# OpenStitching/stitching

Hardware: AMD Instinct MI355X
Metric: warped+blended Mpix/s (higher is better)
Workload: dtype u8/int16 (fixed-point remap, int32 pyramid sums, fp32 weights); 1 GPU; BASELINE config 2: 8 synthetic 4000x3000 frames, one ring; yaw step 38.9 deg = 0.58 hfov (42 % overlap; SURVEY 8(d) names 0.70 hfov); spherical warp + 5-band multiband blend, inputs resident in HBM; frames_per_gpu=8, panoramas_in_flight=2

## Files before the change

### include/stitching_amd.h

```cpp
#ifndef STITCHING_AMD_H
#define STITCHING_AMD_H

#include <stddef.h>
#include <stdint.h>

#ifdef __cplusplus
extern "C" {
#endif

#define STX_VERSION 100

#define STX_OK 0
#define STX_ERR_INVALID (-1)
#define STX_ERR_HIP (-2)
#define STX_ERR_OOM (-3)
#define STX_ERR_STATE (-4)
#define STX_ERR_UNSUPPORTED (-5)

#define STX_TRIG_EXACT 0
#define STX_TRIG_GLIBC 1
#define STX_TRIG_GLIBC_NOFMA 2
int stx_set_trig_mode(int mode);
int stx_get_trig_mode(void);

#define STX_REMAP_Q15 0
#define STX_REMAP_FLOAT 1
#define STX_REMAP_FLOAT_FMA 2
int stx_set_remap_mode(int mode);
int stx_get_remap_mode(void);

#define STX_PYRDOWN_SCALAR 0
#define STX_PYRDOWN_SIMD_V 1
#define STX_PYRDOWN_SIMD_HV 3
#define STX_PYRDOWN_FMA 4
int stx_set_pyrdown_mode(int mode, int lanes);
int stx_get_pyrdown_mode(int* out_lanes);

#define STX_WARP_PLANE 0
#define STX_WARP_AFFINE 1
#define STX_WARP_CYLINDRICAL 2
#define STX_WARP_SPHERICAL 3
#define STX_WARP_FISHEYE 4
#define STX_WARP_STEREOGRAPHIC 5
#define STX_WARP_COMPRESSED_PLANE_A2B1 6
#define STX_WARP_COMPRESSED_PLANE_A15B1 7
#define STX_WARP_COMPRESSED_PLANE_PORTRAIT_A2B1 8
#define STX_WARP_COMPRESSED_PLANE_PORTRAIT_A15B1 9
#define STX_WARP_PANINI_A2B1 10
#define STX_WARP_PANINI_A15B1 11
#define STX_WARP_PANINI_PORTRAIT_A2B1 12
#define STX_WARP_PANINI_PORTRAIT_A15B1 13
#define STX_WARP_MERCATOR 14
#define STX_WARP_TRANSVERSE_MERCATOR 15
#define STX_WARP_TYPE_COUNT 16

#define STX_INTER_NEAREST 0
#define STX_INTER_LINEAR 1
#define STX_BORDER_CONSTANT 0
#define STX_BORDER_REFLECT 2

#define STX_BLEND_NO 0
#define STX_BLEND_FEATHER 1
#define STX_BLEND_MULTIBAND 2

#define STX_U8 0
#define STX_S16 1
#define STX_F32 2

typedef struct stx_ctx stx_ctx;
typedef struct stx_buf stx_buf;
typedef struct stx_blender stx_blender;

int stx_version(void);
const char* stx_last_error(void);
int stx_device_count(int* out_n);
int stx_ctx_create(int device, stx_ctx** out);
int stx_ctx_destroy(stx_ctx* ctx);
int stx_ctx_sync(stx_ctx* ctx);

int stx_buf_from_host(stx_ctx* ctx, const void* host, size_t host_stride_bytes, int w, int h, int channels, int elem,
                      stx_buf** out);
int stx_buf_alloc(stx_ctx* ctx, int w, int h, int channels, int elem, stx_buf** out);
int stx_host_alloc(size_t bytes, void** out);
int stx_host_free(void* p);
int stx_buf_to_host(const stx_buf* buf, void* host, size_t host_stride_bytes);
int stx_buf_from_host_async(stx_ctx* ctx, const void* host, size_t host_stride_bytes, int w, int h, int channels, int elem,
                            stx_buf** out);
int stx_buf_to_host_async(const stx_buf* buf, void* host, size_t host_stride_bytes);
int stx_buf_view(const stx_buf* buf, int x, int y, int w, int h, stx_buf** out);
int stx_buf_info(const stx_buf* buf, int64_t info[6]);
int stx_buf_device_ptr(const stx_buf* buf, void** out);
int stx_buf_free(stx_buf* buf);

int stx_warp_roi(stx_ctx* ctx, int type, float scale, const float K[9], const float R[9], int w, int h,
                 int out_xywh[4]);
int stx_warp_rois(stx_ctx* ctx, int type, float scale, int n, const float* K9s, const float* R9s, const int* sizes_wh,
                  int* out_xywh);
int stx_warp(stx_ctx* ctx, int type, float scale, const float K[9], const float R[9], const stx_buf* src, int interp,
             int border, stx_buf** out, int out_tl[2]);
int stx_warp_image_and_mask(stx_ctx* ctx, int type, float scale, const float K[9], const float R[9],
                            const stx_buf* src, stx_buf** out_img, stx_buf** out_mask, int out_xywh[4]);
int stx_warp_batch(stx_ctx* ctx, int type, float scale, int n, const float* K9s, const float* R9s,
                   const stx_buf* const* srcs, stx_buf** out_imgs, stx_buf** out_masks, int* out_xywh);
int stx_warp_batch_rects(stx_ctx* ctx, int type, float scale, int n, const float* K9s, const float* R9s,
                         const stx_buf* const* srcs, const int* rects_xywh, stx_buf** out_imgs, stx_buf** out_masks);
int stx_warp_batch_gain(stx_ctx* ctx, int type, float scale, int n, const float* K9s, const float* R9s, const stx_buf* const* srcs,
                        const int* rects_xywh, const stx_buf* const* gain_maps_f32, const int* gain_flags, stx_buf** out_imgs,
                        stx_buf** out_masks, int* out_xywh);
int stx_warp_batch_with_rois(stx_ctx* ctx, int type, float scale, int n, const float* K9s, const float* R9s, const stx_buf* const* srcs,
                             const stx_buf* const* gain_maps_f32_or_null, const int* gain_flags_or_null, stx_buf** out_imgs,
                             stx_buf** out_masks, int* out_xywh);
int stx_warp_mask(stx_ctx* ctx, int type, float scale, const float K[9], const float R[9], int w, int h,
                  stx_buf** out_mask, int out_xywh[4]);

int stx_result_roi(int n, const int* corners_xy, const int* sizes_wh, int out_xywh[4]);
int stx_blend_create(stx_ctx* ctx, int kind, int num_bands, float sharpness, const int roi_xywh[4],
                     stx_blender** out);
int stx_blend_num_bands(const stx_blender* b, int* out_num_bands);
int stx_blend_feed(stx_blender* b, const stx_buf* img, const stx_buf* mask, int tlx, int tly);
int stx_blend_finish(stx_blender* b, stx_buf** out_pano_u8, stx_buf** out_mask_u8);
int stx_blend_finish_ex(stx_blender* b, stx_buf** out_pano_u8, stx_buf** out_mask_u8, stx_buf** out_pano_s16);
int stx_blend_destroy(stx_blender* b);

int stx_gain_apply(stx_ctx* ctx, stx_buf* img_u8x3, const float gains_bgr[3]);
int stx_block_gain_apply(stx_ctx* ctx, stx_buf* img_u8x3, const stx_buf* gain_map_f32);
#define STX_GAIN_MAP_BOUNDED 1
int stx_block_gain_apply_batch(stx_ctx* ctx, int n, stx_buf* const* imgs_u8x3, const stx_buf* const* gain_maps_f32,
                               const int* full_wh_xy0, const int* flags);
#define STX_EXPOSURE_GAIN 1
#define STX_EXPOSURE_GAIN_BLOCKS 2
#define STX_EXPOSURE_CHANNELS 3
#define STX_EXPOSURE_CHANNELS_BLOCKS 4
int stx_exposure_feed(stx_ctx* ctx, int kind, int n, const stx_buf* const* imgs_u8x3, const stx_buf* const* masks_u8,
                      const int* corners_xy, int block_size, int nr_feeds, double* out_gains, long long* inout_count,
                      double out_info[4]);
int stx_exposure_stats(stx_ctx* ctx, int kind, int n, const stx_buf* const* imgs_u8x3, const stx_buf* const* masks_u8,
                       const int* corners_xy, int block_size, long long* inout_jobs, int* out_ab, long long* out_c,
                       double* out_sums);
int stx_exposure_solve(int m, int npairs, const int* pairs_ij, const double* n_iij_iji, const unsigned char* skip,
                       double* out_gains);
#define STX_EXPOSURE_SOLVER_DEFAULT (-1)
#define STX_EXPOSURE_SOLVER_HOST 0
#define STX_EXPOSURE_SOLVER_DEVICE 1
int stx_set_exposure_solver(int mode);
int stx_get_exposure_solver(void);
int stx_exposure_feed_ex(stx_ctx* ctx, int kind, int n, const stx_buf* const* imgs_u8x3, const stx_buf* const* masks_u8,
                         const int* corners_xy, int block_size, int nr_feeds, int solver, double* out_gains, long long* inout_count,
                         double out_info[8]);
int stx_exposure_solve_device(stx_ctx* ctx, int m, int npairs, const int* pairs_ij, const double* n_iij_iji, const unsigned char* skip,
                              double* out_gains, double out_info[4]);
int stx_lu_solve_device(stx_ctx* ctx, int n, const double* A_dense_host, const double* b_host, double* x_out, double out_info[4]);
#define STX_SEAM_NO 0
#define STX_SEAM_VORONOI 1
#define STX_SEAM_GAP 10
int stx_seam_find(stx_ctx* ctx, int kind, int n, const int* sizes_wh, const int* corners_xy, const stx_buf* const* masks_in,
                  stx_buf** masks_out, double out_info[4]);
int stx_seam_schedule(int n, const int* sizes_wh, const int* corners_xy, int* inout_npairs, int* out_pairs, int* out_levels);
#define STX_COLOR_SEAM_MAX_LENGTH 16384
#define STX_COLOR_SEAM_MAX_CROSS 4096
int stx_color_seam_find(stx_ctx* ctx, int n, const int* sizes_wh, const int* corners_xy, const stx_buf* const* images,
                        const stx_buf* const* masks_in, stx_buf** masks_out, double out_info[4]);
int stx_crop_lir(stx_ctx* ctx, const stx_buf* mask_u8x1, int out_xywh[4], int out_contours[2], double out_info[1]);
#define STX_FEATURES_MAX_SIDE 32767
#define STX_FEATURES_MAX_LEVELS 16
#define STX_FEATURES_MAX_FEATURES 65536
int stx_features_detect(stx_ctx* ctx, int n, const stx_buf* const* images, const stx_buf* const* masks, int nfeatures, int nlevels,
                        int fast_threshold, const int* level_counts, const int* level_wh, const int* quotas, const int* cxcy,
                        const signed char* patterns, int* out_counts, int* out_lxyb, long long* out_R, unsigned char* out_desc,
                        double out_info[4]);
int stx_resize_linear_exact(stx_ctx* ctx, const stx_buf* src_u8, int dst_w, int dst_h, stx_buf** out);
int stx_seam_mask_resize(stx_ctx* ctx, const stx_buf* seam_mask_u8x1, const stx_buf* final_mask_u8x1, stx_buf** out);
int stx_resize_linear_exact_batch(stx_ctx* ctx, int n, const stx_buf* const* srcs_u8, const int* dst_wh, stx_buf** outs);
int stx_seam_mask_resize_batch(stx_ctx* ctx, int n, const stx_buf* const* seam_masks, const stx_buf* const* final_masks,
                               stx_buf** outs);
int stx_seam_mask_resize_batch_sub(stx_ctx* ctx, int n, const stx_buf* const* seam_masks, const stx_buf* const* final_masks,
// ... 59 lines not shown
```

### stitching_amd/_lib.py

```python
import ctypes as C
import os

from .stitching_error import StitchingError

_HERE = os.path.dirname(os.path.abspath(__file__))
LIB_PATH = os.environ.get("STITCHING_AMD_LIB") or os.path.join(_HERE, "libstitching_amd.so")

STX_OK = 0
WARP_PLANE, WARP_AFFINE, WARP_CYLINDRICAL, WARP_SPHERICAL = 0, 1, 2, 3
WARP_TYPE_IDS = {"plane": 0, "affine": 1, "cylindrical": 2, "spherical": 3, "fisheye": 4, "stereographic": 5,
                 "compressedPlaneA2B1": 6, "compressedPlaneA1.5B1": 7, "compressedPlanePortraitA2B1": 8,
                 "compressedPlanePortraitA1.5B1": 9, "paniniA2B1": 10, "paniniA1.5B1": 11, "paniniPortraitA2B1": 12,
                 "paniniPortraitA1.5B1": 13, "mercator": 14, "transverseMercator": 15}
INTER_NEAREST, INTER_LINEAR = 0, 1
BORDER_CONSTANT, BORDER_REFLECT = 0, 2
BLEND_NO, BLEND_FEATHER, BLEND_MULTIBAND = 0, 1, 2
U8, S16, F32 = 0, 1, 2
TRIG_MODES = {"exact": 0, "glibc": 1, "glibc-nofma": 2}
REMAP_MODES = {"q15": 0, "float": 1, "float-fma": 2}
PYRDOWN_MODES = {"scalar": 0, "simd-v": 1, "simd-hv": 3, "simd-v-fma": 5, "simd-hv-fma": 7}
GAIN_MAP_BOUNDED = 1
EXPOSURE_KINDS = {"gain": 1, "gain_blocks": 2, "channel": 3, "channel_blocks": 4}
EXPOSURE_SOLVERS = {"host": 0, "device": 1}
LU_NB, LU_MAX_N = 32, 16384
SEAM_KINDS = {"no": 0, "voronoi": 1}
COLOR_SEAM_MAX_LENGTH, COLOR_SEAM_MAX_CROSS = 16384, 4096
FEATURES_MAX_SIDE, FEATURES_MAX_LEVELS, FEATURES_MAX_FEATURES = 32767, 16, 65536
CONTRIB_U8_BINARY = 1
STRIP_MASK_BITS = 2

EXPORTS = (
    "stx_version stx_last_error stx_set_trig_mode stx_get_trig_mode stx_set_remap_mode stx_get_remap_mode stx_set_pyrdown_mode stx_get_pyrdown_mode stx_device_count stx_ctx_create stx_ctx_destroy stx_ctx_sync "
    "stx_host_alloc stx_host_free stx_buf_from_host stx_buf_from_host_async stx_buf_alloc stx_buf_to_host stx_buf_to_host_async stx_buf_view stx_buf_info stx_buf_device_ptr stx_buf_free "
    "stx_warp_roi stx_warp_rois stx_warp stx_warp_image_and_mask stx_warp_batch stx_warp_batch_rects stx_warp_batch_gain stx_warp_batch_with_rois stx_warp_mask "
    "stx_gain_apply stx_block_gain_apply stx_block_gain_apply_batch stx_resize_linear_exact stx_resize_linear_exact_batch stx_seam_mask_resize stx_seam_mask_resize_batch stx_seam_mask_resize_batch_sub stx_timelapse_frame stx_result_roi stx_blend_create stx_blend_num_bands stx_blend_feed stx_blend_finish stx_blend_finish_ex "
    "stx_blend_destroy stx_blend_set_band stx_blend_feed_ex stx_blend_contrib_rect stx_blend_export_contrib stx_blend_export_contribs "
    "stx_blend_build stx_blend_feed_contrib stx_blend_feed_contrib_ex stx_buf_flags stx_strip_rect stx_view_rect stx_strip_pack stx_strip_pack_batch stx_strip_pack_batch_ex stx_strip_bytes stx_strip_unpack stx_blend_feed_strips stx_comm_unique_id stx_comm_create stx_comm_exchange stx_comm_exchange_begin stx_comm_exchange_end stx_comm_exchange_begin_on stx_comm_exchange_end_on stx_comm_info stx_comm_destroy stx_prof_enable stx_prof_reset stx_prof_count stx_prof_get stx_mark stx_mark_elapsed_ms "
    "stx_exposure_feed stx_exposure_stats stx_exposure_solve stx_set_exposure_solver stx_get_exposure_solver stx_exposure_feed_ex stx_exposure_solve_device stx_lu_solve_device stx_seam_find stx_seam_schedule stx_color_seam_find stx_crop_lir stx_features_detect "
    "stx_debug_warp_maps stx_debug_feather_dist_cap"
).split()

_lib = None


def build_hint():
    return "build it with `make -C stitching_amd/csrc` or `python -c 'import __graft_entry__ as g; g.build()'`"


def lib():
    global _lib
    if _lib is not None:
        return _lib
    if not os.path.exists(LIB_PATH):
        raise ImportError(f"{LIB_PATH} is missing: the HIP back end is not built ({build_hint()}). "
                          "stitching_amd has no CPU fallback.")
    L = C.CDLL(LIB_PATH)
    vp, vpp = C.c_void_p, C.POINTER(C.c_void_p)
    fp, ip = C.POINTER(C.c_float), C.POINTER(C.c_int)
    L.stx_version.restype = C.c_int
    L.stx_last_error.restype = C.c_char_p
    L.stx_set_trig_mode.argtypes = [C.c_int]
    L.stx_get_trig_mode.restype = C.c_int
    L.stx_set_remap_mode.argtypes = [C.c_int]
    L.stx_get_remap_mode.restype = C.c_int
    L.stx_set_pyrdown_mode.argtypes = [C.c_int, C.c_int]
    L.stx_get_pyrdown_mode.argtypes = [C.POINTER(C.c_int)]
    L.stx_get_pyrdown_mode.restype = C.c_int
    L.stx_device_count.argtypes = [ip]
    L.stx_ctx_create.argtypes = [C.c_int, vpp]
    L.stx_ctx_destroy.argtypes = [vp]
    L.stx_ctx_sync.argtypes = [vp]
    L.stx_buf_from_host.argtypes = [vp, vp, C.c_size_t, C.c_int, C.c_int, C.c_int, C.c_int, vpp]
    L.stx_buf_from_host_async.argtypes = L.stx_buf_from_host.argtypes
    L.stx_buf_alloc.argtypes = [vp, C.c_int, C.c_int, C.c_int, C.c_int, vpp]
    L.stx_host_alloc.argtypes = [C.c_size_t, vpp]
    L.stx_host_free.argtypes = [vp]
    L.stx_buf_to_host.argtypes = [vp, vp, C.c_size_t]
    L.stx_buf_to_host_async.argtypes = [vp, vp, C.c_size_t]
    L.stx_buf_view.argtypes = [vp, C.c_int, C.c_int, C.c_int, C.c_int, vpp]
    L.stx_buf_info.argtypes = [vp, C.POINTER(C.c_int64)]
    L.stx_buf_device_ptr.argtypes = [vp, vpp]
    L.stx_buf_free.argtypes = [vp]
    L.stx_warp_roi.argtypes = [vp, C.c_int, C.c_float, fp, fp, C.c_int, C.c_int, ip]
    L.stx_warp_rois.argtypes = [vp, C.c_int, C.c_float, C.c_int, fp, fp, ip, ip]
    L.stx_warp.argtypes = [vp, C.c_int, C.c_float, fp, fp, vp, C.c_int, C.c_int, vpp, ip]
    L.stx_warp_image_and_mask.argtypes = [vp, C.c_int, C.c_float, fp, fp, vp, vpp, vpp, ip]
    L.stx_warp_batch.argtypes = [vp, C.c_int, C.c_float, C.c_int, fp, fp, vpp, vpp, vpp, ip]
    L.stx_warp_batch_rects.argtypes = [vp, C.c_int, C.c_float, C.c_int, fp, fp, vpp, ip, vpp, vpp]
    L.stx_warp_batch_gain.argtypes = [vp, C.c_int, C.c_float, C.c_int, fp, fp, vpp, ip, vpp, ip, vpp, vpp, ip]
    L.stx_warp_batch_with_rois.argtypes = [vp, C.c_int, C.c_float, C.c_int, fp, fp, vpp, vpp, ip, vpp, vpp, ip]
    L.stx_warp_mask.argtypes = [vp, C.c_int, C.c_float, fp, fp, C.c_int, C.c_int, vpp, ip]
    L.stx_gain_apply.argtypes = [vp, vp, fp]
    L.stx_block_gain_apply.argtypes = [vp, vp, vp]
    L.stx_block_gain_apply_batch.argtypes = [vp, C.c_int, vpp, vpp, ip, ip]
    L.stx_resize_linear_exact.argtypes = [vp, vp, C.c_int, C.c_int, vpp]
    L.stx_resize_linear_exact_batch.argtypes = [vp, C.c_int, vpp, ip, vpp]
    L.stx_seam_mask_resize.argtypes = [vp, vp, vp, vpp]
    L.stx_seam_mask_resize_batch.argtypes = [vp, C.c_int, vpp, vpp, vpp]
    L.stx_seam_mask_resize_batch_sub.argtypes = [vp, C.c_int, vpp, vpp, ip, vpp]
    L.stx_timelapse_frame.argtypes = [vp, vp, C.c_int, C.c_int, ip, vpp]
    L.stx_result_roi.argtypes = [C.c_int, ip, ip, ip]
    L.stx_blend_create.argtypes = [vp, C.c_int, C.c_int, C.c_float, ip, vpp]
    L.stx_blend_num_bands.argtypes = [vp, ip]
    L.stx_blend_feed.argtypes = [vp, vp, vp, C.c_int, C.c_int]
    L.stx_blend_finish.argtypes = [vp, vpp, vpp]
    L.stx_blend_finish_ex.argtypes = [vp, vpp, vpp, vpp]
    L.stx_blend_destroy.argtypes = [vp]
    L.stx_blend_set_band.argtypes = [vp, C.c_int, C.c_int]
    L.stx_blend_feed_ex.argtypes = [vp, vp, vp, C.c_int, C.c_int, C.c_int]
    L.stx_blend_contrib_rect.argtypes = [vp, C.c_int, C.c_int, C.c_int, C.c_int, C.c_int, C.c_int, ip,
                                         C.POINTER(C.c_size_t)]
    L.stx_blend_export_contrib.argtypes = [vp, C.c_int, C.c_int, C.c_int, vpp, ip]
    L.stx_blend_export_contribs.argtypes = [vp, C.c_int, ip, ip, ip, vpp, ip]
    L.stx_blend_build.argtypes = [vp]
    L.stx_blend_feed_contrib.argtypes = [vp, C.c_int, ip, vp]
    L.stx_blend_feed_contrib_ex.argtypes = [vp, C.c_int, ip, vp, C.c_int]
    L.stx_buf_flags.argtypes = [vp, ip]
    L.stx_strip_rect.argtypes = [vp, C.c_int, C.c_int, C.c_int, C.c_int, C.c_int, C.c_int, ip, C.POINTER(C.c_size_t)]
    L.stx_view_rect.argtypes = [vp, C.c_int, C.c_int, C.c_int, C.c_int, C.c_int, C.c_int, C.c_int, C.c_int, ip]
    L.stx_strip_pack.argtypes = [vp, vp, vp, C.c_int, C.c_int, vpp]
    L.stx_strip_unpack.argtypes = [vp, C.c_int, C.c_int, C.c_int, vpp, vpp]
    L.stx_strip_pack_batch.argtypes = [vp, C.c_int, vpp, vpp, ip, ip, vpp]
    L.stx_strip_pack_batch_ex.argtypes = [vp, C.c_int, vpp, vpp, ip, ip, C.c_int, vpp]
    L.stx_strip_bytes.argtypes = [C.c_int, C.c_int, C.c_int, C.POINTER(C.c_size_t)]
    L.stx_blend_feed_strips.argtypes = [vp, C.c_int, vpp, ip, ip, ip, ip, ip, C.c_int]
    L.stx_comm_unique_id.argtypes = [C.POINTER(C.c_ubyte)]
    L.stx_comm_create.argtypes = [vp, C.c_int, C.c_int, C.POINTER(C.c_ubyte), vpp]
    L.stx_comm_exchange.argtypes = [vp, C.c_int, ip, ip, C.POINTER(C.c_void_p), C.POINTER(C.c_size_t)]
    L.stx_comm_exchange_begin.argtypes = [vp, C.c_int, ip, ip, C.POINTER(C.c_void_p), C.POINTER(C.c_size_t)]
    L.stx_comm_exchange_end.argtypes = [vp]
    L.stx_comm_exchange_begin_on.argtypes = [vp, vp, C.c_int, ip, ip, C.POINTER(C.c_void_p), C.POINTER(C.c_size_t)]
    L.stx_comm_exchange_end_on.argtypes = [vp, vp]
    L.stx_comm_info.argtypes = [vp, ip]
    L.stx_comm_destroy.argtypes = [vp]
    L.stx_prof_enable.argtypes = [vp, C.c_int]
    L.stx_prof_reset.argtypes = [vp]
    L.stx_prof_count.argtypes = [vp, ip]
    L.stx_prof_get.argtypes = [vp, C.c_int, C.c_char_p, C.c_int, C.POINTER(C.c_int64), C.POINTER(C.c_double),
                               C.POINTER(C.c_double)]
    L.stx_debug_warp_maps.argtypes = [vp, C.c_int, C.c_float, fp, fp, C.c_int, C.c_int, C.c_int, ip, vpp, vpp, ip]
    llp, dp = C.POINTER(C.c_longlong), C.POINTER(C.c_double)
    L.stx_exposure_feed.argtypes = [vp, C.c_int, C.c_int, vpp, vpp, ip, C.c_int, C.c_int, dp, llp, dp]
    L.stx_exposure_stats.argtypes = [vp, C.c_int, C.c_int, vpp, vpp, ip, C.c_int, llp, ip, llp, dp]
    L.stx_exposure_solve.argtypes = [C.c_int, C.c_int, ip, dp, C.POINTER(C.c_ubyte), dp]
    L.stx_set_exposure_solver.argtypes = [C.c_int]
    L.stx_exposure_feed_ex.argtypes = [vp, C.c_int, C.c_int, vpp, vpp, ip, C.c_int, C.c_int, C.c_int, dp, llp, dp]
    L.stx_exposure_solve_device.argtypes = [vp, C.c_int, C.c_int, ip, dp, C.POINTER(C.c_ubyte), dp, dp]
    L.stx_lu_solve_device.argtypes = [vp, C.c_int, dp, dp, dp, dp]
    L.stx_seam_find.argtypes = [vp, C.c_int, C.c_int, ip, ip, vpp, vpp, dp]
    L.stx_seam_schedule.argtypes = [C.c_int, ip, ip, ip, ip, ip]
    L.stx_color_seam_find.argtypes = [vp, C.c_int, ip, ip, vpp, vpp, vpp, dp]
    L.stx_crop_lir.argtypes = [vp, vp, ip, ip, dp]
    L.stx_features_detect.argtypes = [vp, C.c_int, vpp, vpp, C.c_int, C.c_int, C.c_int, ip, ip, ip, ip, C.POINTER(C.c_byte), ip, ip, llp,
                                      C.POINTER(C.c_ubyte), dp]
    L.stx_mark.argtypes = [vp, C.c_int]
    L.stx_mark_elapsed_ms.argtypes = [vp, C.c_int, C.c_int, C.POINTER(C.c_double)]
    for name in EXPORTS:
        if name not in ("stx_version", "stx_last_error"):
            getattr(L, name).restype = C.c_int
    _lib = L
# ... 8 lines not shown
```

### stitching_amd/blender.py

```python
import ctypes as C

import numpy as np

from . import _lib, config
from .device import DeviceImage, as_device, get_context
from .stitching_error import StitchingError


class _BlenderHandle:

    def __init__(self, ctx, kind, num_bands, sharpness, roi):
        self.ctx = ctx
        self.kind = kind
        h = C.c_void_p()
        r = (C.c_int * 4)(*[int(v) for v in roi])
        _lib.check(ctx._lib.stx_blend_create(ctx.handle, kind, int(num_bands), float(sharpness), r, C.byref(h)))
        self._h = h

    def num_bands(self):
        n = C.c_int()
        _lib.check(self.ctx._lib.stx_blend_num_bands(self._h, C.byref(n)))
        return n.value

    def feed(self, img, mask, corner):
        _lib.check(self.ctx._lib.stx_blend_feed(self._h, img._h, mask._h, int(corner[0]), int(corner[1])))

    def blend(self, want_s16=False):
        pano, mask, p16 = C.c_void_p(), C.c_void_p(), C.c_void_p()
        _lib.check(self.ctx._lib.stx_blend_finish_ex(self._h, C.byref(pano), C.byref(mask),
                                                     C.byref(p16) if want_s16 else None))
        res = [DeviceImage(self.ctx, pano), DeviceImage(self.ctx, mask)]
        if want_s16:
            res.append(DeviceImage(self.ctx, p16))
        return res

    def __del__(self):
        try:
            if self._h is not None:
                if getattr(self.ctx, "handle", None) or getattr(self.ctx, "device", 0) == -1:
                    self.ctx._lib.stx_blend_destroy(self._h)
                self._h = None
        except Exception:
            pass


class Blender:

    BLENDER_CHOICES = (
        "multiband",
        "feather",
        "no",
    )
    DEFAULT_BLENDER = "multiband"
    DEFAULT_BLEND_STRENGTH = 5

    def __init__(
        self, blender_type=DEFAULT_BLENDER, blend_strength=DEFAULT_BLEND_STRENGTH, ctx=None
    ):
        self.blender_type = blender_type
        self.blend_strength = blend_strength
        self.blender = None
        self.ctx = ctx

    @staticmethod
    def result_roi(corners, sizes):
        c = np.ascontiguousarray([[int(p[0]), int(p[1])] for p in corners], np.int32)
        s = np.ascontiguousarray([[int(p[0]), int(p[1])] for p in sizes], np.int32)
        if len(c) == 0 or len(c) != len(s):
            raise StitchingError("prepare needs one size per corner and at least one image")
        out = (C.c_int * 4)()
        ip = C.POINTER(C.c_int)
        _lib.check(_lib.lib().stx_result_roi(len(c), c.ctypes.data_as(ip), s.ctypes.data_as(ip), out))
        return tuple(int(v) for v in out)

    @staticmethod
    def plan(blender_type, blend_strength, dst_sz):
        blend_width = np.sqrt(dst_sz[2] * dst_sz[3]) * blend_strength / 100
        if blender_type == "no" or blend_width < 1:
# ... 38 lines not shown
```

### stitching_amd/csrc/stx_blend.hip

```cpp
#include <cstring>

#include "stx_blend_kernels.h"
#include "stx_device_math.h"
#include "stx_internal.h"

using namespace stxd;

namespace {

constexpr float WEIGHT_EPS = 1e-5f;
constexpr float INV255 = 0.0039215688593685627f;
constexpr float INV256 = 0.00390625f;

template <bool S16>
STX_DEV void load_px0(const StxMbImage& im, int sx, int sy, int& b, int& g, int& r)
{
    if (S16) {
        const short* p = reinterpret_cast<const short*>(im.img0 + (long long)sy * im.img0_stride) + sx * 3;
        b = p[0]; g = p[1]; r = p[2];
    } else {
        const uint8_t* p = im.img0 + (long long)sy * im.img0_stride + sx * 3;
        b = p[0]; g = p[1]; r = p[2];
    }
}
// ... 594 lines not shown
    }
    __syncthreads();
    for (int i = tid; i < CO_TW * CO_TH; i += 256) {
        const int yy = i / CO_TW, xx = i - yy * CO_TW;
        const int x = tx0 + xx, y = ty0 + yy;
        if (x >= tx1 || y >= ty1) continue;
        int v[3];
        mb_gather_norm(P.images, P.n_images, B, B - 2, x, y, v);
        short* O = P.out + (long long)y * P.out_stride + (x - P.out_x0);
#pragma unroll
        for (int c = 0; c < 3; c++)
            O[c * P.out_plane] = (short)sat_s16(pyr_up_at_lds(s1[c], CO_W1, ax0, ay0, pw1, ph1, x, y) + v[c]);
    }
}

template <bool L0>
__global__ __launch_bounds__(256) void mb_level_kernel(MbLevelK P)
{
    mb_level_body<L0>(P);
}

template <bool L0>
__global__ __launch_bounds__(256) void mb_level_multi_kernel(const MbLevelK* __restrict__ Ps)
{
    mb_level_body<L0>(Ps[blockIdx.z]);
}

constexpr int DT_INF = 1 << 28;
constexpr int DT_RC = STX_DT_RC;
STX_DEV int wave_excl_prefix_min(int v)
{
    constexpr int ID = 0x7fffffff;
    v = min(v, __builtin_amdgcn_update_dpp(ID, v, 0x111, 0xf, 0xf, false));
    v = min(v, __builtin_amdgcn_update_dpp(ID, v, 0x112, 0xf, 0xf, false));
    v = min(v, __builtin_amdgcn_update_dpp(ID, v, 0x114, 0xf, 0xf, false));
    v = min(v, __builtin_amdgcn_update_dpp(ID, v, 0x118, 0xf, 0xf, false));
    v = min(v, __builtin_amdgcn_update_dpp(ID, v, 0x142, 0xa, 0xf, false));
    v = min(v, __builtin_amdgcn_update_dpp(ID, v, 0x143, 0xc, 0xf, false));
    return __builtin_amdgcn_update_dpp(ID, v, 0x138, 0xf, 0xf, false);
}

int check_launch(const char* what)
{
    hipError_t e = hipGetLastError();
    if (e != hipSuccess) return stx_fail(STX_ERR_HIP, "%s launch failed: %s", what, hipGetErrorString(e));
    return STX_OK;
}

inline dim3 grid64x4(int w, int h) { return dim3((w + 63) / 64, (h + 3) / 4); }

}

int stx_launch_mb_pyramids(stx_ctx* ctx, const StxMbImage* d_images, const StxMbImage* h_images, int n, int num_bands, int pyr_mode,
                           int pyr_lanes)
{
    for (int lv = 0; lv < num_bands; lv++) {
        double bytes = 0.0;
        bool any_s16 = false;
        for (int i = 0; i < n; i++) {
            const StxMbImage& im = h_images[i];
            const double ip = (double)(im.fw >> lv) * (im.fh >> lv), op = ip / 4.0;
            const double gw = (im.g_u8 ? 3.0 : 6.0) + 4.0;
            const double gw1 = gw - (im.w1_f16 ? 2.0 : 0.0);
            if (lv == 0) bytes += ((im.img0_is_s16 ? 6.0 : 3.0) + 1.0) * im.iw * im.ih + gw1 * op;
            else bytes += (lv == 1 ? gw1 : gw) * ip + gw * op;
            any_s16 = any_s16 || im.img0_is_s16;
        }
        StxProfScope prof(ctx, lv == 0 ? "mb_down0" : "mb_down", bytes);
        const bool batched = pyr_mode == STX_PYRDOWN_SCALAR && stx_fast_mb_down_batch(ctx, d_images, h_images, n, lv);
        for (int i = 0; i < n; i++) {
            const StxMbImage& im = h_images[i];
            if (batched && !(lv == 0 && im.img0_is_s16)) continue;
            const int ow = (im.fw >> lv) >> 1, oh = (im.fh >> lv) >> 1;
            if (lv == 0) {
                if (im.img0_is_s16) hipLaunchKernelGGL(mb_down0_kernel<true>, grid64x4(ow, oh), dim3(256), 0, ctx->stream, im, pyr_mode, pyr_lanes);
                else hipLaunchKernelGGL(mb_down0_kernel<false>, grid64x4(ow, oh), dim3(256), 0, ctx->stream, im, pyr_mode, pyr_lanes);
            } else {
                hipLaunchKernelGGL(mb_down_kernel, grid64x4(ow, oh), dim3(256), 0, ctx->stream, im, lv, pyr_mode, pyr_lanes);
            }
        }
        STX_TRY(check_launch("mb_down"));
    }
    return STX_OK;
}

int stx_launch_mb_coarse(stx_ctx* ctx, const MbLevelK& K, double algo_bytes)
{
    if (K.x1 <= K.x0 || K.y1 <= K.y0) return STX_OK;
    if (K.level != K.num_bands - 2 || K.level < 1 || K.y0 != 0 || K.out_y0 != 0 || K.emit)
        return stx_fail(STX_ERR_INVALID, "mb_coarse: not the argument block of level B-2");
    StxProfScope prof(ctx, "mb_coarse", algo_bytes);
    MbCoarseK C;
    C.images = K.images; C.n_images = K.n_images; C.num_bands = K.num_bands;
    C.x0 = K.x0; C.x1 = K.x1; C.y1 = K.y1;
    C.out = K.out; C.out_stride = K.out_stride; C.out_plane = K.out_plane; C.out_x0 = K.out_x0;
    C.pw = K.pw; C.ph = K.ph;
    const dim3 grid((K.x1 - K.x0 + CO_TW - 1) / CO_TW, (K.y1 + CO_TH - 1) / CO_TH);
    hipLaunchKernelGGL(mb_coarse_kernel, grid, dim3(256), 0, ctx->stream, C);
    return check_launch("mb_coarse");
}

int stx_launch_mb_level(stx_ctx* ctx, const MbLevelK& K, double algo_bytes)
{
    if (K.x1 <= K.x0 || K.y1 <= K.y0) return STX_OK;
    StxProfScope prof(ctx, K.emit ? "mb_contrib" : (K.level == 0 ? "mb_level0" : "mb_level"), algo_bytes);
    if ((K.level > 0 || K.all_u8) && stx_fast_mb_level(ctx, K)) return STX_OK;
    const dim3 grid = grid64x4(K.x1 - K.x0, K.y1 - K.y0);
    if (K.level == 0) hipLaunchKernelGGL(mb_level_kernel<true>, grid, dim3(256), 0, ctx->stream, K);
    else hipLaunchKernelGGL(mb_level_kernel<false>, grid, dim3(256), 0, ctx->stream, K);
    return check_launch("mb_level");
}

int stx_launch_mb_emit_batch(stx_ctx* ctx, const MbLevelK* d_Ks, const MbLevelK* h_Ks, const int* classes, int n, double bytes)
{
    if (n <= 0) return STX_OK;
    StxProfScope prof(ctx, "mb_contrib", bytes);
    for (int start = 0; start < n;) {
        int end = start;
        while (end < n && classes[end] == classes[start]) end++;
        const int cls = classes[start], count = end - start;
        if (cls >= 0) {
            if (!stx_fast_mb_emit_launch(ctx, cls, d_Ks + start, h_Ks + start, count)) return check_launch("mb_contrib");
// ... 1178 lines not shown
```

### stitching_amd/csrc/stx_blend_fast.hip

```cpp
#include <algorithm>
#include <cstdlib>

#include "stx_blend_kernels.h"
#include "stx_device_math.h"

using namespace stxd;

namespace {

#ifndef STX_L0_WAVES
#define STX_L0_WAVES 5
#endif
#ifndef STX_L0_NORM
#define STX_L0_NORM 3
#endif
#ifndef STX_ABLATE_MASK
#define STX_ABLATE_MASK 0
#endif
#ifndef STX_L0_FULL
#define STX_L0_FULL 1
#endif
constexpr float WEIGHT_EPS = 1e-5f;
constexpr float INV255 = 0.0039215688593685627f;
constexpr float INV256 = 0.00390625f;
// ... 247 lines not shown
    const v4u d1 = *reinterpret_cast<const STX_GAS v4u_a4*>(q + 16);
    const v2u d2 = *reinterpret_cast<const STX_GAS v2u_a4*>(q + 32);
    w[0] = __builtin_amdgcn_alignbyte(d0.y, d0.x, s);
    w[1] = __builtin_amdgcn_alignbyte(d0.z, d0.y, s);
    w[2] = __builtin_amdgcn_alignbyte(d0.w, d0.z, s);
    w[3] = __builtin_amdgcn_alignbyte(d1.x, d0.w, s);
    w[4] = __builtin_amdgcn_alignbyte(d1.y, d1.x, s);
    w[5] = __builtin_amdgcn_alignbyte(d1.z, d1.y, s);
    w[6] = __builtin_amdgcn_alignbyte(d1.w, d1.z, s);
    w[7] = __builtin_amdgcn_alignbyte(d2.x, d1.w, s);
    w[8] = __builtin_amdgcn_alignbyte(d2.y, d2.x, s);
}
template <bool MIRROR, int C>
STX_DEV void dn_pack5_channel(const uint32_t* w, short* hs)
{
#define STX_PXB(k) (MIRROR ? 30 - 3 * (k) + C : 3 * (k) + C)
    const pk16 A = pk(pair_u8<STX_PXB(0), STX_PXB(2)>(w)), Bp = pk(pair_u8<STX_PXB(1), STX_PXB(3)>(w));
    const pk16 Cp = pk(pair_u8<STX_PXB(2), STX_PXB(4)>(w)), D = pk(pair_u8<STX_PXB(3), STX_PXB(5)>(w));
    const pk16 E = pk(pair_u8<STX_PXB(4), STX_PXB(6)>(w)), F = pk(pair_u8<STX_PXB(5), STX_PXB(7)>(w));
    const pk16 G = pk(pair_u8<STX_PXB(6), STX_PXB(8)>(w)), H = pk(pair_u8<STX_PXB(7), STX_PXB(9)>(w));
    const pk16 I = pk(pair_u8<STX_PXB(8), STX_PXB(10)>(w));
#undef STX_PXB
    const pk16 o01 = A + E + Cp * pk_splat(6) + (Bp + D) * pk_splat(4);
    const pk16 o23 = E + I + G * pk_splat(6) + (F + H) * pk_splat(4);
    *reinterpret_cast<uint2*>(hs) = make_uint2(unpk(o01), unpk(o23));
}

#ifndef STX_DN0_DOT4
#define STX_DN0_DOT4 0
#endif
STX_DEV float4 dn_mask_sums4(const uint32_t (&mb)[3])
{
#if STX_DN0_DOT4
    const uint32_t o0 = __builtin_amdgcn_udot4(mb[0], 0x04060401u, mb[1] & 1u, false);
    const uint32_t o1 = __builtin_amdgcn_udot4(mb[1], 0x00010406u, __builtin_amdgcn_udot4(mb[0], 0x04010000u, 0u, false), false);
    const uint32_t o2 = __builtin_amdgcn_udot4(mb[1], 0x04060401u, mb[2] & 1u, false);
    const uint32_t o3 = __builtin_amdgcn_udot4(mb[2], 0x00010406u, __builtin_amdgcn_udot4(mb[1], 0x04010000u, 0u, false), false);
    return make_float4((float)o0, (float)o1, (float)o2, (float)o3);
#else
    const pk16 o01 = pk(pair_u8<0, 2>(mb)) + pk(pair_u8<4, 6>(mb)) + pk(pair_u8<2, 4>(mb)) * pk_splat(6) +
                     (pk(pair_u8<1, 3>(mb)) + pk(pair_u8<3, 5>(mb))) * pk_splat(4);
    const pk16 o23 = pk(pair_u8<4, 6>(mb)) + pk(pair_u8<8, 10>(mb)) + pk(pair_u8<6, 8>(mb)) * pk_splat(6) +
                     (pk(pair_u8<5, 7>(mb)) + pk(pair_u8<7, 9>(mb))) * pk_splat(4);
    return make_float4((float)(unpk(o01) & 0xffffu), (float)(unpk(o01) >> 16), (float)(unpk(o23) & 0xffffu), (float)(unpk(o23) >> 16));
#endif
}

struct DnImage0 {
    int fw, fh, iw, ih, left, top;
    uint32_t img0_stride, mask0_stride;
    const uint8_t* img0;
    const uint8_t* mask0;
};
template <bool PK, bool NEAR, class IM>
STX_DEV void dn_task_level0(const IM& im, int row, int xo, short* hs0, short* hs1, short* hs2, float* hw)
{
    const int by = reflect101_near(row, im.fh) - im.top;
    const bool yin = (unsigned)by < (unsigned)im.ih;
    const int sy = NEAR ? reflect_near(by, im.ih) : reflect(by, im.ih);
    const STX_GAS uint8_t* img = gp(im.img0);
    const uint32_t rowoff = (uint32_t)sy * (uint32_t)im.img0_stride;
    const int c0 = 2 * xo - 2;
    const int a0 = c0 - im.left;
    int px[11][3];
    float f[11];
    if (c0 >= 0 && c0 + 10 < im.fw && a0 >= 0 && a0 + 10 < im.iw) {
        uint32_t w[9];
        dn_load36(img, rowoff + (uint32_t)a0 * 3u, w);
        dn_pack5_channel<false, 0>(w, hs0);
        dn_pack5_channel<false, 1>(w, hs1);
        dn_pack5_channel<false, 2>(w, hs2);
        uint32_t mw[3] = {0u, 0u, 0u};
        if (yin) {
            const uint32_t moff = (uint32_t)by * (uint32_t)im.mask0_stride + (uint32_t)a0;
            const STX_GAS uint8_t* mq = gp(im.mask0) + (moff & ~3u);
            const uint32_t ms = moff & 3u;
            const v4u m = *reinterpret_cast<const STX_GAS v4u_a4*>(mq);
            mw[0] = __builtin_amdgcn_alignbyte(m.y, m.x, ms);
            mw[1] = __builtin_amdgcn_alignbyte(m.z, m.y, ms);
            mw[2] = __builtin_amdgcn_alignbyte(m.w, m.z, ms) & 0x00ffffffu;
        }
        bool packed = PK;
        if (!PK) {
            const uint32_t odd = (mw[0] ^ (((mw[0] >> 7) & 0x01010101u) * 255u)) | (mw[1] ^ (((mw[1] >> 7) & 0x01010101u) * 255u)) |
                                 (mw[2] ^ (((mw[2] >> 7) & 0x01010101u) * 255u));
            packed = __builtin_amdgcn_ballot_w64(odd != 0u) == 0ull;
        }
        if (packed) {
            uint32_t mb[3];
            mb[0] = mw[0] & 0x01010101u;
            mb[1] = mw[1] & 0x01010101u;
            mb[2] = mw[2] & 0x01010101u;
            *reinterpret_cast<float4*>(hw) = dn_mask_sums4(mb);
            return;
        }
#pragma unroll
        for (int j = 0; j < 11; j++) f[j] = fmul((float)byte_of(mw, j), INV255);
#pragma unroll
        for (int o = 0; o < 4; o++) hw[o] = h5f(f[2 * o], f[2 * o + 1], f[2 * o + 2], f[2 * o + 3], f[2 * o + 4]);
        return;
    }
    if (c0 >= 0 && c0 + 10 < im.fw && (a0 + 10 < 0 || a0 >= im.iw)) {
        const int s_low = a0 + 10 < 0 ? -(a0 + 10) - 1 : 2 * im.iw - 1 - (a0 + 10);
        if (s_low >= 0 && s_low + 10 < im.iw) {
            uint32_t w[9];
            dn_load36(img, rowoff + (uint32_t)s_low * 3u, w);
            dn_pack5_channel<true, 0>(w, hs0);
            dn_pack5_channel<true, 1>(w, hs1);
            dn_pack5_channel<true, 2>(w, hs2);
            *reinterpret_cast<float4*>(hw) = make_float4(0.f, 0.f, 0.f, 0.f);
            return;
        }
    }
    {
        const STX_GAS uint8_t* mrow = gp(im.mask0) + (uint32_t)min(max(by, 0), im.ih - 1) * (uint32_t)im.mask0_stride;
#pragma unroll
        for (int j = 0; j < 11; j++) {
            const int bx = reflect101_near(c0 + j, im.fw) - im.left;
            const int sx = NEAR ? reflect_near(bx, im.iw) : reflect(bx, im.iw);
            const STX_GAS uint8_t* p = img + (rowoff + (uint32_t)sx * 3u);
            px[j][0] = p[0]; px[j][1] = p[1]; px[j][2] = p[2];
            const float mv = fmul((float)mrow[sx], INV255);
            f[j] = (yin && (unsigned)bx < (unsigned)im.iw) ? mv : 0.f;
        }
    }
#pragma unroll
    for (int o = 0; o < 4; o++) {
        hs0[o] = (short)h5i(px[2 * o][0], px[2 * o + 1][0], px[2 * o + 2][0], px[2 * o + 3][0], px[2 * o + 4][0]);
        hs1[o] = (short)h5i(px[2 * o][1], px[2 * o + 1][1], px[2 * o + 2][1], px[2 * o + 3][1], px[2 * o + 4][1]);
        hs2[o] = (short)h5i(px[2 * o][2], px[2 * o + 1][2], px[2 * o + 2][2], px[2 * o + 3][2], px[2 * o + 4][2]);
        hw[o] = h5f(f[2 * o], f[2 * o + 1], f[2 * o + 2], f[2 * o + 3], f[2 * o + 4]);
    }
}

STX_DEV int occ_pitch(int lw) { return (((lw + 63) >> 6) + 3) & ~3; }
STX_DEV void dn_note_occ(uint8_t* __restrict__ occ, uint32_t nzbits, int tid, int X0, int Y0, int ow, int oh)
{
    const unsigned long long bal = __ballot(nzbits != 0u);
    const int rg = tid >> 5;
    if (occ == nullptr || (tid & 31) != 0 || 2 * rg >= DN_TOH || Y0 + 2 * rg >= oh) return;
    const uint32_t half = (tid & 32) ? (uint32_t)(bal >> 32) : (uint32_t)bal;
    occ[(long long)((Y0 >> 1) + rg) * occ_pitch(ow) + (X0 >> 6)] = half != 0u ? 1 : 0;
}

#ifndef STX_DN0_REV
#define STX_DN0_REV 1
#endif
#ifndef STX_DN0_BATCH
#define STX_DN0_BATCH 3
#endif
template <bool PK>
__global__ __launch_bounds__(256) void mb_down0_lds_kernel(const StxMbImage* __restrict__ images, StxTileMap M)
{
    __shared__ __attribute__((aligned(16))) short s_h[3][DN_ROWS][DN_TOW];
    __shared__ __attribute__((aligned(16))) float s_w[DN_ROWS][DN_TOW];
    const uint32_t zz = STX_DN0_REV ? gridDim.z - 1u - blockIdx.z : blockIdx.z, bb = STX_DN0_REV ? gridDim.x - 1u - blockIdx.x : blockIdx.x;
    const StxMbImage& im = images[zz];
    const int tid = threadIdx.x;
    const int ow = im.fw >> 1, oh = im.fh >> 1;
    int tile_tx, tile_ty;
    if (!xcd_tile(M, bb, tile_tx, tile_ty)) return;
    const int X0 = tile_tx * DN_TOW, Y0 = tile_ty * DN_TOH;
    if (im.img0_is_s16 || X0 >= ow || Y0 >= oh) return;
    uint8_t* const occ = im.occ[1];
    const bool w1h = im.w1_f16 != 0;
    asm volatile("" ::"s"(occ));
    DnImage0 D;
    {
        int fw = im.fw, fh = im.fh, iw_ = im.iw, ih_ = im.ih, left = im.left, top = im.top;
        uint32_t is = (uint32_t)im.img0_stride, ms = (uint32_t)im.mask0_stride;
        unsigned long long ia = (unsigned long long)im.img0, ma = (unsigned long long)im.mask0;
        if (PK) asm volatile("" : "+s"(fw), "+s"(fh), "+s"(iw_), "+s"(ih_), "+s"(left), "+s"(top), "+s"(is), "+s"(ms), "+s"(ia), "+s"(ma));
        D.fw = fw; D.fh = fh; D.iw = iw_; D.ih = ih_; D.left = left; D.top = top; D.img0_stride = is; D.mask0_stride = ms;
        D.img0 = (const uint8_t*)ia; D.mask0 = (const uint8_t*)ma;
    }
    uint32_t g1_plane = 0, g1_stride = 0, w1_stride = 0;
    unsigned long long g1_a = 0, w1_a = 0;
    if (PK) {
        g1_plane = (uint32_t)im.g_plane[1]; g1_stride = (uint32_t)im.g_stride[1]; w1_stride = (uint32_t)im.wt_stride[1];
        g1_a = (unsigned long long)im.g[1]; w1_a = (unsigned long long)im.wt[1];
        asm volatile("" : "+s"(g1_plane), "+s"(g1_stride), "+s"(w1_stride), "+s"(g1_a), "+s"(w1_a));
    }
    const int r_end = 2 * min(DN_TOH, oh - Y0) + 3;
    const bool near = PK ? (D.left <= D.iw && D.fw - D.left - D.iw <= D.iw && D.top <= D.ih && D.fh - D.top - D.ih <= D.ih)
                         : (im.left <= im.iw && im.fw - im.left - im.iw <= im.iw && im.top <= im.ih && im.fh - im.top - im.ih <= im.ih);
    bool batched = false;
    if ((STX_DN0_BATCH & (PK ? 1 : 2)) && near) {
        const int q = tid & 15, rA = tid >> 4;
        const int xo = X0 + 4 * q, c0 = 2 * xo - 2, a0 = c0 - D.left;
        const bool col_ok = xo < ow;
        const bool in_frame = c0 >= 0 && c0 + 10 < D.fw;
        const bool interior = in_frame && a0 >= 0 && a0 + 10 < D.iw;
        const int s_low = a0 + 10 < 0 ? -(a0 + 10) - 1 : 2 * D.iw - 1 - (a0 + 10);
        const bool mirrored = in_frame && (a0 + 10 < 0 || a0 >= D.iw) && s_low >= 0 && s_low + 10 < D.iw;
        batched = __builtin_amdgcn_ballot_w64(col_ok && !(interior || mirrored)) == 0ull;
        if (batched && col_ok) {
            const int acol = interior ? a0 : s_low;
            v4u d0[2], d1[2], mq4[2];
            v2u d2[2];
            uint32_t sh[2], msh[2];
            bool yin[2], live[2];
#pragma unroll
            for (int t = 0; t < 2; t++) {
                const int r = rA + 16 * t;
                live[t] = r < r_end && r < DN_ROWS;
                const int row = 2 * Y0 - 2 + min(r, r_end - 1);
                const int by = reflect101_near(row, D.fh) - D.top;
                yin[t] = (unsigned)by < (unsigned)D.ih;
                const int sy = reflect_near(by, D.ih);
                const uint32_t off = (uint32_t)sy * (uint32_t)D.img0_stride + (uint32_t)acol * 3u;
                const STX_GAS uint8_t* p = gp(D.img0) + (off & ~3u);
                sh[t] = off & 3u;
                d0[t] = *reinterpret_cast<const STX_GAS v4u_a4*>(p);
                d1[t] = *reinterpret_cast<const STX_GAS v4u_a4*>(p + 16);
                d2[t] = *reinterpret_cast<const STX_GAS v2u_a4*>(p + 32);
                const uint32_t moff = (uint32_t)min(max(by, 0), D.ih - 1) * (uint32_t)D.mask0_stride + (uint32_t)acol;
                msh[t] = moff & 3u;
#if STX_ABLATE_MASK
                mq4[t] = v4u{0xffffffffu, 0xffffffffu, 0xffffffffu, 0xffffffffu};
#else
                mq4[t] = *reinterpret_cast<const STX_GAS v4u_a4*>(gp(D.mask0) + (moff & ~3u));
#endif
            }
            __builtin_amdgcn_sched_barrier(0);
#pragma unroll
            for (int t = 0; t < 2; t++) {
                if (!live[t]) continue;
                const int r = rA + 16 * t;
                uint32_t w[9];
                w[0] = __builtin_amdgcn_alignbyte(d0[t].y, d0[t].x, sh[t]);
                w[1] = __builtin_amdgcn_alignbyte(d0[t].z, d0[t].y, sh[t]);
                w[2] = __builtin_amdgcn_alignbyte(d0[t].w, d0[t].z, sh[t]);
                w[3] = __builtin_amdgcn_alignbyte(d1[t].x, d0[t].w, sh[t]);
                w[4] = __builtin_amdgcn_alignbyte(d1[t].y, d1[t].x, sh[t]);
                w[5] = __builtin_amdgcn_alignbyte(d1[t].z, d1[t].y, sh[t]);
                w[6] = __builtin_amdgcn_alignbyte(d1[t].w, d1[t].z, sh[t]);
                w[7] = __builtin_amdgcn_alignbyte(d2[t].x, d1[t].w, sh[t]);
                w[8] = __builtin_amdgcn_alignbyte(d2[t].y, d2[t].x, sh[t]);
                if (interior) {
                    dn_pack5_channel<false, 0>(w, &s_h[0][r][4 * q]);
                    dn_pack5_channel<false, 1>(w, &s_h[1][r][4 * q]);
                    dn_pack5_channel<false, 2>(w, &s_h[2][r][4 * q]);
                } else {
                    dn_pack5_channel<true, 0>(w, &s_h[0][r][4 * q]);
                    dn_pack5_channel<true, 1>(w, &s_h[1][r][4 * q]);
                    dn_pack5_channel<true, 2>(w, &s_h[2][r][4 * q]);
                }
                const uint32_t keep = (yin[t] && interior) ? 0xffffffffu : 0u;
                uint32_t mw[3];
                mw[0] = __builtin_amdgcn_alignbyte(mq4[t].y, mq4[t].x, msh[t]) & keep;
                mw[1] = __builtin_amdgcn_alignbyte(mq4[t].z, mq4[t].y, msh[t]) & keep;
                mw[2] = __builtin_amdgcn_alignbyte(mq4[t].w, mq4[t].z, msh[t]) & keep & 0x00ffffffu;
                bool packed = PK;
                if (!PK) {
                    const uint32_t odd = (mw[0] ^ (((mw[0] >> 7) & 0x01010101u) * 255u)) | (mw[1] ^ (((mw[1] >> 7) & 0x01010101u) * 255u)) |
                                         (mw[2] ^ (((mw[2] >> 7) & 0x01010101u) * 255u));
                    packed = __builtin_amdgcn_ballot_w64(odd != 0u) == 0ull;
                }
                if (packed) {
                    uint32_t mb[3];
                    mb[0] = mw[0] & 0x01010101u;
                    mb[1] = mw[1] & 0x01010101u;
                    mb[2] = mw[2] & 0x01010101u;
                    *reinterpret_cast<float4*>(&s_w[r][4 * q]) = dn_mask_sums4(mb);
                } else {
                    float f[11];
#pragma unroll
                    for (int j = 0; j < 11; j++) f[j] = fmul((float)byte_of(mw, j), INV255);
#pragma unroll
                    for (int o = 0; o < 4; o++) s_w[r][4 * q + o] = h5f(f[2 * o], f[2 * o + 1], f[2 * o + 2], f[2 * o + 3], f[2 * o + 4]);
                }
            }
        }
    }
    for (int task = tid; task < DN_ROWS * (DN_TOW / 4) && !batched; task += 256) {
        const int r = task / (DN_TOW / 4), q = task % (DN_TOW / 4);
        if (X0 + 4 * q >= ow || r >= r_end) continue;
        if (PK) {
            if (near) dn_task_level0<PK, true>(D, 2 * Y0 - 2 + r, X0 + 4 * q, &s_h[0][r][4 * q], &s_h[1][r][4 * q], &s_h[2][r][4 * q], &s_w[r][4 * q]);
            else dn_task_level0<PK, false>(D, 2 * Y0 - 2 + r, X0 + 4 * q, &s_h[0][r][4 * q], &s_h[1][r][4 * q], &s_h[2][r][4 * q], &s_w[r][4 * q]);
        } else {
            if (near) dn_task_level0<PK, true>(im, 2 * Y0 - 2 + r, X0 + 4 * q, &s_h[0][r][4 * q], &s_h[1][r][4 * q], &s_h[2][r][4 * q], &s_w[r][4 * q]);
            else dn_task_level0<PK, false>(im, 2 * Y0 - 2 + r, X0 + 4 * q, &s_h[0][r][4 * q], &s_h[1][r][4 * q], &s_h[2][r][4 * q], &s_w[r][4 * q]);
        }
    }
    __syncthreads();
    const int p = tid & 31, rg = tid >> 5;
    const int xo = X0 + 2 * p;
    if (xo >= ow) return;
    const bool two = xo + 1 < ow;
    uint32_t nz = 0u;
#pragma unroll
    for (int rr = 0; rr < 2; rr++) {
        const int yl = 2 * rg + rr, y = Y0 + yl;
        if (yl >= DN_TOH || y >= oh) break;
#pragma unroll
        for (int c = 0; c < 3; c++) {
            pk16 a[5];
#pragma unroll
            for (int k = 0; k < 5; k++) a[k] = pk(*reinterpret_cast<const uint32_t*>(&s_h[c][2 * yl + k][2 * p]));
            const pk16 v = (a[0] + a[4] + a[2] * pk_splat(6) + (a[1] + a[3]) * pk_splat(4) + pk_splat(128)) >> pk_splat(8);
            STX_GAS uint8_t* o = PK ? gp(reinterpret_cast<uint8_t*>(g1_a)) + ((uint32_t)c * g1_plane + (uint32_t)y * g1_stride + (uint32_t)xo)
                                    : gp(reinterpret_cast<uint8_t*>(im.g[1])) + ((uint32_t)c * (uint32_t)im.g_plane[1] + (uint32_t)y * (uint32_t)im.g_stride[1] + (uint32_t)xo);
            const uint32_t b2 = __builtin_amdgcn_perm(0u, unpk(v), 0x0c0c0200u);
            if (two) *reinterpret_cast<STX_GAS uint16_t*>(o) = (uint16_t)b2;
            else o[0] = (uint8_t)b2;
        }
        float fa[5], fb[5];
        {
            typedef float v2 __attribute__((ext_vector_type(2)));
            v2 r0, r1, r2, r3, r4;
            const uint32_t a = (uint32_t)(uintptr_t)(__attribute__((address_space(3))) const float*)&s_w[2 * yl][2 * p];
            asm volatile("ds_read_b64 %0, %5\n\tds_read_b64 %1, %5 offset:256\n\tds_read_b64 %2, %5 offset:512\n\t"
                         "ds_read_b64 %3, %5 offset:768\n\tds_read_b64 %4, %5 offset:1024\n\ts_waitcnt lgkmcnt(0)"
                         : "=&v"(r0), "=&v"(r1), "=&v"(r2), "=&v"(r3), "=&v"(r4) : "v"(a) : "memory");
            fa[0] = r0.x; fb[0] = r0.y; fa[1] = r1.x; fb[1] = r1.y; fa[2] = r2.x; fb[2] = r2.y;
            fa[3] = r3.x; fb[3] = r3.y; fa[4] = r4.x; fb[4] = r4.y;
        }
        const float wa = fmul(h5f(fa[0], fa[1], fa[2], fa[3], fa[4]), INV256);
        const float wb = fmul(h5f(fb[0], fb[1], fb[2], fb[3], fb[4]), INV256);
        if (w1h) {
            STX_GAS _Float16* o = PK ? gp(reinterpret_cast<_Float16*>(w1_a)) + ((uint32_t)y * w1_stride + (uint32_t)xo)
                                     : reinterpret_cast<STX_GAS _Float16*>(gp(im.wt[1])) + ((uint32_t)y * (uint32_t)im.wt_stride[1] + (uint32_t)xo);
            typedef _Float16 v2h16 __attribute__((ext_vector_type(2)));
            if (two) { const v2h16 wab = {(_Float16)wa, (_Float16)wb}; *reinterpret_cast<STX_GAS v2h16*>(o) = wab; }
            else o[0] = (_Float16)wa;
        } else {
            STX_GAS float* o = PK ? gp(reinterpret_cast<float*>(w1_a)) + ((uint32_t)y * w1_stride + (uint32_t)xo)
                                  : gp(im.wt[1]) + ((uint32_t)y * (uint32_t)im.wt_stride[1] + (uint32_t)xo);
            typedef float v2fl __attribute__((ext_vector_type(2)));
            if (two) { const v2fl wab = {wa, wb}; *reinterpret_cast<STX_GAS v2fl*>(o) = wab; }
            else o[0] = wa;
        }
        nz |= __float_as_uint(wa) | (two ? __float_as_uint(wb) : 0u);
    }
    dn_note_occ(occ, nz, tid, X0, Y0, ow, oh);
}

STX_DEV void dn_load19_u8(const STX_GAS uint8_t* __restrict__ base, uint32_t off, int c0, int iw, bool fast, int s[19])
{
    if (fast) {
        const STX_GAS uint8_t* p = base + (off + (uint32_t)c0);
        const uint32_t a = *reinterpret_cast<const STX_GAS uint32_t*>(p - 2);
        const v4u b = *reinterpret_cast<const STX_GAS v4u*>(p + 2);
        const uint32_t c = *reinterpret_cast<const STX_GAS uint32_t*>(p + 18);
        const uint32_t w[6] = {a, b.x, b.y, b.z, b.w, c};
#pragma unroll
        for (int j = 0; j < 19; j++) s[j] = (int)byte_of(w, j + 2);
    } else {
#pragma unroll
        for (int j = 0; j < 19; j++) s[j] = base[off + (uint32_t)reflect101_near(c0 + j, iw)];
    }
}

STX_DEV void dn_load19_s16(const STX_GAS short* __restrict__ base, uint32_t off, int c0, int iw, bool fast, int s[19])
{
    if (fast) {
        const STX_GAS short* p = base + (off + (uint32_t)c0);
        const uint32_t a = *reinterpret_cast<const STX_GAS uint32_t*>(p);
        const v4u b = *reinterpret_cast<const STX_GAS v4u*>(p + 2);
        const v4u c = *reinterpret_cast<const STX_GAS v4u*>(p + 10);
        s[0] = s16lo(a); s[1] = s16hi(a);
        s[2] = s16lo(b.x); s[3] = s16hi(b.x); s[4] = s16lo(b.y); s[5] = s16hi(b.y);
        s[6] = s16lo(b.z); s[7] = s16hi(b.z); s[8] = s16lo(b.w); s[9] = s16hi(b.w);
        s[10] = s16lo(c.x); s[11] = s16hi(c.x); s[12] = s16lo(c.y); s[13] = s16hi(c.y);
        s[14] = s16lo(c.z); s[15] = s16hi(c.z); s[16] = s16lo(c.w); s[17] = s16hi(c.w);
        s[18] = p[18];
    } else {
#pragma unroll
        for (int j = 0; j < 19; j++) s[j] = base[off + (uint32_t)reflect101_near(c0 + j, iw)];
    }
}

STX_DEV void dn_hsum_store_i(const int (&s)[19], int* row_q)
{
    int4 lo, hi;
    lo.x = h5i(s[0], s[1], s[2], s[3], s[4]);
    lo.y = h5i(s[2], s[3], s[4], s[5], s[6]);
    lo.z = h5i(s[4], s[5], s[6], s[7], s[8]);
    lo.w = h5i(s[6], s[7], s[8], s[9], s[10]);
    hi.x = h5i(s[8], s[9], s[10], s[11], s[12]);
    hi.y = h5i(s[10], s[11], s[12], s[13], s[14]);
    hi.z = h5i(s[12], s[13], s[14], s[15], s[16]);
    hi.w = h5i(s[14], s[15], s[16], s[17], s[18]);
    *reinterpret_cast<int4*>(row_q) = make_int4(lo.x, lo.z, hi.x, hi.z);
    *reinterpret_cast<int4*>(row_q + 32) = make_int4(lo.y, lo.w, hi.y, hi.w);
}
STX_DEV void dn_hsum_store_f(const float (&f)[19], float* row_q)
{
    float4 lo, hi;
    lo.x = h5f(f[0], f[1], f[2], f[3], f[4]);
    lo.y = h5f(f[2], f[3], f[4], f[5], f[6]);
    lo.z = h5f(f[4], f[5], f[6], f[7], f[8]);
    lo.w = h5f(f[6], f[7], f[8], f[9], f[10]);
    hi.x = h5f(f[8], f[9], f[10], f[11], f[12]);
    hi.y = h5f(f[10], f[11], f[12], f[13], f[14]);
    hi.z = h5f(f[12], f[13], f[14], f[15], f[16]);
    hi.w = h5f(f[14], f[15], f[16], f[17], f[18]);
    *reinterpret_cast<float4*>(row_q) = make_float4(lo.x, lo.z, hi.x, hi.z);
    *reinterpret_cast<float4*>(row_q + 32) = make_float4(lo.y, lo.w, hi.y, hi.w);
}

__global__ __launch_bounds__(256) void mb_down_lds_kernel(const StxMbImage* __restrict__ images, int lv, StxTileMap M)
{
    __shared__ __attribute__((aligned(16))) int s_h[3][DN_ROWS][DN_TOW];
    __shared__ __attribute__((aligned(16))) float s_w[DN_ROWS][DN_TOW];
    const StxMbImage& im = images[blockIdx.z];
    const int tid = threadIdx.x;
    const int iw = im.fw >> lv, ih = im.fh >> lv;
    const int ow = iw >> 1, oh = ih >> 1;
    int tile_tx, tile_ty;
    if (!xcd_tile(M, blockIdx.x, tile_tx, tile_ty)) return;
    const int X0 = tile_tx * DN_TOW, Y0 = tile_ty * DN_TOH;
    if (X0 >= ow || Y0 >= oh) return;
    const bool g8b = im.g_u8 != 0;
    unsigned long long G_a = (unsigned long long)im.g[lv], W_a = (unsigned long long)im.wt[lv];
    unsigned long long Go_a = (unsigned long long)im.g[lv + 1], Wo_a = (unsigned long long)im.wt[lv + 1];
    uint32_t gs = (uint32_t)im.g_stride[lv], gpl = (uint32_t)im.g_plane[lv], wst = (uint32_t)im.wt_stride[lv];
    uint32_t gos = (uint32_t)im.g_stride[lv + 1], gopl = (uint32_t)im.g_plane[lv + 1], wost = (uint32_t)im.wt_stride[lv + 1];
    asm volatile("" : "+s"(G_a), "+s"(W_a), "+s"(Go_a), "+s"(Wo_a), "+s"(gs), "+s"(gpl), "+s"(wst), "+s"(gos), "+s"(gopl), "+s"(wost));
    const short* G = (const short*)G_a;
    uint8_t* const occ = im.occ[lv + 1];
    const bool w_half = lv == 1 && im.w1_f16 != 0;
    asm volatile("" ::"s"(occ));
    const int r_end = 2 * min(DN_TOH, oh - Y0) + 3;
    for (int task = tid; task < DN_ROWS * (DN_TOW / 8); task += 256) {
        const int r = task / (DN_TOW / 8), q = task % (DN_TOW / 8);
        if (X0 + 8 * q >= ow || r >= r_end) continue;
        const int sy = reflect101_near(2 * Y0 - 2 + r, ih);
        const int c0 = 2 * (X0 + 8 * q) - 2;
        const bool fast = c0 >= 0 && c0 + 18 < iw;
        typedef _Float16 v2h16 __attribute__((ext_vector_type(2)));
        typedef _Float16 v8h16 __attribute__((ext_vector_type(8)));
        if (g8b && __builtin_amdgcn_ballot_w64(!fast) == 0ull) {
            uint32_t ra[3], rc[3];
            v4u rb[3];
#pragma unroll
            for (int c = 0; c < 3; c++) {
                const STX_GAS uint8_t* pp = gp(reinterpret_cast<const uint8_t*>(G)) + ((uint32_t)c * gpl + (uint32_t)sy * gs + (uint32_t)c0);
                ra[c] = *reinterpret_cast<const STX_GAS uint32_t*>(pp - 2);
                rb[c] = *reinterpret_cast<const STX_GAS v4u*>(pp + 2);
                rc[c] = *reinterpret_cast<const STX_GAS uint32_t*>(pp + 18);
            }
            float f[19];
            if (w_half) {
                const STX_GAS _Float16* hq = gp(reinterpret_cast<const _Float16*>(W_a)) + (uint32_t)sy * wst;
                const v2h16 ha = *reinterpret_cast<const STX_GAS v2h16*>(hq + c0);
                const v8h16 hb = *reinterpret_cast<const STX_GAS v8h16*>(hq + c0 + 2), hc = *reinterpret_cast<const STX_GAS v8h16*>(hq + c0 + 10);
                const _Float16 hl = hq[c0 + 18];
                __builtin_amdgcn_sched_barrier(0);
                f[0] = (float)ha.x; f[1] = (float)ha.y;
#pragma unroll
                for (int k = 0; k < 8; k++) { f[2 + k] = (float)hb[k]; f[10 + k] = (float)hc[k]; }
                f[18] = (float)hl;
            } else {
                const STX_GAS float* wq0 = gp(reinterpret_cast<const float*>(W_a)) + (uint32_t)sy * wst;
                const v2u wa = *reinterpret_cast<const STX_GAS v2u*>(wq0 + c0);
                v4u wb4[4];
#pragma unroll
                for (int k4 = 0; k4 < 4; k4++) wb4[k4] = *reinterpret_cast<const STX_GAS v4u*>(wq0 + c0 + 2 + 4 * k4);
                const float wl = wq0[c0 + 18];
                __builtin_amdgcn_sched_barrier(0);
                f[0] = __uint_as_float(wa.x); f[1] = __uint_as_float(wa.y);
#pragma unroll
                for (int k = 0; k < 4; k++) {
                    f[2 + 4 * k] = __uint_as_float(wb4[k].x); f[3 + 4 * k] = __uint_as_float(wb4[k].y); f[4 + 4 * k] = __uint_as_float(wb4[k].z);
                    f[5 + 4 * k] = __uint_as_float(wb4[k].w);
                }
                f[18] = wl;
            }
#pragma unroll
            for (int c = 0; c < 3; c++) {
                const uint32_t w6[6] = {ra[c], rb[c].x, rb[c].y, rb[c].z, rb[c].w, rc[c]};
                int s[19];
#pragma unroll
                for (int j = 0; j < 19; j++) s[j] = (int)byte_of(w6, j + 2);
                dn_hsum_store_i(s, &s_h[c][r][4 * q]);
            }
            dn_hsum_store_f(f, &s_w[r][4 * q]);
            continue;
        }
#pragma unroll
        for (int c = 0; c < 3; c++) {
            int s[19];
            if (g8b) dn_load19_u8(gp(reinterpret_cast<const uint8_t*>(G)), (uint32_t)c * gpl + (uint32_t)sy * gs, c0, iw, fast, s);
            else dn_load19_s16(gp(G), (uint32_t)c * gpl + (uint32_t)sy * gs, c0, iw, fast, s);
            dn_hsum_store_i(s, &s_h[c][r][4 * q]);
        }
        const STX_GAS float* wq = gp(reinterpret_cast<const float*>(W_a)) + (uint32_t)sy * wst;
        float f[19];
        if (w_half) {
            const STX_GAS _Float16* hq = gp(reinterpret_cast<const _Float16*>(W_a)) + (uint32_t)sy * wst;
            if (fast) {
                const v2h16 a = *reinterpret_cast<const STX_GAS v2h16*>(hq + c0);
                const v8h16 b = *reinterpret_cast<const STX_GAS v8h16*>(hq + c0 + 2), c = *reinterpret_cast<const STX_GAS v8h16*>(hq + c0 + 10);
                f[0] = (float)a.x; f[1] = (float)a.y;
#pragma unroll
                for (int k = 0; k < 8; k++) { f[2 + k] = (float)b[k]; f[10 + k] = (float)c[k]; }
                f[18] = (float)hq[c0 + 18];
            } else {
#pragma unroll
                for (int j = 0; j < 19; j++) f[j] = (float)hq[reflect101_near(c0 + j, iw)];
            }
        } else if (fast) {
            const v2u a = *reinterpret_cast<const STX_GAS v2u*>(wq + c0);
            f[0] = __uint_as_float(a.x); f[1] = __uint_as_float(a.y);
#pragma unroll
            for (int k = 0; k < 4; k++) {
                const v4u b = *reinterpret_cast<const STX_GAS v4u*>(wq + c0 + 2 + 4 * k);
                f[2 + 4 * k] = __uint_as_float(b.x); f[3 + 4 * k] = __uint_as_float(b.y); f[4 + 4 * k] = __uint_as_float(b.z);
                f[5 + 4 * k] = __uint_as_float(b.w);
            }
            f[18] = wq[c0 + 18];
        } else {
#pragma unroll
            for (int j = 0; j < 19; j++) f[j] = wq[reflect101_near(c0 + j, iw)];
        }
        dn_hsum_store_f(f, &s_w[r][4 * q]);
    }
    __syncthreads();
    const int p = tid & 31, rg = tid >> 5;
    const int xo = X0 + 2 * p;
    if (xo >= ow) return;
    const bool two = xo + 1 < ow;
    uint32_t nz = 0u;
#pragma unroll
    for (int rr = 0; rr < 2; rr++) {
        const int yl = 2 * rg + rr, y = Y0 + yl;
        if (yl >= DN_TOH || y >= oh) break;
#pragma unroll
        for (int c = 0; c < 3; c++) {
            int a[5], b[5];
#pragma unroll
            for (int k = 0; k < 5; k++) {
                a[k] = s_h[c][2 * yl + k][p];
                b[k] = s_h[c][2 * yl + k][32 + p];
            }
            const int va = (h5i(a[0], a[1], a[2], a[3], a[4]) + 128) >> 8;
            const int vb = (h5i(b[0], b[1], b[2], b[3], b[4]) + 128) >> 8;
            const uint32_t oo = (uint32_t)c * gopl + (uint32_t)y * gos + (uint32_t)xo;
            if (g8b) {
                STX_GAS uint8_t* o = gp(reinterpret_cast<uint8_t*>(Go_a)) + oo;
                if (two) *reinterpret_cast<STX_GAS uint16_t*>(o) = (uint16_t)((uint32_t)va | ((uint32_t)vb << 8));
                else o[0] = (uint8_t)va;
            } else {
                STX_GAS short* o = gp(reinterpret_cast<short*>(Go_a)) + oo;
                if (two) *reinterpret_cast<STX_GAS uint32_t*>(o) = pack16(va, vb);
                else o[0] = (short)va;
            }
        }
        float fa[5], fb[5];
#pragma unroll
        for (int k = 0; k < 5; k++) {
            fa[k] = s_w[2 * yl + k][p];
            fb[k] = s_w[2 * yl + k][32 + p];
        }
        const float wa = fmul(h5f(fa[0], fa[1], fa[2], fa[3], fa[4]), INV256);
        const float wb = fmul(h5f(fb[0], fb[1], fb[2], fb[3], fb[4]), INV256);
        STX_GAS float* o = gp(reinterpret_cast<float*>(Wo_a)) + ((uint32_t)y * wost + (uint32_t)xo);
        typedef float v2fl __attribute__((ext_vector_type(2)));
        if (two) { const v2fl wab = {wa, wb}; *reinterpret_cast<STX_GAS v2fl*>(o) = wab; }
        else o[0] = wa;
        nz |= __float_as_uint(wa) | (two ? __float_as_uint(wb) : 0u);
    }
    dn_note_occ(occ, nz, tid, X0, Y0, ow, oh);
}

STX_DEV int s6(int v) { return (v + 32) >> 6; }

STX_DEV int trunc_small(float v) { return (int)v; }

template <class T>
STX_DEV void up_patch(const T* __restrict__ plane, long long stride, int cw, int ch, int cx, int cy, int up[2][8])
{
    const int rr[3] = {up_idx(cy - 1, ch), cy, up_idx(cy + 1, ch)};
    const bool le = cx == 0, re = cx + 4 >= cw;
    int he[3][4], ho[3][4];
#pragma unroll
    for (int r = 0; r < 3; r++) {
        const T* p = plane + (long long)rr[r] * stride;
        int c[6];
        if (sizeof(T) == 2) {
            const v4u w = *reinterpret_cast<const v4u_a4*>(p + cx - 2);
            c[1] = s16lo(w.y); c[2] = s16hi(w.y); c[3] = s16lo(w.z); c[4] = s16hi(w.z);
            c[0] = s16hi(w.x);
            c[5] = s16lo(w.w);
        } else {
            const v3u w = *reinterpret_cast<const v3u_a4*>(p + cx - 4);
            c[0] = (int)(w.x >> 24);
            c[1] = (int)(w.y & 255u); c[2] = (int)((w.y >> 8) & 255u); c[3] = (int)((w.y >> 16) & 255u); c[4] = (int)(w.y >> 24);
            c[5] = (int)(w.z & 255u);
        }
        if (le) c[0] = c[2];
        if (re) c[5] = c[4];
#pragma unroll
        for (int j = 0; j < 4; j++) {
            he[r][j] = c[j] + 6 * c[j + 1] + c[j + 2];
            ho[r][j] = 4 * (c[j + 1] + c[j + 2]);
        }
    }
#pragma unroll
    for (int j = 0; j < 4; j++) {
        up[0][2 * j] = s6(he[0][j] + 6 * he[1][j] + he[2][j]);
        up[0][2 * j + 1] = s6(ho[0][j] + 6 * ho[1][j] + ho[2][j]);
        up[1][2 * j] = s6(4 * (he[1][j] + he[2][j]));
        up[1][2 * j + 1] = s6(4 * (ho[1][j] + ho[2][j]));
    }
}

template <bool L0>
STX_DEV void level_epilogue(const MbLevelK& P, int X0, int Y0, int (&acc)[2][8][3], float (&ws)[2][8])
{
    int v[2][8][3];
#pragma unroll
    for (int r = 0; r < 2; r++)
#pragma unroll
        for (int j = 0; j < 8; j++) {
            const float den = fadd(ws[r][j], WEIGHT_EPS);
// ... 1119 lines not shown
#elif STX_LVPK_EPI == 2
        up_patch_pks_load(gp(plane0), (uint32_t)P.up_stride, P.ph >> 1, (uint32_t)(X0 >> 1) * 2u, Y0 >> 1, uw[0]);
        up_patch_pks_load(gp(plane0 + P.up_plane), (uint32_t)P.up_stride, P.ph >> 1, (uint32_t)(X0 >> 1) * 2u, Y0 >> 1, uw[1]);
        __builtin_amdgcn_sched_barrier(0);
#endif
#pragma unroll
        for (int c = 0; c < 3; c++) {
            const short* plane = P.up + c * P.up_plane - ((long long)P.up_y0 * P.up_stride + P.up_x0);
#if STX_LVPK_EPI == 2
            if (c == 0) {
                up_patch_pks_load(gp(plane0 + 2 * P.up_plane), (uint32_t)P.up_stride, P.ph >> 1, (uint32_t)(X0 >> 1) * 2u, Y0 >> 1, uw[2]);
                __builtin_amdgcn_sched_barrier(0);
            }
#elif STX_LVPK_EPI < 2
            up_patch_pks_load(gp(plane), (uint32_t)P.up_stride, P.ph >> 1, (uint32_t)(X0 >> 1) * 2u, Y0 >> 1, uw[c]);
#endif
            pk16s up[2][4];
            if (!up_patch_pks_math(uw[c], usel, up)) {
                int u32[2][8];
                up_patch(plane, P.up_stride, P.pw >> 1, P.ph >> 1, X0 >> 1, Y0 >> 1, u32);
#pragma unroll
                for (int r = 0; r < 2; r++) {
                    up[r][0] = pks(pack16(u32[r][0], u32[r][2]));
                    up[r][1] = pks(pack16(u32[r][4], u32[r][6]));
                    up[r][2] = pks(pack16(u32[r][1], u32[r][3]));
                    up[r][3] = pks(pack16(u32[r][5], u32[r][7]));
                }
            }
#pragma unroll
            for (int r = 0; r < 2; r++)
#pragma unroll
                for (int q = 0; q < 4; q++) v[r][c][q] = unpks(__builtin_elementwise_add_sat(up[r][q], pks(v[r][c][q])));
        }
    }
#pragma unroll
    for (int r = 0; r < 2; r++) {
        if (Y0 + r >= P.y1) break;
#pragma unroll
        for (int c = 0; c < 3; c++) {
            v4u o;
            o.x = __builtin_amdgcn_perm(v[r][c][2], v[r][c][0], 0x05040100u);
            o.y = __builtin_amdgcn_perm(v[r][c][2], v[r][c][0], 0x07060302u);
            o.z = __builtin_amdgcn_perm(v[r][c][3], v[r][c][1], 0x05040100u);
            o.w = __builtin_amdgcn_perm(v[r][c][3], v[r][c][1], 0x07060302u);
            *reinterpret_cast<STX_GAS v4u*>(gp(P.out) + c * P.out_plane + (long long)(Y0 + r - P.out_y0) * P.out_stride + (X0 - P.out_x0)) = o;
        }
    }
}

bool launched_ok() { return hipGetLastError() == hipSuccess; }

}

bool stx_fast_mb_down_batch(stx_ctx* ctx, const StxMbImage* d_images, const StxMbImage* h_images, int n, int level)
{
    int mw = 0, mh = 0;
    for (int i = 0; i < n; i++) {
        mw = std::max(mw, (h_images[i].fw >> level) >> 1);
        mh = std::max(mh, (h_images[i].fh >> level) >> 1);
    }
    if (n <= 0 || mw < 1 || mh < 1 || n > 65535) return false;
    StxTileMap M = stx_tile_map((mw + DN_TOW - 1) / DN_TOW, (mh + DN_TOH - 1) / DN_TOH, DN_BAND);
#ifndef STX_DN_PLAIN_FROM
#define STX_DN_PLAIN_FROM 3
#endif
    M.plain = level >= STX_DN_PLAIN_FROM;
    bool pk_ok = true;
    for (int i = 0; i < n; i++) pk_ok = pk_ok && !h_images[i].img0_is_s16 && h_images[i].mask_binary;
    dim3 grid(stx_tile_grid(M), 1, n);
    static const unsigned pad_lds = getenv("STITCHING_AMD_D0_LDS") ? (unsigned)atoi(getenv("STITCHING_AMD_D0_LDS")) : 0u;
    if (level == 0 && pk_ok) hipLaunchKernelGGL(mb_down0_lds_kernel<true>, grid, dim3(256), pad_lds, ctx->stream, d_images, M);
    else if (level == 0) hipLaunchKernelGGL(mb_down0_lds_kernel<false>, grid, dim3(256), 0, ctx->stream, d_images, M);
    else hipLaunchKernelGGL(mb_down_lds_kernel, grid, dim3(256), 0, ctx->stream, d_images, level, M);
    return launched_ok();
}

static bool fast_level_ok(const MbLevelK& K, MbLevelK* KT)
{
    if (K.num_bands - K.level < 3) return false;
    if ((K.x0 | K.y0 | K.out_x0 | K.out_y0 | K.pano_x0 | K.pano_y0) & 7) return false;
    if (K.up && ((K.up_x0 | K.up_y0) & 3)) return false;
    if (K.n_images > 255) return false;
    *KT = K;
    KT->tiles = stx_tile_map((K.x1 - K.x0 + 511) / 512, (K.y1 - K.y0 + LV_TH - 1) / LV_TH, LV_BAND);
    return true;
}

int stx_fast_mb_emit_class(const MbLevelK& K, MbLevelK* KT)
{
    if (!(K.level > 0 || K.all_u8) || !fast_level_ok(K, KT)) { *KT = K; return -1; }
    return K.level == 0 ? 0 : (K.all_u8 ? 1 : 2);
}

bool stx_fast_mb_emit_launch(stx_ctx* ctx, int cls, const MbLevelK* d_Ks, const MbLevelK* h_Ks, int count)
{
    unsigned gx = 1;
    for (int i = 0; i < count; i++) gx = std::max(gx, stx_tile_grid(h_Ks[i].tiles));
    const dim3 grid(gx, 1, (unsigned)count);
    if (cls == 0) hipLaunchKernelGGL((mb_emit_multi_kernel<true, false>), grid, dim3(LV_THREADS), 0, ctx->stream, d_Ks);
    else if (cls == 1) hipLaunchKernelGGL((mb_emit_multi_kernel<false, true>), grid, dim3(LV_THREADS), 0, ctx->stream, d_Ks);
    else hipLaunchKernelGGL((mb_emit_multi_kernel<false, false>), grid, dim3(LV_THREADS), 0, ctx->stream, d_Ks);
    return launched_ok();
}

static bool no_defer()
{
    static const bool off = getenv("STITCHING_AMD_NO_DEFER") != nullptr;
    return off;
}

bool stx_fast_mb_level(stx_ctx* ctx, const MbLevelK& K)
{
    MbLevelK KT;
    if (!fast_level_ok(K, &KT)) return false;
    dim3 grid(stx_tile_grid(KT.tiles), 1);
    hipStream_t st = ctx->stream;
    if (K.level == 0 && K.pk_ok && !K.emit && K.num_bands > 0) {
        static const unsigned pad_lds = getenv("STITCHING_AMD_L0_LDS") ? (unsigned)atoi(getenv("STITCHING_AMD_L0_LDS")) : 0u;
        if (K.has_contrib) hipLaunchKernelGGL(mb_level0_pk_kernel<true>, grid, dim3(LV_THREADS), pad_lds, st, KT);
        else hipLaunchKernelGGL(mb_level0_pk_kernel<false>, grid, dim3(LV_THREADS), pad_lds, st, KT);
    } else if (K.level == 0 && K.all_u8 && !K.has_contrib && !K.emit && K.num_bands > 0 && !no_defer()) {
        const int segs = std::min(KT.tiles.tiles_x, STX_DEFER_SEGS);
        const size_t seg_cap = (size_t)((KT.tiles.tiles_x + STX_DEFER_SEGS - 1) / STX_DEFER_SEGS) * (size_t)KT.tiles.tiles_y * (unsigned)LV_THREADS;
        const size_t counters = (size_t)STX_DEFER_SEGS * 128;
        KT.defer_segs = segs;
        StxDevBlock q;
// ... 39 lines not shown
```

### stitching_amd/csrc/stx_blend_host.cpp

```cpp
#include <algorithm>
#include <climits>
#include <cmath>
#include <cstdlib>
#include <cstring>
#include <memory>

#include "stx_blend_kernels.h"
#include "stx_internal.h"

STX_EXPORT int stx_debug_feather_dist_cap(void) { return STX_FEATHER_DIST_CAP; }

STX_EXPORT int stx_result_roi(int n, const int* corners_xy, const int* sizes_wh, int out_xywh[4])
{
    if (n <= 0 || !corners_xy || !sizes_wh || !out_xywh) return stx_fail(STX_ERR_INVALID, "bad argument");
    int tlx = INT_MAX, tly = INT_MAX, brx = INT_MIN, bry = INT_MIN;
    for (int i = 0; i < n; i++) {
        tlx = std::min(tlx, corners_xy[2 * i]);
        tly = std::min(tly, corners_xy[2 * i + 1]);
        brx = std::max(brx, corners_xy[2 * i] + sizes_wh[2 * i]);
        bry = std::max(bry, corners_xy[2 * i + 1] + sizes_wh[2 * i + 1]);
    }
    out_xywh[0] = tlx; out_xywh[1] = tly; out_xywh[2] = brx - tlx; out_xywh[3] = bry - tly;
    return STX_OK;
}

constexpr size_t MB_FRONT_PAD = 64;

static void blender_release(stx_blender* b)
{
    for (stx_buf* h : b->held) stx_buf_release(h);
    b->held.clear();
    for (void* p : b->pyr_allocs) stx_dev_free(b->ctx, p);
    b->pyr_allocs.clear();
    b->d_all = nullptr;
    b->images.clear();
    b->built.clear();
    b->no_images.clear();
    b->feather_images.clear();
}

STX_EXPORT int stx_blend_create(stx_ctx* ctx, int kind, int num_bands, float sharpness, const int roi_xywh[4],
                                stx_blender** out)
{
    if (!roi_xywh || !out) return stx_fail(STX_ERR_INVALID, "null argument");
    if (!ctx && kind != STX_BLEND_MULTIBAND) return stx_fail(STX_ERR_INVALID, "ctx is null");
    if (ctx) STX_TRY(stx_set_device(ctx));
    if (kind < STX_BLEND_NO || kind > STX_BLEND_MULTIBAND) return stx_fail(STX_ERR_INVALID, "unknown blender kind %d", kind);
    int w = roi_xywh[2], h = roi_xywh[3];
    if (w <= 0 || h <= 0) return stx_fail(STX_ERR_INVALID, "empty destination roi %dx%d", w, h);
    std::unique_ptr<stx_blender> b(new stx_blender());
    b->ctx = ctx;
    b->kind = kind;
    b->sharpness = sharpness;
    b->fw = w; b->fh = h;
    if (kind == STX_BLEND_MULTIBAND) {
        if (num_bands < 0) return stx_fail(STX_ERR_INVALID, "num_bands %d", num_bands);
        double max_len = (double)std::max(w, h);
        int nb = std::min(num_bands, (int)std::ceil(std::log(max_len) / std::log(2.0)));
        if (nb > STX_MAX_BANDS) nb = STX_MAX_BANDS;
        b->num_bands = nb;
        w += ((1 << nb) - w % (1 << nb)) % (1 << nb);
        h += ((1 << nb) - h % (1 << nb)) % (1 << nb);
    }
    b->rx = roi_xywh[0]; b->ry = roi_xywh[1]; b->rw = w; b->rh = h;
    b->band_x0 = 0; b->band_x1 = b->fw;
    b->pyr_mode = pyrdown_now();
    *out = b.release();
    return STX_OK;
}

STX_EXPORT int stx_blend_num_bands(const stx_blender* b, int* out_num_bands)
{
    if (!b || !out_num_bands) return stx_fail(STX_ERR_INVALID, "null argument");
    *out_num_bands = b->num_bands;
    return STX_OK;
}

void mb_feed_rect(const stx_blender* b, int w, int h, int tlx, int tly, int* fx, int* fy, int* fw, int* fh)
{
    const int nb = b->num_bands;
    const int gap = 3 * (1 << nb);
    int tlnx = std::max(b->rx, tlx - gap), tlny = std::max(b->ry, tly - gap);
    int brnx = std::min(b->rx + b->rw, tlx + w + gap), brny = std::min(b->ry + b->rh, tly + h + gap);
    tlnx = b->rx + (((tlnx - b->rx) >> nb) << nb);
    tlny = b->ry + (((tlny - b->ry) >> nb) << nb);
    int width = brnx - tlnx, height = brny - tlny;
// ... 38 lines not shown
struct ContribLayout {
    size_t g_off[STX_MAX_BANDS + 1], w_off[STX_MAX_BANDS + 1];
    long long g_stride[STX_MAX_BANDS + 1], w_stride[STX_MAX_BANDS + 1];
    size_t bytes;
};
static void mb_contrib_layout(int nb, int w, int h, ContribLayout* L)
{
    size_t off = 0;
    for (int i = 0; i <= nb; i++) {
        const int lw = w >> i, lh = h >> i;
        L->g_stride[i] = (long long)align_up((size_t)std::max(lw, 1), 32);
        L->w_stride[i] = (long long)align_up((size_t)std::max(lw, 1), 16);
        L->g_off[i] = off;
        off = align_up(off + (size_t)L->g_stride[i] * std::max(lh, 1) * 3 * sizeof(short), 256);
        L->w_off[i] = off;
        off = align_up(off + (size_t)L->w_stride[i] * std::max(lh, 1) * sizeof(float), 256);
    }
    L->bytes = off;
}

static void mb_insert_sorted(stx_blender* b, const StxMbImage& im, bool is_built)
{
    size_t pos = b->images.size();
    while (pos > 0 && b->images[pos - 1].order > im.order) pos--;
    b->images.insert(b->images.begin() + pos, im);
    b->built.insert(b->built.begin() + pos, is_built ? 1 : 0);
    b->d_all = nullptr;
}

static int mb_feed(stx_blender* b, const stx_buf* img, const stx_buf* mask, int tlx, int tly, int order)
{
    stx_ctx* ctx = b->ctx;
    const int nb = b->num_bands, w = img->w, h = img->h;
    StxMbImage im;
    memset(&im, 0, sizeof(im));
    im.kind = 0;
    im.order = order;
    mb_feed_rect(b, w, h, tlx, tly, &im.fx, &im.fy, &im.fw, &im.fh);
    im.img0 = img->ptr; im.img0_stride = (long long)img->stride; im.img0_is_s16 = img->elem == STX_S16;
    im.mask0 = mask->ptr; im.mask0_stride = (long long)mask->stride; im.mask_binary = mask->mask_binary;
    im.iw = w; im.ih = h;
    im.ix = tlx - b->rx; im.iy = tly - b->ry;
    im.left = im.ix - im.fx; im.top = im.iy - im.fy;
    im.g_u8 = img->elem == STX_U8 ? 1 : 0;
    static const bool w1_f32 = getenv("STITCHING_AMD_W1_F32") != nullptr;
    im.w1_f16 = (mask->mask_binary && !w1_f32) ? 1 : 0;
    for (int i = 1; i <= nb; i++) {
        const int lw = im.fw >> i, lh = im.fh >> i;
        const long long gs = (long long)align_up((size_t)lw, im.g_u8 ? 64 : 32), ws = (long long)align_up((size_t)lw, 16);
        void *g = nullptr, *wt = nullptr;
        STX_TRY(stx_dev_alloc(ctx, MB_FRONT_PAD + (size_t)gs * lh * 3 * (im.g_u8 ? 1 : sizeof(short)) + 64, &g));
        b->pyr_allocs.push_back(g);
        STX_TRY(stx_dev_alloc(ctx, (size_t)ws * lh * ((i == 1 && im.w1_f16) ? sizeof(uint16_t) : sizeof(float)), &wt));
        b->pyr_allocs.push_back(wt);
        im.g[i] = (short*)((uint8_t*)g + MB_FRONT_PAD); im.g_stride[i] = gs; im.g_plane[i] = gs * lh;
        im.wt[i] = (float*)wt; im.wt_stride[i] = ws;
    }
    mb_insert_sorted(b, im, nb == 0);
    stx_buf_retain(const_cast<stx_buf*>(img));
    stx_buf_retain(const_cast<stx_buf*>(mask));
    b->held.push_back(const_cast<stx_buf*>(img));
    b->held.push_back(const_cast<stx_buf*>(mask));
    return STX_OK;
}

static int mb_upload(stx_blender* b, const StxMbImage* h, int n, StxMbImage** d_out)
{
    stx_ctx* ctx = b->ctx;
    void* d = nullptr;
    STX_TRY(stx_dev_alloc(ctx, sizeof(StxMbImage) * std::max(n, 1), &d));
    b->pyr_allocs.push_back(d);
    if (n > 0) STX_TRY(stx_stage_upload(ctx, d, h, sizeof(StxMbImage) * (size_t)n));
    *d_out = (StxMbImage*)d;
    return STX_OK;
}

static int mb_ensure_pyramids(stx_blender* b)
{
    std::vector<StxMbImage> todo;
    for (size_t i = 0; i < b->images.size(); i++)
        if (b->images[i].kind == 0 && !b->built[i]) todo.push_back(b->images[i]);
    if (todo.empty()) return STX_OK;
    static const bool occ_off = getenv("STITCHING_AMD_NO_OCC") != nullptr;
    const int pyr = b->pyr_mode;
    if (todo.size() <= 65535 && !occ_off && (pyr & 255) == STX_PYRDOWN_SCALAR) {
        const int nl = b->num_bands + 1;
        std::vector<size_t> off(todo.size() * (size_t)nl, 0);
        size_t bytes = 0;
        for (size_t t = 0; t < todo.size(); t++) {
            if (todo[t].img0_is_s16) continue;
            for (int i = 1; i < nl; i++) {
                off[t * nl + i] = bytes;
                bytes += (size_t)((((todo[t].fh >> i) + 1) >> 1) + 1) * (size_t)(((((todo[t].fw >> i) + 63) >> 6) + 3) & ~3);
            }
        }
        if (bytes > 0) {
            void* arena = nullptr;
            STX_TRY(stx_dev_alloc(b->ctx, bytes + 16, &arena));
            b->pyr_allocs.push_back(arena);
            size_t t = 0;
            for (size_t i = 0; i < b->images.size(); i++) {
                if (!(b->images[i].kind == 0 && !b->built[i])) continue;
                if (!todo[t].img0_is_s16)
                    for (int l = 1; l < nl; l++) todo[t].occ[l] = b->images[i].occ[l] = (uint8_t*)arena + off[t * nl + l];
                t++;
            }
        }
    }
    StxMbImage* d = nullptr;
    STX_TRY(mb_upload(b, todo.data(), (int)todo.size(), &d));
    b->d_all = todo.size() == b->images.size() && memcmp(todo.data(), b->images.data(), sizeof(StxMbImage) * todo.size()) == 0 ? d : nullptr;
    STX_TRY(stx_launch_mb_pyramids(b->ctx, d, todo.data(), (int)todo.size(), b->num_bands, pyr & 255, pyr >> 8));
    for (size_t i = 0; i < b->images.size(); i++) b->built[i] = 1;
    return STX_OK;
}

static double mb_level_bytes(const stx_blender* b, const std::vector<StxMbImage>& imgs, int lv, int x0, int x1, bool emit,
                             bool with16)
{
    const int nb = b->num_bands;
    const int ph = lv == 0 ? b->fh : b->rh >> lv;
    double bytes = 0.0;
    for (const StxMbImage& im : imgs) {
        int rx = im.fx >> lv, rw = im.fw >> lv, ry = im.fy >> lv, rh = im.fh >> lv;
        if (lv == 0 && im.kind == 0) { rx = im.ix; rw = im.iw; ry = im.iy; rh = im.ih; }
        const double cols = std::max(0, std::min(rx + rw, x1) - std::max(rx, x0)), rows = std::min(ry + rh, ph) - ry;
        if (cols <= 0 || rows <= 0) continue;
        const double g3 = im.g_u8 ? 3.0 : 6.0;
        if (im.kind == 1) bytes += cols * rows * 10.0;
        else if (lv == 0) bytes += cols * rows * ((im.img0_is_s16 ? 6 : 3) + 1) + (nb > 0 ? cols * rows * g3 / 4.0 : 0.0);
        else bytes += cols * rows * (g3 + ((lv == 1 && im.w1_f16) ? 2.0 : 4.0)) + (lv < nb ? cols * rows * g3 / 4.0 : 0.0);
    }
    const double area = (double)(x1 - x0) * ph;
    if (emit) return bytes + area * 10.0;
    if (lv < nb) bytes += area * 6.0 / 4.0;
    bytes += lv == 0 ? area * (4 + (with16 ? 6 : 0)) : area * 6.0;
    return bytes;
}

STX_EXPORT int stx_blend_feed_ex(stx_blender* b, const stx_buf* img, const stx_buf* mask, int tlx, int tly, int order)
{
    if (!b || !img || !mask) return stx_fail(STX_ERR_INVALID, "null argument");
    if (b->finished) return stx_fail(STX_ERR_STATE, "feed after blend()");
    if (!b->ctx) return stx_fail(STX_ERR_STATE, "geometry-only blender (created without a context)");
    STX_TRY(stx_set_device(b->ctx));
    if (img->c != 3 || (img->elem != STX_U8 && img->elem != STX_S16))
        return stx_fail(STX_ERR_INVALID, "feed: image must be u8x3 or s16x3");
    if (mask->c != 1 || mask->elem != STX_U8) return stx_fail(STX_ERR_INVALID, "feed: mask must be u8x1");
    if (mask->w != img->w || mask->h != img->h)
        return stx_fail(STX_ERR_INVALID, "feed: mask %dx%d does not match image %dx%d", mask->w, mask->h, img->w, img->h);
    if (img->ctx != b->ctx || mask->ctx != b->ctx) return stx_fail(STX_ERR_INVALID, "feed: buffers belong to another context");
    const int ux = b->kind == STX_BLEND_MULTIBAND ? b->rx + b->fw : b->rx + b->rw;
    const int uy = b->kind == STX_BLEND_MULTIBAND ? b->ry + b->fh : b->ry + b->rh;
    if (tlx < b->rx || tly < b->ry || tlx + img->w > ux || tly + img->h > uy)
        return stx_fail(STX_ERR_INVALID, "feed: image at (%d,%d) size %dx%d leaves the prepared roi (%d,%d,%d,%d)", tlx, tly,
                        img->w, img->h, b->rx, b->ry, ux - b->rx, uy - b->ry);
    if (order < 0) order = b->next_order;
    b->next_order = std::max(b->next_order, order + 1);
    if (b->kind == STX_BLEND_MULTIBAND) return mb_feed(b, img, mask, tlx, tly, order);
    if (b->kind == STX_BLEND_NO) {
        NoImg im;
        memset(&im, 0, sizeof(im));
        im.img = img->ptr; im.istride = (long long)img->stride; im.is_s16 = img->elem == STX_S16;
        im.mask = mask->ptr; im.mstride = (long long)mask->stride;
        im.x = tlx - b->rx; im.y = tly - b->ry; im.w = img->w; im.h = img->h;
        im.mask_binary = mask->mask_binary;
        b->no_images.push_back(im);
        stx_buf_retain(const_cast<stx_buf*>(img));
        stx_buf_retain(const_cast<stx_buf*>(mask));
        b->held.push_back(const_cast<stx_buf*>(img));
        b->held.push_back(const_cast<stx_buf*>(mask));
        return STX_OK;
    }
    FeatherImg im;
    memset(&im, 0, sizeof(im));
    im.img = img->ptr; im.istride = (long long)img->stride; im.is_s16 = img->elem == STX_S16;
    im.mask = mask->ptr; im.mstride = (long long)mask->stride;
    im.x = tlx - b->rx; im.y = tly - b->ry; im.w = img->w; im.h = img->h;
    im.dstride = ((long long)img->w + 15) & ~15ll;
    im.n_chunks = (img->h + STX_DT_RC - 1) / STX_DT_RC;
    void *wm = nullptr, *summ = nullptr;
    STX_TRY(stx_dev_alloc(b->ctx, 64 + sizeof(uint16_t) * (size_t)im.dstride * img->h + 64, &wm));
    b->pyr_allocs.push_back(wm);
    wm = (uint8_t*)wm + 64;
    STX_TRY(stx_dev_alloc(b->ctx, (sizeof(unsigned long long) + 2 * sizeof(int)) * (size_t)im.dstride * im.n_chunks, &summ));
    b->pyr_allocs.push_back(summ);
    im.dist = (uint16_t*)wm;
    im.zbits = (unsigned long long*)summ;
    im.first = (int*)(im.zbits + (size_t)im.dstride * im.n_chunks); im.last = im.first + (size_t)im.dstride * im.n_chunks;
    b->feather_images.push_back(im);
    stx_buf_retain(const_cast<stx_buf*>(img));
    stx_buf_retain(const_cast<stx_buf*>(mask));
    b->held.push_back(const_cast<stx_buf*>(img));
    b->held.push_back(const_cast<stx_buf*>(mask));
    return STX_OK;
}
// ... 19 lines not shown
    StxMbImage* d_images = b->d_all;
    if (!d_images) STX_TRY(mb_upload(b, b->images.data(), n, &d_images));
    bool all_u8 = true, has_contrib = false, pk_ok = true;
    for (const StxMbImage& im : b->images) {
        if (im.kind == 0 && im.img0_is_s16) all_u8 = false;
        if (im.kind == 1) has_contrib = true;
        if ((im.kind == 0 && im.img0_is_s16) || !im.mask_binary) pk_ok = false;
    }
    int xb[STX_MAX_BANDS + 1], xe[STX_MAX_BANDS + 1];
    mb_level_regions(b, b->band_x0, b->band_x1, xb, xe);
    std::vector<short*> out(nb + 2, nullptr);
    std::vector<long long> ostride(nb + 2, 0), oplane(nb + 2, 0);
    static const bool no_fusion = getenv("STITCHING_AMD_NO_COARSE_FUSION") != nullptr;
    const bool fuse = nb >= 3 && !no_fusion;
    for (int lv = fuse ? nb - 2 : nb; lv >= 0; lv--) {
        MbLevelK K;
        mb_fill_common(b, &K, d_images, n, lv);
        K.all_u8 = all_u8 ? 1 : 0;
        K.has_contrib = has_contrib ? 1 : 0;
        K.pk_ok = pk_ok ? 1 : 0;
        K.x0 = xb[lv]; K.x1 = xe[lv]; K.y0 = 0; K.y1 = lv == 0 ? b->fh : b->rh >> lv;
        if (lv < nb) {
            K.up = out[lv + 1]; K.up_stride = ostride[lv + 1]; K.up_plane = oplane[lv + 1];
            K.up_x0 = xb[lv + 1]; K.up_y0 = 0;
        }
        if (lv == 0) {
            K.pano = pano->ptr; K.pano_stride = (long long)pano->stride;
            K.pmask = pmask->ptr; K.pmask_stride = (long long)pmask->stride;
            if (pano16) { K.pano16 = (short*)pano16->ptr; K.pano16_stride = (long long)pano16->stride; }
            K.pano_x0 = b->band_x0; K.pano_y0 = 0;
        } else {
            const int w = xe[lv] - xb[lv], ph = b->rh >> lv;
            const long long st = (long long)align_up((size_t)std::max(w, 1), 32);
            void* p = nullptr;
            STX_TRY(stx_dev_alloc(ctx, MB_FRONT_PAD + (size_t)st * ph * 3 * sizeof(short), &p));
            b->pyr_allocs.push_back(p);
            out[lv] = (short*)((uint8_t*)p + MB_FRONT_PAD); ostride[lv] = st; oplane[lv] = st * ph;
            K.out = out[lv]; K.out_stride = st; K.out_plane = st * ph;
            K.out_x0 = xb[lv]; K.out_y0 = 0;
        }
        if (fuse && lv == nb - 2) {
            double bytes = mb_level_bytes(b, b->images, lv, K.x0, K.x1, false, false) - (double)(K.x1 - K.x0) * (b->rh >> lv) * 6.0 / 4.0;
            for (int l2 = nb - 1; l2 <= nb; l2++)
                bytes += mb_level_bytes(b, b->images, l2, xb[l2], xe[l2], false, false) - (double)(xe[l2] - xb[l2]) * (b->rh >> l2) * (l2 < nb ? 7.5 : 6.0);
            K.up = nullptr;
            STX_TRY(stx_launch_mb_coarse(ctx, K, bytes));
            continue;
        }
        STX_TRY(stx_launch_mb_level(ctx, K, mb_level_bytes(b, b->images, lv, K.x0, K.x1, false, pano16 != nullptr)));
    }
    return STX_OK;
}

STX_EXPORT int stx_blend_set_band(stx_blender* b, int x0, int x1)
{
    if (!b) return stx_fail(STX_ERR_INVALID, "null argument");
    if (b->kind != STX_BLEND_MULTIBAND) return stx_fail(STX_ERR_UNSUPPORTED, "bands exist for the multi-band blender only");
    if (b->finished) return stx_fail(STX_ERR_STATE, "set_band after blend()");
    const int al = (1 << b->num_bands) - 1;
    if (x0 < 0 || x1 > b->fw || x1 <= x0 || (x0 & al) || ((x1 & al) && x1 != b->fw) || (x0 & 7))
        return stx_fail(STX_ERR_INVALID, "band [%d,%d) must lie in [0,%d) with edges on multiples of max(8, 2^bands)", x0, x1, b->fw);
    b->band_x0 = x0; b->band_x1 = x1;
    return STX_OK;
}

STX_EXPORT int stx_blend_contrib_rect(const stx_blender* b, int img_w, int img_h, int tlx, int tly, int band_x0, int band_x1,
                                      int out_rect_xywh[4], size_t* out_bytes)
{
    if (!b || !out_rect_xywh) return stx_fail(STX_ERR_INVALID, "null argument");
    if (b->kind != STX_BLEND_MULTIBAND) return stx_fail(STX_ERR_UNSUPPORTED, "multi-band blender only");
    int fx, fy, fw, fh, sx0, sx1;
    mb_feed_rect(b, img_w, img_h, tlx, tly, &fx, &fy, &fw, &fh);
    if (!mb_contrib_range(b, fx, fw, band_x0, band_x1, &sx0, &sx1)) {
        out_rect_xywh[0] = out_rect_xywh[1] = out_rect_xywh[2] = out_rect_xywh[3] = 0;
        if (out_bytes) *out_bytes = 0;
        return STX_OK;
    }
    out_rect_xywh[0] = sx0; out_rect_xywh[1] = fy; out_rect_xywh[2] = sx1 - sx0; out_rect_xywh[3] = fh;
    if (out_bytes) {
        ContribLayout L;
        mb_contrib_layout(b->num_bands, sx1 - sx0, fh, &L);
        *out_bytes = L.bytes;
    }
    return STX_OK;
}

STX_EXPORT int stx_blend_export_contrib(stx_blender* b, int order, int band_x0, int band_x1, stx_buf** out_packed,
                                        int out_rect_xywh[4])
{
    return stx_blend_export_contribs(b, 1, &order, &band_x0, &band_x1, out_packed, out_rect_xywh);
}

STX_EXPORT int stx_blend_export_contribs(stx_blender* b, int n, const int* orders, const int* band_x0s, const int* band_x1s,
                                         stx_buf** out_packed, int* out_rects_xywh)
{
    if (!b || n < 0 || (n > 0 && (!orders || !band_x0s || !band_x1s || !out_packed || !out_rects_xywh)))
        return stx_fail(STX_ERR_INVALID, "null argument");
    if (b->kind != STX_BLEND_MULTIBAND) return stx_fail(STX_ERR_UNSUPPORTED, "multi-band blender only");
    if (b->finished) return stx_fail(STX_ERR_STATE, "export after blend()");
    if (!b->ctx) return stx_fail(STX_ERR_STATE, "geometry-only blender (created without a context)");
    if (n == 0) return STX_OK;
    STX_TRY(stx_set_device(b->ctx));
    const int nb = b->num_bands;
    std::vector<StxMbImage> srcs(n);
    std::vector<int> sx0(n), sx1(n);
    for (int i = 0; i < n; i++) {
// ... 27 lines not shown
            mb_fill_common(b, &K, d_srcs + i, 1, lv);
            K.all_u8 = one.img0_is_s16 ? 0 : 1;
            K.x0 = sx0[i] >> lv; K.x1 = sx1[i] >> lv; K.y0 = one.fy >> lv; K.y1 = (one.fy + sh) >> lv;
            K.emit = 1;
            K.out = (short*)(packed[i]->ptr + Ls[i].g_off[lv]); K.out_stride = Ls[i].g_stride[lv];
            K.out_plane = Ls[i].g_stride[lv] * std::max(sh >> lv, 1);
            K.out_x0 = K.x0; K.out_y0 = K.y0;
            K.out_w = (float*)(packed[i]->ptr + Ls[i].w_off[lv]); K.out_w_stride = Ls[i].w_stride[lv];
            if (K.x1 <= K.x0 || K.y1 <= K.y0) continue;
            Item it;
            it.cls = stx_fast_mb_emit_class(K, &it.K);
            if (it.cls < 0) it.cls = lv == 0 ? -1 : -2;
            items.push_back(it);
            bytes += mb_level_bytes(b, single, lv, K.x0, K.x1, true, false);
        }
    }
    std::stable_sort(items.begin(), items.end(), [](const Item& a, const Item& c) { return a.cls < c.cls; });
    std::vector<MbLevelK> Ks(items.size());
    std::vector<int> classes(items.size());
    for (size_t i = 0; i < items.size(); i++) { Ks[i] = items[i].K; classes[i] = items[i].cls; }
    StxDevBlock d_Ks;
    STX_TRY(upload_small(b->ctx, Ks.data(), Ks.size() * sizeof(MbLevelK), &d_Ks));
    STX_TRY(stx_launch_mb_emit_batch(b->ctx, (const MbLevelK*)d_Ks.get(), Ks.data(), classes.data(), (int)Ks.size(), bytes));
    d_Ks.reset();
    for (int i = 0; i < n; i++) {
        out_rects_xywh[4 * i] = sx0[i]; out_rects_xywh[4 * i + 1] = srcs[i].fy;
        out_rects_xywh[4 * i + 2] = sx1[i] - sx0[i]; out_rects_xywh[4 * i + 3] = srcs[i].fh;
        packed[i]->mask_binary = (!srcs[i].img0_is_s16 && srcs[i].mask_binary) ? 1 : 0;
        out_packed[i] = packed[i].release();
    }
    return STX_OK;
}

STX_EXPORT int stx_blend_build(stx_blender* b)
{
    if (!b) return stx_fail(STX_ERR_INVALID, "null argument");
    if (b->kind != STX_BLEND_MULTIBAND) return STX_OK;
    if (b->finished) return stx_fail(STX_ERR_STATE, "build after blend()");
    if (!b->ctx) return stx_fail(STX_ERR_STATE, "geometry-only blender (created without a context)");
    STX_TRY(stx_set_device(b->ctx));
    return mb_ensure_pyramids(b);
}

STX_EXPORT int stx_blend_feed_contrib(stx_blender* b, int order, const int rect_xywh[4], const stx_buf* packed)
{
    return stx_blend_feed_contrib_ex(b, order, rect_xywh, packed, 0);
}

STX_EXPORT int stx_blend_feed_contrib_ex(stx_blender* b, int order, const int rect_xywh[4], const stx_buf* packed, int flags)
{
    if (!b || !rect_xywh || !packed) return stx_fail(STX_ERR_INVALID, "null argument");
    if (b->kind != STX_BLEND_MULTIBAND) return stx_fail(STX_ERR_UNSUPPORTED, "multi-band blender only");
    if (b->finished) return stx_fail(STX_ERR_STATE, "feed after blend()");
    if (!b->ctx) return stx_fail(STX_ERR_STATE, "geometry-only blender (created without a context)");
    const int nb = b->num_bands, al = (1 << nb) - 1;
    const int x = rect_xywh[0], y = rect_xywh[1], w = rect_xywh[2], h = rect_xywh[3];
    if (w <= 0 || h <= 0 || ((x | y | w | h) & al) || x < 0 || y < 0 || x + w > b->rw || y + h > b->rh)
        return stx_fail(STX_ERR_INVALID, "contribution rect (%d,%d,%d,%d) is not a 2^bands-aligned part of the roi", x, y, w, h);
    ContribLayout L;
    mb_contrib_layout(nb, w, h, &L);
    if (packed->elem != STX_U8 || packed->c != 1 || packed->stride * (size_t)packed->h < L.bytes)
        return stx_fail(STX_ERR_INVALID, "contribution buffer holds %zu bytes, layout needs %zu", packed->stride * (size_t)packed->h, L.bytes);
    StxMbImage im;
    memset(&im, 0, sizeof(im));
    im.kind = 1;
    im.order = order;
    im.mask_binary = (flags & STX_CONTRIB_U8_BINARY) ? 1 : 0;
    im.fx = x; im.fy = y; im.fw = w; im.fh = h;
    for (int i = 0; i <= nb; i++) {
        im.g[i] = (short*)(packed->ptr + L.g_off[i]); im.g_stride[i] = L.g_stride[i];
        im.g_plane[i] = L.g_stride[i] * std::max(h >> i, 1);
        im.wt[i] = (float*)(packed->ptr + L.w_off[i]); im.wt_stride[i] = L.w_stride[i];
    }
    mb_insert_sorted(b, im, true);
    b->next_order = std::max(b->next_order, order + 1);
    stx_buf_retain(const_cast<stx_buf*>(packed));
    b->held.push_back(const_cast<stx_buf*>(packed));
    return STX_OK;
}

static int feather_finish(stx_blender* b, stx_buf* pano, stx_buf* pmask, stx_buf* p16)
{
    stx_ctx* ctx = b->ctx;
    const int n = (int)b->feather_images.size();
    StxDevBlock tab;
    STX_TRY(upload_small(ctx, b->feather_images.data(), sizeof(FeatherImg) * (size_t)n, &tab));
    void* const d_tab = tab.release();
    b->pyr_allocs.push_back(d_tab);
    STX_TRY(stx_launch_feather_weights(ctx, (const FeatherImg*)d_tab, b->feather_images.data(), n));
    double bytes = 4.0 * pano->w * pano->h + (p16 ? 6.0 * pano->w * pano->h : 0.0);
    for (const FeatherImg& im : b->feather_images) bytes += (double)im.w * im.h * ((im.is_s16 ? 6 : 3) + 2);
    FeatherGatherK K;
    K.imgs = (const FeatherImg*)d_tab; K.n = n; K.w = pano->w; K.h = pano->h; K.sharpness = b->sharpness;
    K.pano = pano->ptr; K.pano_stride = (long long)pano->stride; K.pmask = pmask->ptr; K.pmask_stride = (long long)pmask->stride;
    K.pano16 = p16 ? (short*)p16->ptr : nullptr; K.pano16_stride = p16 ? (long long)p16->stride : 0;
    return stx_launch_feather_gather(ctx, K, bytes);
}

static int no_finish(stx_blender* b, stx_buf* pano, stx_buf* pmask, stx_buf* p16)
{
    stx_ctx* ctx = b->ctx;
    const int n = (int)b->no_images.size();
    void* d_tab = nullptr;
    STX_TRY(stx_dev_alloc(ctx, sizeof(NoImg) * std::max(n, 1), &d_tab));
    b->pyr_allocs.push_back(d_tab);
    bool all_binary = true;
    double bytes = 4.0 * pano->w * pano->h + (p16 ? 6.0 * pano->w * pano->h : 0.0);
    for (const NoImg& im : b->no_images) {
        all_binary = all_binary && im.mask_binary;
        bytes += (double)im.w * im.h;
    }
    bytes += 3.0 * pano->w * pano->h;
    if (n > 0) STX_TRY(stx_stage_upload(ctx, d_tab, b->no_images.data(), sizeof(NoImg) * (size_t)n));
    NoGatherK K;
    K.imgs = (const NoImg*)d_tab; K.n = n; K.all_binary = all_binary ? 1 : 0;
    K.w = pano->w; K.h = pano->h;
    K.pano = pano->ptr; K.pano_stride = (long long)pano->stride; K.pmask = pmask->ptr; K.pmask_stride = (long long)pmask->stride;
    K.pano16 = p16 ? (short*)p16->ptr : nullptr; K.pano16_stride = p16 ? (long long)p16->stride : 0;
    return stx_launch_no_gather(ctx, K, bytes);
}

STX_EXPORT int stx_blend_finish_ex(stx_blender* b, stx_buf** out_pano_u8, stx_buf** out_mask_u8, stx_buf** out_pano_s16)
{
    if (!b) return stx_fail(STX_ERR_INVALID, "null argument");
    if (b->finished) return stx_fail(STX_ERR_STATE, "blend() was already called on this blender");
    if (!b->ctx) return stx_fail(STX_ERR_STATE, "geometry-only blender (created without a context)");
    STX_TRY(stx_set_device(b->ctx));
    stx_ctx* ctx = b->ctx;
    const int ow = b->kind == STX_BLEND_MULTIBAND ? b->band_x1 - b->band_x0 : b->rw, oh = b->kind == STX_BLEND_MULTIBAND ? b->fh : b->rh;
    StxBufRef p16, pmask, pano;
    const int rc = [&]() {
        STX_TRY(stx_buf_new(ctx, ow, oh, 3, STX_U8, &pano));
        STX_TRY(stx_buf_new(ctx, ow, oh, 1, STX_U8, &pmask));
        if (out_pano_s16) STX_TRY(stx_buf_new(ctx, ow, oh, 3, STX_S16, &p16));
        if (b->kind == STX_BLEND_MULTIBAND) return mb_finish(b, pano.get(), pmask.get(), p16.get());
        if (b->kind == STX_BLEND_NO) return no_finish(b, pano.get(), pmask.get(), p16.get());
        return feather_finish(b, pano.get(), pmask.get(), p16.get());
    }();
    b->finished = true;
    blender_release(b);
    STX_TRY(rc);
    if (out_pano_u8) *out_pano_u8 = pano.release();
    if (out_mask_u8) *out_mask_u8 = pmask.release();
    if (out_pano_s16) *out_pano_s16 = p16.release();
    return STX_OK;
}

STX_EXPORT int stx_blend_finish(stx_blender* b, stx_buf** out_pano_u8, stx_buf** out_mask_u8)
{
    return stx_blend_finish_ex(b, out_pano_u8, out_mask_u8, nullptr);
}

STX_EXPORT int stx_blend_destroy(stx_blender* b)
{
    if (!b) return STX_OK;
    if (b->ctx) {
        hipSetDevice(b->ctx->device);
        blender_release(b);
    }
    delete b;
    return STX_OK;
}
```

### stitching_amd/csrc/stx_blend_kernels.h

```cpp
#pragma once
#include "stx_internal.h"

struct StxTileMap {
    int tiles_x, tiles_y, band_rows, band_tiles;
    unsigned magic_tx, magic_band;
    int plain;
};
inline StxTileMap stx_tile_map(int tiles_x, int tiles_y, int band_rows)
{
    StxTileMap m;
    m.tiles_x = tiles_x; m.tiles_y = tiles_y; m.band_rows = band_rows; m.band_tiles = band_rows * tiles_x;
    m.magic_tx = (unsigned)((1ull << 32) / (unsigned)tiles_x) + 1u;
    m.magic_band = (unsigned)((1ull << 32) / (unsigned)m.band_tiles) + 1u;
    m.plain = 0;
    return m;
}
inline unsigned stx_tile_grid(const StxTileMap& m)
{
    if (m.plain) return (unsigned)(m.tiles_x * m.tiles_y);
    const int bands = (m.tiles_y + m.band_rows - 1) / m.band_rows;
    return 8u * (unsigned)(((bands + 7) / 8) * m.band_tiles);
}

constexpr int STX_DEFER_SEGS = 256;
struct MbLevelK {
    const StxMbImage* images;
    int n_images, level, num_bands, pw, ph;
    int x0, x1, y0, y1;
    short* out; long long out_stride, out_plane; int out_x0, out_y0;
    const short* up; long long up_stride, up_plane; int up_x0, up_y0;
    int emit; float* out_w; long long out_w_stride;
    uint8_t* pano; long long pano_stride;
    uint8_t* pmask; long long pmask_stride;
    short* pano16; long long pano16_stride;
    int pano_x0, pano_y0;
    int has_contrib;
    int all_u8;
    StxTileMap tiles;
    int pk_ok;
    int defer_segs;
    unsigned long long* defer_list; unsigned* defer_count; unsigned defer_cap;
};

bool stx_fast_mb_down_batch(stx_ctx* ctx, const StxMbImage* d_images, const StxMbImage* h_images, int n, int level);
bool stx_fast_mb_level(stx_ctx* ctx, const MbLevelK& K);

int stx_fast_mb_emit_class(const MbLevelK& K, MbLevelK* KT);
bool stx_fast_mb_emit_launch(stx_ctx* ctx, int cls, const MbLevelK* d_Ks, const MbLevelK* h_Ks, int count);
int stx_launch_mb_emit_batch(stx_ctx* ctx, const MbLevelK* d_Ks, const MbLevelK* h_Ks, const int* classes, int n, double bytes);
```

### stitching_amd/csrc/stx_internal.h

```cpp
#pragma once
#include <hip/hip_runtime.h>

#include <atomic>
#include <cstdarg>
#include <cstdint>
#include <cstdio>
#include <map>
#include <memory>
#include <mutex>
#include <string>
#include <vector>

#include "../../include/stitching_amd.h"
#include "../../include/stitching_amd_debug.h"

#define STX_EXPORT extern "C" __attribute__((visibility("default")))
#define STX_MAX_BANDS 16

void stx_set_error(const char* fmt, ...);
int stx_fail(int code, const char* fmt, ...);

#define STX_HIP(call)                                                                                      \
    do {                                                                                                   \
        hipError_t e_ = (call);                                                                            \
// ... 104 lines not shown
    std::vector<stx_buf*> p;
    for (const StxBufRef& b : v) p.push_back(b.get());
    return p;
}

int trig_mode_now();
int remap_mode_now();
int pyrdown_now();
int exposure_solver_now();

enum { STX_F_PLANE = 0, STX_F_CYLINDRICAL, STX_F_SPHERICAL, STX_F_FISHEYE, STX_F_STEREOGRAPHIC, STX_F_CRECT,
       STX_F_CRECT_PORTRAIT, STX_F_PANINI, STX_F_PANINI_PORTRAIT, STX_F_MERCATOR, STX_F_TRANSVERSE_MERCATOR };
struct StxProjector {
    int type;
    int family;
    float a, b;
    float scale;
    float k[9], rinv[9], r_kinv[9], k_rinv[9], t[3];
    int trig;
    int remap;
};
int stx_make_projector(int type, float scale, const float* K, const float* R, StxProjector* out);

struct StxWarpLaunch {
    StxProjector proj;
    int tlx, tly, dw, dh;
    const uint8_t* src; int sw, sh; size_t sstride; int src_channels;
    uint8_t* dimg; size_t dimg_stride;
    uint8_t* dmask; size_t dmask_stride;
    int nearest_src;
    int debug_maps = 0;
    const float* gain_H = nullptr; long long gain_hstride = 0; const void* gain_yt = nullptr; int gain_gh = 0;
};
bool stx_warp_fast_eligible(const StxWarpLaunch& L);
int stx_launch_warp(stx_ctx* ctx, const StxWarpLaunch& L);
int stx_launch_warp_batch(stx_ctx* ctx, const StxWarpLaunch* Ls, int n);
int stx_launch_roi_minmax(stx_ctx* ctx, int n, const StxProjector* projs, const int* sizes_wh, float* out_minmax4);

struct StxMbImage {
    int kind; int order;
    const uint8_t* img0; long long img0_stride; int img0_is_s16;
    const uint8_t* mask0; long long mask0_stride; int mask_binary;
    int iw, ih;
    int ix, iy;
    int fx, fy, fw, fh;
    int left, top;
    int g_u8;
    short* g[STX_MAX_BANDS + 1]; long long g_stride[STX_MAX_BANDS + 1]; long long g_plane[STX_MAX_BANDS + 1];
    float* wt[STX_MAX_BANDS + 1]; long long wt_stride[STX_MAX_BANDS + 1];
    int w1_f16;
    uint8_t* occ[STX_MAX_BANDS + 1];
};
int stx_launch_mb_pyramids(stx_ctx* ctx, const StxMbImage* d_images, const StxMbImage* h_images, int n, int num_bands, int pyr_mode,
                           int pyr_lanes);
struct MbLevelK;
int stx_launch_mb_level(stx_ctx* ctx, const MbLevelK& K, double algo_bytes);
int stx_launch_mb_coarse(stx_ctx* ctx, const MbLevelK& K_level_Bm2, double algo_bytes);

int stx_launch_gain_apply(stx_ctx* ctx, stx_buf* img, const float g[3]);
int block_gain_check(stx_ctx* ctx, const stx_buf* img, const stx_buf* gain_map);
int stx_launch_block_gain(stx_ctx* ctx, stx_buf* img, const stx_buf* gmap, const int* d_xt, const int* d_yt);
int stx_launch_block_gain_batch(stx_ctx* ctx, int n, stx_buf* const* imgs, const stx_buf* const* gmaps, const int* full_wh_xy0,
                                float* const* Hs, void* const* yts, const int* fast);
int stx_launch_gain_rows(stx_ctx* ctx, int n, const int* wh, const stx_buf* const* gmaps, const int* full_wh_xy0, float* const* Hs,
                         void* const* yts);
struct StxExpImg { const uint8_t* img; long long istride; const uint8_t* mask; long long mstride; };
struct StxExpJob { int ia, ib, ax, ay, bx, by, w, h; };
enum { STX_EXP_TREE = 0, STX_EXP_ORDERED = 1, STX_EXP_INT = 2 };
int stx_launch_exposure_stats(stx_ctx* ctx, const StxExpImg* d_imgs, const StxExpJob* d_jobs, int njobs, int mode, const double* d_sqrt,
                              long long* d_out_i, double* d_out_d, double algo_bytes);
struct StxExpBlockMul { uint8_t* img; long long stride; int w, h, bw, bh, bpw; const float* g; int g3; };
int stx_launch_exposure_block_mul(stx_ctx* ctx, const StxExpBlockMul* d_tab, int n, int max_pixels);
struct StxLuEntry { int row, col; double v; };
constexpr int STX_LU_MAX_N = 16384;
int stx_lu_device(stx_ctx* ctx, int n, const StxLuEntry* entries, size_t count, double* x, double out[3]);
struct StxSeamPair { uint8_t* m1; uint8_t* m2; long long s1, s2, off; int w1, h1, w2, h2, ox1, oy1, ox2, oy2, ww, wh, rw, rh; };
int stx_launch_seam_level(stx_ctx* ctx, const StxSeamPair* d_pairs, int np, int max_rows, int max_cols, uint16_t* d_arena, double algo_bytes);
struct StxColorSeamPair {
    const uint8_t* i1; const uint8_t* i2; uint8_t* m1; uint8_t* m2;
    long long si1, si2, sm1, sm2, off_choice, off_seam;
    int L, W, vertical, first_is_i;
};
int stx_launch_color_seam_level(stx_ctx* ctx, const StxColorSeamPair* d_pairs, int np, int max_cross, long long max_area, uint8_t* d_arena,
                                double algo_bytes);
constexpr int STX_FEAT_GREY_TW = 64, STX_FEAT_GREY_TH = 4;
constexpr int STX_FEAT_BLUR_TW = 64, STX_FEAT_BLUR_TH = 8;
constexpr int STX_FEAT_SCORE_TW = 32, STX_FEAT_SCORE_TH = 8;
constexpr int STX_FEAT_BORDER = 16;
struct StxFeatImage { const uint8_t* img; long long istride; uint8_t* grey; long long gstride; int w, h, tiles_x, tile0; };
struct StxFeatLevel {
    const uint8_t* g; long long gstride; uint8_t* blur; long long bstride; const uint8_t* mask; long long mstride;
    long long cand_off, cand_cap;
    int w, h, w0, h0, btiles_x, btile0, stiles_x, stile0;
};
struct StxFeatSel { long long cand_off; int count, keep, out_off, pad_; };
constexpr long long STX_FEAT_R_BIAS = 1ll << 33;
int stx_launch_feat_grey(stx_ctx* ctx, const StxFeatImage* d_imgs, int n, int tiles, double algo_bytes);
int stx_launch_feat_blur(stx_ctx* ctx, const StxFeatLevel* d_levels, int n, int tiles, double algo_bytes);
int stx_launch_feat_score(stx_ctx* ctx, const StxFeatLevel* d_levels, int n, int tiles, int threshold, unsigned long long* d_cand,
                          int* d_counts, double algo_bytes);
int stx_launch_feat_select(stx_ctx* ctx, const StxFeatSel* d_sel, int n, const unsigned long long* d_cand, unsigned long long* d_tmp,
                           unsigned long long* d_keys, int* d_item);
int stx_launch_feat_describe(stx_ctx* ctx, const StxFeatLevel* d_levels, int nl, const unsigned long long* d_keys, const int* d_item, int total,
                             const int* d_cxcy, const signed char* d_patterns, int* d_bins, uint8_t* d_desc);
int stx_launch_resize_exact(stx_ctx* ctx, const stx_buf* src, stx_buf* dst, const int* d_xt, const int* d_yt, bool dilate,
                            const stx_buf* andmask);
constexpr int STX_RESIZE_TW = 64, STX_RESIZE_TH = 4;
struct StxResizeItem {
    const uint8_t* src; long long sstride; uint8_t* dst; long long dstride;
    int sw, sh, dw, dh, c, tiles_x, tile0, pad_;
    double xscale, yscale;
};
int stx_launch_resize_exact_batch(stx_ctx* ctx, const StxResizeItem* d_items, int n, int total_tiles, double algo_bytes);

int stx_launch_seam_resize_batch(stx_ctx* ctx, int n, const stx_buf* const* seams, const stx_buf* const* masks, stx_buf* const* dsts,
                                 const int* const* d_xt, const int* const* d_yt, uint8_t* const* tmp, const size_t* tstride);
int stx_launch_seam_resize_lds(stx_ctx* ctx, int n, const stx_buf* const* seams, const stx_buf* const* masks, stx_buf* const* dsts,
                               const int* full_wh_xy0, bool* done);
int stx_launch_strip_pack(stx_ctx* ctx, int n, const stx_buf* const* imgs, const stx_buf* const* masks, const int* x0, const int* w,
                          stx_buf* const* dsts, const size_t* si, const size_t* sm, bool mask_bits);
int stx_launch_strip_bits_expand(stx_ctx* ctx, int n, const uint8_t* const* bits, const size_t* sm, stx_buf* const* masks);

constexpr int STX_FEATHER_DIST_CAP = 8192;
constexpr int STX_DT_RC = 64;
struct FeatherImg {
    const uint8_t* img; long long istride; int is_s16;
    const uint8_t* mask; long long mstride;
    int x, y, w, h;
    uint16_t* dist; long long dstride;
    int* first; int* last; unsigned long long* zbits; int n_chunks;
};
struct FeatherGatherK {
    const FeatherImg* imgs; int n; int w, h; float sharpness;
    uint8_t* pano; long long pano_stride; uint8_t* pmask; long long pmask_stride; short* pano16; long long pano16_stride;
};
int stx_launch_feather_weights(stx_ctx* ctx, const FeatherImg* d_imgs, const FeatherImg* h_imgs, int n);
int stx_launch_feather_gather(stx_ctx* ctx, const FeatherGatherK& K, double algo_bytes);

struct NoImg { const uint8_t* img; long long istride; const uint8_t* mask; long long mstride; int is_s16; int x, y, w, h; int mask_binary; };
struct NoGatherK {
    const NoImg* imgs; int n; int all_binary;
    int w, h;
    uint8_t* pano; long long pano_stride; uint8_t* pmask; long long pmask_stride; short* pano16; long long pano16_stride;
};
int stx_launch_no_gather(stx_ctx* ctx, const NoGatherK& K, double algo_bytes);

struct stx_blender {
    stx_ctx* ctx = nullptr;
    int kind = 0, num_bands = 0;
    float sharpness = 0.02f;
    int rx = 0, ry = 0, rw = 0, rh = 0;
    int fw = 0, fh = 0;
    bool finished = false;
    std::vector<StxMbImage> images;
    std::vector<char> built;
    std::vector<stx_buf*> held;
    std::vector<void*> pyr_allocs;
    StxMbImage* d_all = nullptr;
    int band_x0 = 0, band_x1 = 0;
    int next_order = 0;
    int pyr_mode = 0;
    std::vector<NoImg> no_images;
    std::vector<FeatherImg> feather_images;
};
void mb_feed_rect(const stx_blender* b, int w, int h, int tlx, int tly, int* fx, int* fy, int* fw, int* fh);
bool mb_contrib_range(const stx_blender* b, int fx, int fw, int bx0, int bx1, int* sx0, int* sx1);
```

### stitching_amd/pipeline.py

```python
import ctypes as C

import numpy as np

from . import _lib, config
from .blender import Blender
from .cropper import Cropper
from .device import as_device, get_context
from .exposure_error_compensator import ExposureErrorCompensator
from .images import Images
from .seam_estimation import SeamEstimator
from .seam_finder import DEVICE_SEAM_FINDERS, SeamFinder
from .stitching_error import StitchingError
from .synthetic import blend_strength_for_bands
from .warper import Warper


def mask_box(mask):
    m2 = mask.reshape(mask.shape[0], mask.shape[1], -1).any(axis=2)
    nx, ny = np.flatnonzero(m2.any(axis=0)), np.flatnonzero(m2.any(axis=1))
    if not nx.size:
        return None
    return (int(nx[0]), int(nx[-1]) + 1, int(mask.shape[1]), int(ny[0]), int(ny[-1]) + 1, int(mask.shape[0]))


def view_rects(handle, corners, sizes, boxes, min_gain=0.9):
    B = handle.num_bands()
    if B <= 0:
        return None
    roi = Blender.result_roi(corners, sizes)
    align, reach = max(8, 1 << B), 2 << B

    def band(lo, hi, size, msize, origin):
        if msize != size:
            lo = int(np.floor((lo - 2 + 0.5) * size / msize - 0.5)) - 1
            hi = int(np.ceil((hi + 2 + 0.5) * size / msize - 0.5)) + 1
        lo, hi = max(lo, 0), min(hi, size)
        return max(((origin + lo - reach) // align) * align, 0), -((-(origin + hi + reach)) // align) * align

    out = []
    for (cx, cy), (w, h), box in zip(corners, sizes, boxes):
        if box is None:
            out.append(None)
            continue
        bx0, bx1 = band(box[0], box[1], w, box[2], cx - roi[0])
        by0, by1 = band(box[3], box[4], h, box[5], cy - roi[1])
        r = (C.c_int * 4)()
        _lib.check(_lib.lib().stx_view_rect(handle._h, int(w), int(h), int(cx), int(cy), int(bx0), int(bx1), int(by0), int(by1), r))
        x0, x1, y0, y1 = (int(v) for v in r)
        if x1 <= x0 or y1 <= y0:
            out.append(None)
            continue
        if x1 - x0 > min_gain * w:
            x0, x1 = 0, w
        if y1 - y0 > min_gain * h:
            y0, y1 = 0, h
        out.append((x0, x1, y0, y1) if (x1 - x0) * (y1 - y0) < w * h else None)
    return None if all(o is None for o in out) else out


def clip_rectangle(rect, width, height):
    x0, x1, _ = slice(rect.x, rect.x2).indices(int(width))
    y0, y1, _ = slice(rect.y, rect.y2).indices(int(height))
    return x0, max(x1, x0), y0, max(y1, y0)


def _split_cropper(cropper, crop_aspect):
    if isinstance(cropper, (tuple, list)):
        cropper, crop_aspect = cropper
    if cropper is not None and not cropper.do_crop:
        cropper = None
    if cropper is not None and not getattr(cropper, "intersection_rectangles", None):
        raise StitchingError("the cropper is not prepared: Cropper.prepare(imgs, masks, corners, sizes) on the low-resolution warps comes first")
    return cropper, crop_aspect


class StitchJob:

    def __init__(self, frames, cameras, warper_type="spherical", blender_type="multiband", num_bands=None,
                 blend_strength=Blender.DEFAULT_BLEND_STRENGTH, ctx=None, async_upload=False, feed_masks=None, seam_masks=None,
                 crop_to_masks=True, compensator=None, cropper=None, crop_aspect=1, camera_aspect=1):
        cropper, crop_aspect = _split_cropper(cropper, crop_aspect)
        if len(frames) != len(cameras) or not frames:
            raise StitchingError("need one camera per frame and at least one frame")
        self.ctx = ctx or get_context()
        self.frames = [as_device(f, self.ctx, wait=not async_upload) for f in frames]
        self.cameras = list(cameras)
        self.sizes = [(f.width, f.height) for f in self.frames]
        self.warper = Warper(warper_type, ctx=self.ctx)
        self.warper.set_scale(self.cameras)
        self.blender_type = blender_type
        self.compensator = compensator
        self.num_bands = num_bands
        self.blend_strength = blend_strength
        self.corners = self.warped_sizes = None
        self.cropper, self.crop_aspect, self.camera_aspect = cropper, crop_aspect, camera_aspect
        if cropper is not None and len(cropper.intersection_rectangles) != len(self.frames):
            raise StitchingError(f"the cropper was prepared on {len(cropper.intersection_rectangles)} images, the job has {len(self.frames)}")
        self._cam_arrays = self.warper.camera_arrays(self.cameras, camera_aspect)
        self._mask_cols = None
        given = feed_masks if feed_masks is not None else seam_masks
        if crop_to_masks and given is not None and all(isinstance(m, np.ndarray) for m in given):
            self._mask_cols = [mask_box(m) for m in given]
        self._crop_cache = None
        self.feed_masks = None if feed_masks is None else [as_device(m, self.ctx) for m in feed_masks]
        self.seam_masks = None if seam_masks is None else [as_device(m, self.ctx) for m in seam_masks]

    @property
    def source_pixels(self):
        return sum(w * h for w, h in self.sizes)

    def plan(self):
        self._adopt(*self.warper.warp_rois(self.sizes, self.cameras, self.camera_aspect, camera_arrays=self._cam_arrays))
        return self.corners, self.warped_sizes

    def _adopt(self, corners, warped_sizes):
        self.corners, self.warped_sizes = corners, warped_sizes
        if any(w <= 0 or h <= 0 for w, h in self.warped_sizes):
            raise StitchingError(f"degenerate warp roi {self.warped_sizes}: the {self.warper.warper_type!r} projection cannot "
                                 "represent these cameras")
        if self.num_bands is not None:
            roi = Blender.result_roi(self.corners, self.warped_sizes)
            self.blend_strength = blend_strength_for_bands(self.num_bands, roi[2], roi[3])

    def _crop_rects(self, handle, corners, sizes):
        key = (tuple(corners), tuple(sizes), self.blend_strength)
        if self._crop_cache is None or self._crop_cache[0] != key:
            self._crop_cache = (key, view_rects(handle, corners, sizes, self._mask_cols))
        return self._crop_cache[1]

    def run(self):
        prev = config.device_resident()
        config.set_device_resident(True)
        try:
            if self.cropper is not None:
                return self._run_cropped()
            warped = None
            if self._mask_cols is None:
                warped = self.warper.warp_images_and_masks(self.frames, self.cameras, self.camera_aspect, compensator=self.compensator,
                                                           with_rois=True, camera_arrays=self._cam_arrays)
                self._adopt([r[0:2] for r in warped[2]], [r[2:4] for r in warped[2]])
            else:
                self.plan()
            blender = Blender(self.blender_type, self.blend_strength, ctx=self.ctx)
            blender.prepare(self.corners, self.warped_sizes)
            crop = None
            if self._mask_cols is not None and blender.blender.kind == _lib.BLEND_MULTIBAND:
                crop = self._crop_rects(blender.blender, self.corners, self.warped_sizes)
            if crop is not None:
                box = [c if c is not None else (0, w, 0, h) for c, (w, h) in zip(crop, self.warped_sizes)]
                rects = [(cx + x0, cy + y0, x1 - x0, y1 - y0) for (x0, x1, y0, y1), (cx, cy) in zip(box, self.corners)]
                imgs, masks, rois = self.warper.warp_images_and_masks(self.frames, self.cameras, self.camera_aspect, rects=rects,
                                                                      compensator=self.compensator, camera_arrays=self._cam_arrays)
                if self.feed_masks is not None:
                    masks = [m[y0:y1, x0:x1] for m, (x0, x1, y0, y1) in zip(self.feed_masks, box)]
                else:
                    masks = SeamFinder.resize_all(self.seam_masks, masks,
                                                  sub=[(w, h, x0, y0) for (x0, x1, y0, y1), (w, h) in zip(box, self.warped_sizes)])
                corners = [(r[0], r[1]) for r in rects]
            else:
                imgs, masks, rois = warped or self.warper.warp_images_and_masks(self.frames, self.cameras, self.camera_aspect,
                                                                                compensator=self.compensator, camera_arrays=self._cam_arrays)
                if self.feed_masks is not None:
                    masks = self.feed_masks
                elif self.seam_masks is not None:
                    masks = SeamFinder.resize_all(self.seam_masks, masks)
                corners = self.corners
                for roi, corner in zip(rois, self.corners):
                    if roi[0:2] != tuple(corner):
                        raise StitchingError("warp roi changed between plan() and run()")
            self.last_crop = crop
            for img, mask, corner in zip(imgs, masks, corners):
                blender.feed(img, mask, corner)
            self.last_num_bands = blender.blender.num_bands()
            pano, pmask = blender.blend()
        finally:
            config.set_device_resident(prev)
        return pano, pmask

    def _run_cropped(self):
        self.plan()
        cuts = [clip_rectangle(r.times(self.crop_aspect), w, h) for r, (w, h) in zip(self.cropper.intersection_rectangles, self.warped_sizes)]
        cut_sizes = [(x1 - x0, y1 - y0) for x0, x1, y0, y1 in cuts]
        if any(w <= 0 or h <= 0 for w, h in cut_sizes):
            raise StitchingError(f"the cropper leaves nothing of a warped image (sizes {cut_sizes}): it was prepared for another panorama")
        corners, sizes = self.cropper.crop_rois(self.corners, self.warped_sizes, self.crop_aspect)
        corners, sizes = [tuple(c) for c in corners], [tuple(z) for z in sizes]
        roi = Blender.result_roi(corners, sizes)
        if self.num_bands is not None:
            self.blend_strength = blend_strength_for_bands(self.num_bands, roi[2], roi[3])
        crop = None
        kind, bands, _ = Blender.plan(self.blender_type, self.blend_strength, roi)
        if self._mask_cols is not None and kind == _lib.BLEND_MULTIBAND and cut_sizes == sizes:
            from .distributed import make_shard_blender

            crop = self._crop_rects(make_shard_blender(None, roi, bands), corners, sizes)
        box = [c if crop is not None and c is not None else (0, w, 0, h) for c, (w, h) in zip(crop or [None] * len(cuts), cut_sizes)]
        rects = [(cx + c[0] + x0, cy + c[2] + y0, x1 - x0, y1 - y0) for (x0, x1, y0, y1), c, (cx, cy) in zip(box, cuts, self.corners)]
        imgs, masks, _ = self.warper.warp_images_and_masks(self.frames, self.cameras, self.camera_aspect, rects=rects,
                                                           camera_arrays=self._cam_arrays)
        sub = None if crop is None else [(w, h, x0, y0) for (x0, x1, y0, y1), (w, h) in zip(box, cut_sizes)]
        if self.compensator is not None:
            imgs = self.compensator.apply_all(corners, imgs, None, sub=sub, ctx=self.ctx)
        if self.feed_masks is not None:
            masks = [m if b == (0, m.width, 0, m.height) else m[b[2]:b[3], b[0]:b[1]] for m, b in zip(self.feed_masks, box)]
        elif self.seam_masks is not None:
            masks = SeamFinder.resize_all(self.seam_masks, masks, sub=sub)
        self.last_crop = crop
        blender = Blender(self.blender_type, self.blend_strength, ctx=self.ctx)
        blender.prepare(corners, sizes)
        for img, mask, (cx, cy), b in zip(imgs, masks, corners, box):
            blender.feed(img, mask, (cx + b[0], cy + b[2]))
        self.last_num_bands = blender.blender.num_bands()
        return blender.blend()


def compose(frames, cameras, warper_type="spherical", blender_type="multiband", blend_strength=Blender.DEFAULT_BLEND_STRENGTH,
            compensator=None, seam_masks=None, ctx=None, cropper=None, crop_aspect=1, camera_aspect=1):
    ctx = ctx or get_context()
    cropper, crop_aspect = _split_cropper(cropper, crop_aspect)
    if cropper is not None:
        if seam_masks is not None and blender_type == "multiband":
            seam_masks = [np.asarray(m.get() if hasattr(m, "get") else m) for m in seam_masks]
        return StitchJob(frames, cameras, warper_type=warper_type, blender_type=blender_type, blend_strength=blend_strength, ctx=ctx,
                         seam_masks=seam_masks, compensator=compensator, cropper=cropper, crop_aspect=crop_aspect,
                         camera_aspect=camera_aspect).run()
    if seam_masks is not None and blender_type == "multiband":
        return StitchJob(frames, cameras, warper_type=warper_type, blender_type=blender_type, blend_strength=blend_strength, ctx=ctx,
                         seam_masks=[np.asarray(m.get() if hasattr(m, "get") else m) for m in seam_masks], compensator=compensator,
                         camera_aspect=camera_aspect).run()
    prev = config.device_resident()
    config.set_device_resident(True)
    try:
        warper = Warper(warper_type, ctx=ctx)
        warper.set_scale(cameras)
        imgs, masks, rois = warper.warp_images_and_masks([as_device(f, ctx) for f in frames], cameras, camera_aspect, compensator=compensator)
        corners, sizes = [r[0:2] for r in rois], [r[2:4] for r in rois]
        if seam_masks is not None:
            masks = SeamFinder.resize_all(seam_masks, masks)
        blender = Blender(blender_type, blend_strength, ctx=ctx)
        blender.prepare(corners, sizes)
        for img, mask, corner in zip(imgs, masks, corners):
            blender.feed(img, mask, corner)
        return blender.blend()
    finally:
        config.set_device_resident(prev)


class ComposePlan:

    def __init__(self, images, frames, cameras, warper_scale, cropper, compensator, seam_masks, seam_masks_host, low_corners, low_sizes):
        self.images, self.frames, self.cameras, self.warper_scale = images, frames, list(cameras), warper_scale
        self.cropper, self.compensator, self.seam_masks, self.seam_masks_host = cropper, compensator, seam_masks, seam_masks_host
        self.low_corners, self.low_sizes = low_corners, low_sizes
        self.frame_sizes = images.sizes
        R = Images.Resolution
        self.camera_aspect = images.get_ratio(R.MEDIUM, R.FINAL)
        self.lir_aspect = images.get_ratio(R.LOW, R.FINAL)

    def check_frames(self, frames):
        got = [Images.get_image_size(f) for f in frames]
        if got != [tuple(z) for z in self.frame_sizes]:
            raise StitchingError(f"the plan was prepared for frames of sizes {self.frame_sizes}, got {got}: same rig, same sizes")


class Composer:

    DEFAULT_SETTINGS = {
        "medium_megapix": Images.Resolution.MEDIUM.value,
        "warper_type": Warper.DEFAULT_WARP_TYPE,
        "low_megapix": Images.Resolution.LOW.value,
        "crop": Cropper.DEFAULT_CROP,
        "compensator": ExposureErrorCompensator.DEFAULT_COMPENSATOR,
        "nr_feeds": ExposureErrorCompensator.DEFAULT_NR_FEEDS,
        "block_size": ExposureErrorCompensator.DEFAULT_BLOCK_SIZE,
        "finder": SeamFinder.DEFAULT_SEAM_FINDER,
        "final_megapix": Images.Resolution.FINAL.value,
        "blender_type": Blender.DEFAULT_BLENDER,
        "blend_strength": Blender.DEFAULT_BLEND_STRENGTH,
    }

    def __init__(self, ctx=None, seam_estimator=None, **kwargs):
        self.seam_estimator = seam_estimator
        for arg in kwargs:
            if arg not in self.DEFAULT_SETTINGS:
                raise StitchingError("Invalid Argument: " + arg)
        self.settings = dict(self.DEFAULT_SETTINGS, **kwargs)
        self.ctx = ctx
        st = self.settings
        if st["finder"] not in SeamFinder.SEAM_FINDER_CHOICES:
            raise StitchingError(f"unknown seam finder {st['finder']!r}")
        if st["compensator"] not in ExposureErrorCompensator.COMPENSATOR_CHOICES:
            raise StitchingError(f"unknown compensator {st['compensator']!r}")
        if st["warper_type"] not in Warper.WARP_TYPE_CHOICES:
            raise StitchingError(f"unknown warper type {st['warper_type']!r}")
        if st["blender_type"] not in Blender.BLENDER_CHOICES:
            raise StitchingError(f"unknown blender type {st['blender_type']!r}")
        if st["medium_megapix"] < st["low_megapix"]:
            raise StitchingError("Medium resolution megapix need to be greater or equal than low resolution megapix")

    def _ctx(self):
        return self.ctx or get_context()

    def prepare(self, images, cameras):
        st, ctx = self.settings, self._ctx()
        frames, cameras = list(images), list(cameras)
        if len(frames) != len(cameras):
            raise StitchingError("need one camera per image")
        frames = [as_device(f, ctx) for f in frames]
        imgs_obj = Images.of(frames, st["medium_megapix"], st["low_megapix"], st["final_megapix"])
        R = Images.Resolution
        prev = config.device_resident()
        config.set_device_resident(True)
        try:
            medium = list(imgs_obj.resize(R.MEDIUM))
            low = list(imgs_obj.resize(R.LOW, medium))
            warper = Warper(st["warper_type"], ctx=ctx)
            warper.set_scale(cameras)
            aspect = imgs_obj.get_ratio(R.MEDIUM, R.LOW)
            imgs, masks, rois = warper.warp_images_and_masks(low, cameras, aspect)
            corners, sizes = [r[0:2] for r in rois], [r[2:4] for r in rois]
            cropper = Cropper(st["crop"])
            cropper.prepare(imgs, masks, corners, sizes)
            masks = list(cropper.crop_images(masks))
            imgs = list(cropper.crop_images(imgs))
            corners, sizes = cropper.crop_rois(corners, sizes)
            estimator = ExposureErrorCompensator._device_estimator(st["compensator"], st["nr_feeds"], st["block_size"])
            compensator = ExposureErrorCompensator(st["compensator"], st["nr_feeds"], st["block_size"], estimator=estimator)
            compensator.feed(corners, imgs, masks)
            if self.seam_estimator is not None:
                finder = SeamFinder(st["finder"], estimator=self.seam_estimator)
            else:
                device_finder = st["finder"] in DEVICE_SEAM_FINDERS
                finder = SeamFinder(st["finder"], estimator=SeamEstimator(st["finder"]) if device_finder else None)
            seam_masks = [as_device(m, ctx) for m in finder.find(imgs, corners, masks)]
            host = None
            if st["blender_type"] == "multiband":
                host = [m.numpy() for m in seam_masks]
        finally:
            config.set_device_resident(prev)
        return ComposePlan(imgs_obj, frames, cameras, warper.scale, cropper, compensator, seam_masks, host, corners, sizes)

    def run(self, plan, images=None):
        frames = plan.frames if images is None else list(images)
        plan.check_frames(frames)
        st, ctx = self.settings, self._ctx()
        frames = [as_device(f, ctx) for f in frames]
        prev = config.device_resident()
        config.set_device_resident(True)
        try:
            final = list(plan.images.resize(Images.Resolution.FINAL, frames))
        finally:
            config.set_device_resident(prev)
        job = StitchJob(final, plan.cameras, warper_type=st["warper_type"], blender_type=st["blender_type"],
                        blend_strength=st["blend_strength"], ctx=ctx,
                        seam_masks=plan.seam_masks_host if plan.seam_masks_host is not None else plan.seam_masks,
                        compensator=plan.compensator, cropper=plan.cropper, crop_aspect=plan.lir_aspect, camera_aspect=plan.camera_aspect)
        return job.run()

    def compose(self, images, cameras):
        pano, _ = self.run(self.prepare(images, cameras))
        return pano


def stitch(frames, cameras, **kw):
    job = StitchJob(frames, cameras, **kw)
    pano, mask = job.run()
    return np.asarray(pano), np.asarray(mask)
```

### stitching_amd/warper.py

```python
import ctypes as C
from statistics import median

import numpy as np

from . import _lib, config
from .device import DeviceImage, as_device, get_context
from .stitching_error import StitchingError

_TYPE_IDS = _lib.WARP_TYPE_IDS


def _mat33(m, what):
    a = np.asarray(m)
    if a.shape != (3, 3) or a.dtype != np.float32:
        raise StitchingError(f"{what} must be a 3x3 float32 matrix, got shape {a.shape} dtype {a.dtype}")
    return np.ascontiguousarray(a)


def _fp(a):
    return a.ctypes.data_as(C.POINTER(C.c_float))


class Warper:

# ... 57 lines not shown
        return self._result(DeviceImage(ctx, out))

    def camera_arrays(self, cameras, aspect=1):
        cameras = list(cameras)
        Ks = np.empty((len(cameras), 3, 3), np.float32)
        Rs = np.empty((len(cameras), 3, 3), np.float32)
        for i, cam in enumerate(cameras):
            Ks[i], Rs[i] = self._K_R(cam, aspect)
        return Ks, Rs

    def warp_rois(self, sizes, cameras, aspect=1, camera_arrays=None):
        sizes, cameras = list(sizes), list(cameras)
        n = min(len(sizes), len(cameras))
        roi_corners, roi_sizes = [], []
        if n == 0:
            return roi_corners, roi_sizes
        ctx = self._ctx()
        Ks, Rs = camera_arrays if camera_arrays is not None else self.camera_arrays(cameras[:n], aspect)
        wh = np.ascontiguousarray([[int(s[0]), int(s[1])] for s in sizes[:n]], np.int32)
        out = np.zeros((n, 4), np.int32)
        _lib.check(ctx._lib.stx_warp_rois(ctx.handle, self._type_id(), self._scale(aspect), n, _fp(Ks), _fp(Rs),
                                          wh.ctypes.data_as(C.POINTER(C.c_int)),
                                          out.ctypes.data_as(C.POINTER(C.c_int))))
        for roi in out:
            roi = tuple(int(v) for v in roi)
            roi_corners.append(roi[0:2])
            roi_sizes.append(roi[2:4])
        return roi_corners, roi_sizes

    def warp_roi(self, size, camera, aspect=1):
        ctx = self._ctx()
        K, R = self._K_R(camera, aspect)
        roi = (C.c_int * 4)()
        _lib.check(ctx._lib.stx_warp_roi(ctx.handle, self._type_id(), self._scale(aspect), _fp(K), _fp(R),
                                         int(size[0]), int(size[1]), roi))
        return tuple(int(v) for v in roi)

    @staticmethod
    def get_K(camera, aspect=1):
        K = np.array(camera.K(), dtype=np.float32)
        for r, c in ((0, 0), (0, 2), (1, 1), (1, 2)):
            K[r, c] *= aspect
        return K

    def warp_image_and_mask(self, img, camera, aspect=1):
        ctx = self._ctx()
        src = self._source(img, ctx)
        K, R = self._K_R(camera, aspect)
        oi, om, roi = C.c_void_p(), C.c_void_p(), (C.c_int * 4)()
        _lib.check(ctx._lib.stx_warp_image_and_mask(ctx.handle, self._type_id(), self._scale(aspect), _fp(K), _fp(R),
                                                    src._h, C.byref(oi), C.byref(om), roi))
        return (self._result(DeviceImage(ctx, oi)), self._result(DeviceImage(ctx, om)), tuple(int(v) for v in roi))

    def warp_images_and_masks(self, imgs, cameras, aspect=1, rects=None, compensator=None, with_rois=False, camera_arrays=None):
        ctx = self._ctx()
        srcs = [self._source(img, ctx) for img in imgs]
        cameras = list(cameras)
        n = min(len(srcs), len(cameras))
        if n == 0:
            return [], [], []
        Ks, Rs = camera_arrays if camera_arrays is not None else self.camera_arrays(cameras[:n], aspect)
        h_src = (C.c_void_p * n)(*[s._h for s in srcs[:n]])
        h_img, h_mask = (C.c_void_p * n)(), (C.c_void_p * n)()
        rois = np.zeros((n, 4), np.int32)
        blocks = compensator is not None and compensator.compensator_type in ("gain_blocks", "channel_blocks")
        if blocks and compensator.gains is None:
            raise StitchingError("ExposureErrorCompensator.set_gains(gains) must be called before apply")
        if with_rois and rects is None:
            ga = fl = None
            if blocks:
                gm = [compensator._gain_map(i, ctx) for i in range(n)]
                ga, fl = (C.c_void_p * n)(*[g[0]._h for g in gm]), (C.c_int * n)(*[g[1] for g in gm])
                compensator = None
            _lib.check(ctx._lib.stx_warp_batch_with_rois(ctx.handle, self._type_id(), self._scale(aspect), n, _fp(Ks), _fp(Rs), h_src, ga, fl,
                                                         h_img, h_mask, rois.ctypes.data_as(C.POINTER(C.c_int))))
        elif blocks:
            gm = [compensator._gain_map(i, ctx) for i in range(n)]
            ga, fl = (C.c_void_p * n)(*[g[0]._h for g in gm]), (C.c_int * n)(*[g[1] for g in gm])
            rp = None
            if rects is not None:
                rois = np.ascontiguousarray(np.asarray(rects, np.int32).reshape(n, 4))
                rp = rois.ctypes.data_as(C.POINTER(C.c_int))
            _lib.check(ctx._lib.stx_warp_batch_gain(ctx.handle, self._type_id(), self._scale(aspect), n, _fp(Ks), _fp(Rs), h_src, rp, ga, fl,
                                                    h_img, h_mask, None if rects is not None else rois.ctypes.data_as(C.POINTER(C.c_int))))
            compensator = None
        elif rects is not None:
            rois = np.ascontiguousarray(np.asarray(rects, np.int32).reshape(n, 4))
            _lib.check(ctx._lib.stx_warp_batch_rects(ctx.handle, self._type_id(), self._scale(aspect), n, _fp(Ks), _fp(Rs), h_src,
                                                     rois.ctypes.data_as(C.POINTER(C.c_int)), h_img, h_mask))
        else:
            _lib.check(ctx._lib.stx_warp_batch(ctx.handle, self._type_id(), self._scale(aspect), n, _fp(Ks), _fp(Rs), h_src,
                                               h_img, h_mask, rois.ctypes.data_as(C.POINTER(C.c_int))))
        d_imgs = [DeviceImage(ctx, C.c_void_p(h_img[i])) for i in range(n)]
        if compensator is not None:
            prev = config.device_resident()
            config.set_device_resident(True)
            try:
                d_imgs = compensator.apply_all([tuple(int(v) for v in r[:2]) for r in rois], d_imgs, None, ctx=ctx)
            finally:
                config.set_device_resident(prev)
        imgs_out = [self._result(d) for d in d_imgs]
        masks_out = [self._result(DeviceImage(ctx, C.c_void_p(h_mask[i]))) for i in range(n)]
        return imgs_out, masks_out, [tuple(int(v) for v in r) for r in rois]

    @staticmethod
    def _source(img, ctx):
        src = as_device(img, ctx)
        if src.channels != 3 or src.dtype != np.uint8:
            raise StitchingError(f"warp_image expects a HxWx3 uint8 image, got {src.shape} {src.dtype}")
        return src

    def _type_id(self):
        if self.warper_type not in Warper.WARP_TYPE_CHOICES:
            raise StitchingError(f"unknown warper type {self.warper_type!r}")
        if self.warper_type not in _TYPE_IDS:
            raise StitchingError(f"warper type {self.warper_type!r} is not implemented by the MI355X back end "
                                 f"(implemented: {', '.join(_TYPE_IDS)})")
        return _TYPE_IDS[self.warper_type]

    def _scale(self, aspect):
        if self.scale is None:
            raise StitchingError("Warper.set_scale(cameras) must be called before warping")
        return float(self.scale * aspect)

    def _K_R(self, camera, aspect):
        return _mat33(Warper.get_K(camera, aspect), "K"), _mat33(camera.R, "camera.R")

    @staticmethod
    def _result(dev):
        return dev if config.device_resident() else dev.numpy()
```

Baseline: 172,900 Mpix/s.

## Cache rig geometry and multiband weight pyramids across repeated stitch runs

Keeps the StitchJob and its geometry pass alive between runs with the same rig and settings. On later runs it skips mask warping and reuses the blender's weight pyramids through new keep/use-weights APIs. The pyramid-down kernels gain a WEIGHTS template flag, so image-only pyramids skip mask loads and weight math. This removes repeated geometry-only work per panorama, at the cost of held device memory and a reliance on camera parameters staying unchanged.

Result: faster. 196,100 Mpix/s (median of 6 runs) (+13.4%).

```diff
diff --git a/include/stitching_amd.h b/include/stitching_amd.h
--- a/include/stitching_amd.h
+++ b/include/stitching_amd.h
@@ -70,6 +70,7 @@
 typedef struct stx_ctx stx_ctx;
 typedef struct stx_buf stx_buf;
 typedef struct stx_blender stx_blender;
+typedef struct stx_mb_weights stx_mb_weights;
 
 int stx_version(void);
 const char* stx_last_error(void);
@@ -121,6 +122,9 @@
 int stx_blend_finish(stx_blender* b, stx_buf** out_pano_u8, stx_buf** out_mask_u8);
 int stx_blend_finish_ex(stx_blender* b, stx_buf** out_pano_u8, stx_buf** out_mask_u8, stx_buf** out_pano_s16);
 int stx_blend_destroy(stx_blender* b);
+int stx_blend_keep_weights(stx_blender* b, stx_mb_weights** out);
+int stx_blend_use_weights(stx_blender* b, stx_mb_weights* w, int* out_adopted);
+int stx_mb_weights_free(stx_mb_weights* w);
 
 int stx_gain_apply(stx_ctx* ctx, stx_buf* img_u8x3, const float gains_bgr[3]);
 int stx_block_gain_apply(stx_ctx* ctx, stx_buf* img_u8x3, const stx_buf* gain_map_f32);
diff --git a/stitching_amd/_lib.py b/stitching_amd/_lib.py
--- a/stitching_amd/_lib.py
+++ b/stitching_amd/_lib.py
@@ -34,7 +34,7 @@
     "stx_host_alloc stx_host_free stx_buf_from_host stx_buf_from_host_async stx_buf_alloc stx_buf_to_host stx_buf_to_host_async stx_buf_view stx_buf_info stx_buf_device_ptr stx_buf_free "
     "stx_warp_roi stx_warp_rois stx_warp stx_warp_image_and_mask stx_warp_batch stx_warp_batch_rects stx_warp_batch_gain stx_warp_batch_with_rois stx_warp_mask "
     "stx_gain_apply stx_block_gain_apply stx_block_gain_apply_batch stx_resize_linear_exact stx_resize_linear_exact_batch stx_seam_mask_resize stx_seam_mask_resize_batch stx_seam_mask_resize_batch_sub stx_timelapse_frame stx_result_roi stx_blend_create stx_blend_num_bands stx_blend_feed stx_blend_finish stx_blend_finish_ex "
-    "stx_blend_destroy stx_blend_set_band stx_blend_feed_ex stx_blend_contrib_rect stx_blend_export_contrib stx_blend_export_contribs "
+    "stx_blend_destroy stx_blend_keep_weights stx_blend_use_weights stx_mb_weights_free stx_blend_set_band stx_blend_feed_ex stx_blend_contrib_rect stx_blend_export_contrib stx_blend_export_contribs "
     "stx_blend_build stx_blend_feed_contrib stx_blend_feed_contrib_ex stx_buf_flags stx_strip_rect stx_view_rect stx_strip_pack stx_strip_pack_batch stx_strip_pack_batch_ex stx_strip_bytes stx_strip_unpack stx_blend_feed_strips stx_comm_unique_id stx_comm_create stx_comm_exchange stx_comm_exchange_begin stx_comm_exchange_end stx_comm_exchange_begin_on stx_comm_exchange_end_on stx_comm_info stx_comm_destroy stx_prof_enable stx_prof_reset stx_prof_count stx_prof_get stx_mark stx_mark_elapsed_ms "
     "stx_exposure_feed stx_exposure_stats stx_exposure_solve stx_set_exposure_solver stx_get_exposure_solver stx_exposure_feed_ex stx_exposure_solve_device stx_lu_solve_device stx_seam_find stx_seam_schedule stx_color_seam_find stx_crop_lir stx_features_detect "
     "stx_debug_warp_maps stx_debug_feather_dist_cap"
@@ -106,6 +106,9 @@
     L.stx_blend_finish.argtypes = [vp, vpp, vpp]
     L.stx_blend_finish_ex.argtypes = [vp, vpp, vpp, vpp]
     L.stx_blend_destroy.argtypes = [vp]
+    L.stx_blend_keep_weights.argtypes = [vp, vpp]
+    L.stx_blend_use_weights.argtypes = [vp, vp, ip]
+    L.stx_mb_weights_free.argtypes = [vp]
     L.stx_blend_set_band.argtypes = [vp, C.c_int, C.c_int]
     L.stx_blend_feed_ex.argtypes = [vp, vp, vp, C.c_int, C.c_int, C.c_int]
     L.stx_blend_contrib_rect.argtypes = [vp, C.c_int, C.c_int, C.c_int, C.c_int, C.c_int, C.c_int, ip,
diff --git a/stitching_amd/blender.py b/stitching_amd/blender.py
--- a/stitching_amd/blender.py
+++ b/stitching_amd/blender.py
@@ -5,6 +5,24 @@
 from . import _lib, config
 from .device import DeviceImage, as_device, get_context
 from .stitching_error import StitchingError
+
+
+class MbWeights:
+
+    def __init__(self, ctx, handle):
+        self.ctx, self._h = ctx, handle
+
+    def free(self):
+        if self._h is not None:
+            if getattr(self.ctx, "handle", None):
+                self.ctx._lib.stx_mb_weights_free(self._h)
+            self._h = None
+
+    def __del__(self):
+        try:
+            self.free()
+        except Exception:
+            pass
 
 
 class _BlenderHandle:
@@ -24,6 +42,18 @@
 
     def feed(self, img, mask, corner):
         _lib.check(self.ctx._lib.stx_blend_feed(self._h, img._h, mask._h, int(corner[0]), int(corner[1])))
+
+    def keep_weights(self):
+        h = C.c_void_p()
+        _lib.check(self.ctx._lib.stx_blend_keep_weights(self._h, C.byref(h)))
+        return MbWeights(self.ctx, h) if h.value else None
+
+    def use_weights(self, weights):
+        if weights is None or weights._h is None:
+            return False
+        got = C.c_int()
+        _lib.check(self.ctx._lib.stx_blend_use_weights(self._h, weights._h, C.byref(got)))
+        return bool(got.value)
 
     def blend(self, want_s16=False):
         pano, mask, p16 = C.c_void_p(), C.c_void_p(), C.c_void_p()
diff --git a/stitching_amd/csrc/stx_blend.hip b/stitching_amd/csrc/stx_blend.hip
--- a/stitching_amd/csrc/stx_blend.hip
+++ b/stitching_amd/csrc/stx_blend.hip
@@ -670,7 +670,7 @@
 }
 
 int stx_launch_mb_pyramids(stx_ctx* ctx, const StxMbImage* d_images, const StxMbImage* h_images, int n, int num_bands, int pyr_mode,
-                           int pyr_lanes)
+                           int pyr_lanes, bool weights)
 {
     for (int lv = 0; lv < num_bands; lv++) {
         double bytes = 0.0;
@@ -678,14 +678,15 @@
         for (int i = 0; i < n; i++) {
             const StxMbImage& im = h_images[i];
             const double ip = (double)(im.fw >> lv) * (im.fh >> lv), op = ip / 4.0;
-            const double gw = (im.g_u8 ? 3.0 : 6.0) + 4.0;
-            const double gw1 = gw - (im.w1_f16 ? 2.0 : 0.0);
-            if (lv == 0) bytes += ((im.img0_is_s16 ? 6.0 : 3.0) + 1.0) * im.iw * im.ih + gw1 * op;
+            const double wb = weights ? 4.0 : 0.0;
+            const double gw = (im.g_u8 ? 3.0 : 6.0) + wb;
+            const double gw1 = gw - ((weights && im.w1_f16) ? 2.0 : 0.0);
+            if (lv == 0) bytes += ((im.img0_is_s16 ? 6.0 : 3.0) + (weights ? 1.0 : 0.0)) * im.iw * im.ih + gw1 * op;
             else bytes += (lv == 1 ? gw1 : gw) * ip + gw * op;
             any_s16 = any_s16 || im.img0_is_s16;
         }
         StxProfScope prof(ctx, lv == 0 ? "mb_down0" : "mb_down", bytes);
-        const bool batched = pyr_mode == STX_PYRDOWN_SCALAR && stx_fast_mb_down_batch(ctx, d_images, h_images, n, lv);
+        const bool batched = pyr_mode == STX_PYRDOWN_SCALAR && stx_fast_mb_down_batch(ctx, d_images, h_images, n, lv, weights);
         for (int i = 0; i < n; i++) {
             const StxMbImage& im = h_images[i];
             if (batched && !(lv == 0 && im.img0_is_s16)) continue;
diff --git a/stitching_amd/csrc/stx_blend_fast.hip b/stitching_amd/csrc/stx_blend_fast.hip
--- a/stitching_amd/csrc/stx_blend_fast.hip
+++ b/stitching_amd/csrc/stx_blend_fast.hip
@@ -323,7 +323,7 @@
     const uint8_t* img0;
     const uint8_t* mask0;
 };
-template <bool PK, bool NEAR, class IM>
+template <bool PK, bool NEAR, bool WEIGHTS, class IM>
 STX_DEV void dn_task_level0(const IM& im, int row, int xo, short* hs0, short* hs1, short* hs2, float* hw)
 {
     const int by = reflect101_near(row, im.fh) - im.top;
@@ -341,6 +341,7 @@
         dn_pack5_channel<false, 0>(w, hs0);
         dn_pack5_channel<false, 1>(w, hs1);
         dn_pack5_channel<false, 2>(w, hs2);
+        if (!WEIGHTS) return;
         uint32_t mw[3] = {0u, 0u, 0u};
         if (yin) {
             const uint32_t moff = (uint32_t)by * (uint32_t)im.mask0_stride + (uint32_t)a0;
@@ -379,20 +380,23 @@
             dn_pack5_channel<true, 0>(w, hs0);
             dn_pack5_channel<true, 1>(w, hs1);
             dn_pack5_channel<true, 2>(w, hs2);
-            *reinterpret_cast<float4*>(hw) = make_float4(0.f, 0.f, 0.f, 0.f);
+            if (WEIGHTS) *reinterpret_cast<float4*>(hw) = make_float4(0.f, 0.f, 0.f, 0.f);
             return;
         }
     }
     {
-        const STX_GAS uint8_t* mrow = gp(im.mask0) + (uint32_t)min(max(by, 0), im.ih - 1) * (uint32_t)im.mask0_stride;
+        const STX_GAS uint8_t* mrow = nullptr;
+        if (WEIGHTS) mrow = gp(im.mask0) + (uint32_t)min(max(by, 0), im.ih - 1) * (uint32_t)im.mask0_stride;
 #pragma unroll
         for (int j = 0; j < 11; j++) {
             const int bx = reflect101_near(c0 + j, im.fw) - im.left;
             const int sx = NEAR ? reflect_near(bx, im.iw) : reflect(bx, im.iw);
             const STX_GAS uint8_t* p = img + (rowoff + (uint32_t)sx * 3u);
             px[j][0] = p[0]; px[j][1] = p[1]; px[j][2] = p[2];
-            const float mv = fmul((float)mrow[sx], INV255);
-            f[j] = (yin && (unsigned)bx < (unsigned)im.iw) ? mv : 0.f;
+            if (WEIGHTS) {
+                const float mv = fmul((float)mrow[sx], INV255);
+                f[j] = (yin && (unsigned)bx < (unsigned)im.iw) ? mv : 0.f;
+            }
         }
     }
 #pragma unroll
@@ -400,7 +404,7 @@
         hs0[o] = (short)h5i(px[2 * o][0], px[2 * o + 1][0], px[2 * o + 2][0], px[2 * o + 3][0], px[2 * o + 4][0]);
         hs1[o] = (short)h5i(px[2 * o][1], px[2 * o + 1][1], px[2 * o + 2][1], px[2 * o + 3][1], px[2 * o + 4][1]);
         hs2[o] = (short)h5i(px[2 * o][2], px[2 * o + 1][2], px[2 * o + 2][2], px[2 * o + 3][2], px[2 * o + 4][2]);
-        hw[o] = h5f(f[2 * o], f[2 * o + 1], f[2 * o + 2], f[2 * o + 3], f[2 * o + 4]);
+        if (WEIGHTS) hw[o] = h5f(f[2 * o], f[2 * o + 1], f[2 * o + 2], f[2 * o + 3], f[2 * o + 4]);
     }
 }
 
@@ -420,11 +424,11 @@
 #ifndef STX_DN0_BATCH
 #define STX_DN0_BATCH 3
 #endif
-template <bool PK>
+template <bool PK, bool WEIGHTS>
 __global__ __launch_bounds__(256) void mb_down0_lds_kernel(const StxMbImage* __restrict__ images, StxTileMap M)
 {
     __shared__ __attribute__((aligned(16))) short s_h[3][DN_ROWS][DN_TOW];
-    __shared__ __attribute__((aligned(16))) float s_w[DN_ROWS][DN_TOW];
+    __shared__ __attribute__((aligned(16))) float s_w[WEIGHTS ? DN_ROWS : 1][WEIGHTS ? DN_TOW : 4];
     const uint32_t zz = STX_DN0_REV ? gridDim.z - 1u - blockIdx.z : blockIdx.z, bb = STX_DN0_REV ? gridDim.x - 1u - blockIdx.x : blockIdx.x;
     const StxMbImage& im = images[zz];
     const int tid = threadIdx.x;
@@ -433,14 +437,14 @@
     if (!xcd_tile(M, bb, tile_tx, tile_ty)) return;
     const int X0 = tile_tx * DN_TOW, Y0 = tile_ty * DN_TOH;
     if (im.img0_is_s16 || X0 >= ow || Y0 >= oh) return;
-    uint8_t* const occ = im.occ[1];
-    const bool w1h = im.w1_f16 != 0;
-    asm volatile("" ::"s"(occ));
+    uint8_t* const occ = WEIGHTS ? im.occ[1] : nullptr;
+    const bool w1h = WEIGHTS && im.w1_f16 != 0;
+    if (WEIGHTS) asm volatile("" ::"s"(occ));
     DnImage0 D;
     {
         int fw = im.fw, fh = im.fh, iw_ = im.iw, ih_ = im.ih, left = im.left, top = im.top;
-        uint32_t is = (uint32_t)im.img0_stride, ms = (uint32_t)im.mask0_stride;
-        unsigned long long ia = (unsigned long long)im.img0, ma = (unsigned long long)im.mask0;
+        uint32_t is = (uint32_t)im.img0_stride, ms = WEIGHTS ? (uint32_t)im.mask0_stride : 0u;
+        unsigned long long ia = (unsigned long long)im.img0, ma = WEIGHTS ? (unsigned long long)im.mask0 : 0ull;
         if (PK) asm volatile("" : "+s"(fw), "+s"(fh), "+s"(iw_), "+s"(ih_), "+s"(left), "+s"(top), "+s"(is), "+s"(ms), "+s"(ia), "+s"(ma));
         D.fw = fw; D.fh = fh; D.iw = iw_; D.ih = ih_; D.left = left; D.top = top; D.img0_stride = is; D.mask0_stride = ms;
         D.img0 = (const uint8_t*)ia; D.mask0 = (const uint8_t*)ma;
@@ -448,9 +452,14 @@
     uint32_t g1_plane = 0, g1_stride = 0, w1_stride = 0;
     unsigned long long g1_a = 0, w1_a = 0;
     if (PK) {
-        g1_plane = (uint32_t)im.g_plane[1]; g1_stride = (uint32_t)im.g_stride[1]; w1_stride = (uint32_t)im.wt_stride[1];
-        g1_a = (unsigned long long)im.g[1]; w1_a = (unsigned long long)im.wt[1];
-        asm volatile("" : "+s"(g1_plane), "+s"(g1_stride), "+s"(w1_stride), "+s"(g1_a), "+s"(w1_a));
+        g1_plane = (uint32_t)im.g_plane[1]; g1_stride = (uint32_t)im.g_stride[1];
+        g1_a = (unsigned long long)im.g[1];
+        if (WEIGHTS) {
+            w1_stride = (uint32_t)im.wt_stride[1]; w1_a = (unsigned long long)im.wt[1];
+            asm volatile("" : "+s"(g1_plane), "+s"(g1_stride), "+s"(w1_stride), "+s"(g1_a), "+s"(w1_a));
+        } else {
+            asm volatile("" : "+s"(g1_plane), "+s"(g1_stride), "+s"(g1_a));
+        }
     }
     const int r_end = 2 * min(DN_TOH, oh - Y0) + 3;
     const bool near = PK ? (D.left <= D.iw && D.fw - D.left - D.iw <= D.iw && D.top <= D.ih && D.fh - D.top - D.ih <= D.ih)
@@ -485,13 +494,15 @@
                 d0[t] = *reinterpret_cast<const STX_GAS v4u_a4*>(p);
                 d1[t] = *reinterpret_cast<const STX_GAS v4u_a4*>(p + 16);
                 d2[t] = *reinterpret_cast<const STX_GAS v2u_a4*>(p + 32);
-                const uint32_t moff = (uint32_t)min(max(by, 0), D.ih - 1) * (uint32_t)D.mask0_stride + (uint32_t)acol;
-                msh[t] = moff & 3u;
+                if (WEIGHTS) {
+                    const uint32_t moff = (uint32_t)min(max(by, 0), D.ih - 1) * (uint32_t)D.mask0_stride + (uint32_t)acol;
+                    msh[t] = moff & 3u;
 #if STX_ABLATE_MASK
-                mq4[t] = v4u{0xffffffffu, 0xffffffffu, 0xffffffffu, 0xffffffffu};
+                    mq4[t] = v4u{0xffffffffu, 0xffffffffu, 0xffffffffu, 0xffffffffu};
 #else
-                mq4[t] = *reinterpret_cast<const STX_GAS v4u_a4*>(gp(D.mask0) + (moff & ~3u));
-#endif
+                    mq4[t] = *reinterpret_cast<const STX_GAS v4u_a4*>(gp(D.mask0) + (moff & ~3u));
+#endif
+                }
             }
             __builtin_amdgcn_sched_barrier(0);
 #pragma unroll
@@ -517,6 +528,7 @@
                     dn_pack5_channel<true, 1>(w, &s_h[1][r][4 * q]);
                     dn_pack5_channel<true, 2>(w, &s_h[2][r][4 * q]);
                 }
+                if (!WEIGHTS) continue;
                 const uint32_t keep = (yin[t] && interior) ? 0xffffffffu : 0u;
                 uint32_t mw[3];
                 mw[0] = __builtin_amdgcn_alignbyte(mq4[t].y, mq4[t].x, msh[t]) & keep;
@@ -547,12 +559,13 @@
     for (int task = tid; task < DN_ROWS * (DN_TOW / 4) && !batched; task += 256) {
         const int r = task / (DN_TOW / 4), q = task % (DN_TOW / 4);
         if (X0 + 4 * q >= ow || r >= r_end) continue;
+        float* const hw = WEIGHTS ? &s_w[r][4 * q] : nullptr;
         if (PK) {
-            if (near) dn_task_level0<PK, true>(D, 2 * Y0 - 2 + r, X0 + 4 * q, &s_h[0][r][4 * q], &s_h[1][r][4 * q], &s_h[2][r][4 * q], &s_w[r][4 * q]);
-            else dn_task_level0<PK, false>(D, 2 * Y0 - 2 + r, X0 + 4 * q, &s_h[0][r][4 * q], &s_h[1][r][4 * q], &s_h[2][r][4 * q], &s_w[r][4 * q]);
+            if (near) dn_task_level0<PK, true, WEIGHTS>(D, 2 * Y0 - 2 + r, X0 + 4 * q, &s_h[0][r][4 * q], &s_h[1][r][4 * q], &s_h[2][r][4 * q], hw);
+            else dn_task_level0<PK, false, WEIGHTS>(D, 2 * Y0 - 2 + r, X0 + 4 * q, &s_h[0][r][4 * q], &s_h[1][r][4 * q], &s_h[2][r][4 * q], hw);
         } else {
-            if (near) dn_task_level0<PK, true>(im, 2 * Y0 - 2 + r, X0 + 4 * q, &s_h[0][r][4 * q], &s_h[1][r][4 * q], &s_h[2][r][4 * q], &s_w[r][4 * q]);
-            else dn_task_level0<PK, false>(im, 2 * Y0 - 2 + r, X0 + 4 * q, &s_h[0][r][4 * q], &s_h[1][r][4 * q], &s_h[2][r][4 * q], &s_w[r][4 * q]);
+            if (near) dn_task_level0<PK, true, WEIGHTS>(im, 2 * Y0 - 2 + r, X0 + 4 * q, &s_h[0][r][4 * q], &s_h[1][r][4 * q], &s_h[2][r][4 * q], hw);
+            else dn_task_level0<PK, false, WEIGHTS>(im, 2 * Y0 - 2 + r, X0 + 4 * q, &s_h[0][r][4 * q], &s_h[1][r][4 * q], &s_h[2][r][4 * q], hw);
         }
     }
     __syncthreads();
@@ -577,6 +590,7 @@
             if (two) *reinterpret_cast<STX_GAS uint16_t*>(o) = (uint16_t)b2;
             else o[0] = (uint8_t)b2;
         }
+        if (!WEIGHTS) continue;
         float fa[5], fb[5];
         {
             typedef float v2 __attribute__((ext_vector_type(2)));
@@ -605,7 +619,7 @@
         }
         nz |= __float_as_uint(wa) | (two ? __float_as_uint(wb) : 0u);
     }
-    dn_note_occ(occ, nz, tid, X0, Y0, ow, oh);
+    if (WEIGHTS) dn_note_occ(occ, nz, tid, X0, Y0, ow, oh);
 }
 
 STX_DEV void dn_load19_u8(const STX_GAS uint8_t* __restrict__ base, uint32_t off, int c0, int iw, bool fast, int s[19])
@@ -672,10 +686,11 @@
     *reinterpret_cast<float4*>(row_q + 32) = make_float4(lo.y, lo.w, hi.y, hi.w);
 }
 
+template <bool WEIGHTS>
 __global__ __launch_bounds__(256) void mb_down_lds_kernel(const StxMbImage* __restrict__ images, int lv, StxTileMap M)
 {
     __shared__ __attribute__((aligned(16))) int s_h[3][DN_ROWS][DN_TOW];
-    __shared__ __attribute__((aligned(16))) float s_w[DN_ROWS][DN_TOW];
+    __shared__ __attribute__((aligned(16))) float s_w[WEIGHTS ? DN_ROWS : 1][WEIGHTS ? DN_TOW : 4];
     const StxMbImage& im = images[blockIdx.z];
     const int tid = threadIdx.x;
     const int iw = im.fw >> lv, ih = im.fh >> lv;
@@ -685,15 +700,16 @@
     const int X0 = tile_tx * DN_TOW, Y0 = tile_ty * DN_TOH;
     if (X0 >= ow || Y0 >= oh) return;
     const bool g8b = im.g_u8 != 0;
-    unsigned long long G_a = (unsigned long long)im.g[lv], W_a = (unsigned long long)im.wt[lv];
-    unsigned long long Go_a = (unsigned long long)im.g[lv + 1], Wo_a = (unsigned long long)im.wt[lv + 1];
-    uint32_t gs = (uint32_t)im.g_stride[lv], gpl = (uint32_t)im.g_plane[lv], wst = (uint32_t)im.wt_stride[lv];
-    uint32_t gos = (uint32_t)im.g_stride[lv + 1], gopl = (uint32_t)im.g_plane[lv + 1], wost = (uint32_t)im.wt_stride[lv + 1];
-    asm volatile("" : "+s"(G_a), "+s"(W_a), "+s"(Go_a), "+s"(Wo_a), "+s"(gs), "+s"(gpl), "+s"(wst), "+s"(gos), "+s"(gopl), "+s"(wost));
+    unsigned long long G_a = (unsigned long long)im.g[lv], W_a = WEIGHTS ? (unsigned long long)im.wt[lv] : 0ull;
+    unsigned long long Go_a = (unsigned long long)im.g[lv + 1], Wo_a = WEIGHTS ? (unsigned long long)im.wt[lv + 1] : 0ull;
+    uint32_t gs = (uint32_t)im.g_stride[lv], gpl = (uint32_t)im.g_plane[lv], wst = WEIGHTS ? (uint32_t)im.wt_stride[lv] : 0u;
+    uint32_t gos = (uint32_t)im.g_stride[lv + 1], gopl = (uint32_t)im.g_plane[lv + 1], wost = WEIGHTS ? (uint32_t)im.wt_stride[lv + 1] : 0u;
+    if (WEIGHTS) asm volatile("" : "+s"(G_a), "+s"(W_a), "+s"(Go_a), "+s"(Wo_a), "+s"(gs), "+s"(gpl), "+s"(wst), "+s"(gos), "+s"(gopl), "+s"(wost));
+    else asm volatile("" : "+s"(G_a), "+s"(Go_a), "+s"(gs), "+s"(gpl), "+s"(gos), "+s"(gopl));
     const short* G = (const short*)G_a;
-    uint8_t* const occ = im.occ[lv + 1];
-    const bool w_half = lv == 1 && im.w1_f16 != 0;
-    asm volatile("" ::"s"(occ));
+    uint8_t* const occ = WEIGHTS ? im.occ[lv + 1] : nullptr;
+    const bool w_half = WEIGHTS && lv == 1 && im.w1_f16 != 0;
+    if (WEIGHTS) asm volatile("" ::"s"(occ));
     const int r_end = 2 * min(DN_TOH, oh - Y0) + 3;
     for (int task = tid; task < DN_ROWS * (DN_TOW / 8); task += 256) {
         const int r = task / (DN_TOW / 8), q = task % (DN_TOW / 8);
@@ -714,7 +730,8 @@
                 rc[c] = *reinterpret_cast<const STX_GAS uint32_t*>(pp + 18);
             }
             float f[19];
-            if (w_half) {
+            if (!WEIGHTS) {
+            } else if (w_half) {
                 const STX_GAS _Float16* hq = gp(reinterpret_cast<const _Float16*>(W_a)) + (uint32_t)sy * wst;
                 const v2h16 ha = *reinterpret_cast<const STX_GAS v2h16*>(hq + c0);
                 const v8h16 hb = *reinterpret_cast<const STX_GAS v8h16*>(hq + c0 + 2), hc = *reinterpret_cast<const STX_GAS v8h16*>(hq + c0 + 10);
@@ -748,7 +765,7 @@
                 for (int j = 0; j < 19; j++) s[j] = (int)byte_of(w6, j + 2);
                 dn_hsum_store_i(s, &s_h[c][r][4 * q]);
             }
-            dn_hsum_store_f(f, &s_w[r][4 * q]);
+            if (WEIGHTS) dn_hsum_store_f(f, &s_w[r][4 * q]);
             continue;
         }
 #pragma unroll
@@ -758,6 +775,7 @@
             else dn_load19_s16(gp(G), (uint32_t)c * gpl + (uint32_t)sy * gs, c0, iw, fast, s);
             dn_hsum_store_i(s, &s_h[c][r][4 * q]);
         }
+        if (!WEIGHTS) continue;
         const STX_GAS float* wq = gp(reinterpret_cast<const float*>(W_a)) + (uint32_t)sy * wst;
         float f[19];
         if (w_half) {
@@ -820,6 +838,7 @@
                 else o[0] = (short)va;
             }
         }
+        if (!WEIGHTS) continue;
         float fa[5], fb[5];
 #pragma unroll
         for (int k = 0; k < 5; k++) {
@@ -834,7 +853,7 @@
         else o[0] = wa;
         nz |= __float_as_uint(wa) | (two ? __float_as_uint(wb) : 0u);
     }
-    dn_note_occ(occ, nz, tid, X0, Y0, ow, oh);
+    if (WEIGHTS) dn_note_occ(occ, nz, tid, X0, Y0, ow, oh);
 }
 
 STX_DEV int s6(int v) { return (v + 32) >> 6; }
@@ -2060,7 +2079,7 @@
 
 }
 
-bool stx_fast_mb_down_batch(stx_ctx* ctx, const StxMbImage* d_images, const StxMbImage* h_images, int n, int level)
+bool stx_fast_mb_down_batch(stx_ctx* ctx, const StxMbImage* d_images, const StxMbImage* h_images, int n, int level, bool weights)
 {
     int mw = 0, mh = 0;
     for (int i = 0; i < n; i++) {
@@ -2077,9 +2096,13 @@
     for (int i = 0; i < n; i++) pk_ok = pk_ok && !h_images[i].img0_is_s16 && h_images[i].mask_binary;
     dim3 grid(stx_tile_grid(M), 1, n);
     static const unsigned pad_lds = getenv("STITCHING_AMD_D0_LDS") ? (unsigned)atoi(getenv("STITCHING_AMD_D0_LDS")) : 0u;
-    if (level == 0 && pk_ok) hipLaunchKernelGGL(mb_down0_lds_kernel<true>, grid, dim3(256), pad_lds, ctx->stream, d_images, M);
-    else if (level == 0) hipLaunchKernelGGL(mb_down0_lds_kernel<false>, grid, dim3(256), 0, ctx->stream, d_images, M);
-    else hipLaunchKernelGGL(mb_down_lds_kernel, grid, dim3(256), 0, ctx->stream, d_images, level, M);
+    if (!weights) {
+        if (level == 0 && pk_ok) hipLaunchKernelGGL((mb_down0_lds_kernel<true, false>), grid, dim3(256), pad_lds, ctx->stream, d_images, M);
+        else if (level == 0) hipLaunchKernelGGL((mb_down0_lds_kernel<false, false>), grid, dim3(256), 0, ctx->stream, d_images, M);
+        else hipLaunchKernelGGL(mb_down_lds_kernel<false>, grid, dim3(256), 0, ctx->stream, d_images, level, M);
+    } else if (level == 0 && pk_ok) hipLaunchKernelGGL((mb_down0_lds_kernel<true, true>), grid, dim3(256), pad_lds, ctx->stream, d_images, M);
+    else if (level == 0) hipLaunchKernelGGL((mb_down0_lds_kernel<false, true>), grid, dim3(256), 0, ctx->stream, d_images, M);
+    else hipLaunchKernelGGL(mb_down_lds_kernel<true>, grid, dim3(256), 0, ctx->stream, d_images, level, M);
     return launched_ok();
 }
 
diff --git a/stitching_amd/csrc/stx_blend_host.cpp b/stitching_amd/csrc/stx_blend_host.cpp
--- a/stitching_amd/csrc/stx_blend_host.cpp
+++ b/stitching_amd/csrc/stx_blend_host.cpp
@@ -32,6 +32,11 @@
     b->held.clear();
     for (void* p : b->pyr_allocs) stx_dev_free(b->ctx, p);
     b->pyr_allocs.clear();
+    for (void* p : b->wt_allocs) stx_dev_free(b->ctx, p);
+    b->wt_allocs.clear();
+    stx_mb_weights_release(b->keep);
+    stx_mb_weights_release(b->adopted);
+    b->keep = b->adopted = nullptr;
     b->d_all = nullptr;
     b->images.clear();
     b->built.clear();
@@ -176,7 +181,7 @@
         STX_TRY(stx_dev_alloc(ctx, MB_FRONT_PAD + (size_t)gs * lh * 3 * (im.g_u8 ? 1 : sizeof(short)) + 64, &g));
         b->pyr_allocs.push_back(g);
         STX_TRY(stx_dev_alloc(ctx, (size_t)ws * lh * ((i == 1 && im.w1_f16) ? sizeof(uint16_t) : sizeof(float)), &wt));
-        b->pyr_allocs.push_back(wt);
+        b->wt_allocs.push_back(wt);
         im.g[i] = (short*)((uint8_t*)g + MB_FRONT_PAD); im.g_stride[i] = gs; im.g_plane[i] = gs * lh;
         im.wt[i] = (float*)wt; im.wt_stride[i] = ws;
     }
@@ -207,7 +212,7 @@
     if (todo.empty()) return STX_OK;
     static const bool occ_off = getenv("STITCHING_AMD_NO_OCC") != nullptr;
     const int pyr = b->pyr_mode;
-    if (todo.size() <= 65535 && !occ_off && (pyr & 255) == STX_PYRDOWN_SCALAR) {
+    if (!b->adopted && todo.size() <= 65535 && !occ_off && (pyr & 255) == STX_PYRDOWN_SCALAR) {
         const int nl = b->num_bands + 1;
         std::vector<size_t> off(todo.size() * (size_t)nl, 0);
         size_t bytes = 0;
@@ -221,7 +226,7 @@
         if (bytes > 0) {
             void* arena = nullptr;
             STX_TRY(stx_dev_alloc(b->ctx, bytes + 16, &arena));
-            b->pyr_allocs.push_back(arena);
+            b->wt_allocs.push_back(arena);
             size_t t = 0;
             for (size_t i = 0; i < b->images.size(); i++) {
                 if (!(b->images[i].kind == 0 && !b->built[i])) continue;
@@ -234,7 +239,7 @@
     StxMbImage* d = nullptr;
     STX_TRY(mb_upload(b, todo.data(), (int)todo.size(), &d));
     b->d_all = todo.size() == b->images.size() && memcmp(todo.data(), b->images.data(), sizeof(StxMbImage) * todo.size()) == 0 ? d : nullptr;
-    STX_TRY(stx_launch_mb_pyramids(b->ctx, d, todo.data(), (int)todo.size(), b->num_bands, pyr & 255, pyr >> 8));
+    STX_TRY(stx_launch_mb_pyramids(b->ctx, d, todo.data(), (int)todo.size(), b->num_bands, pyr & 255, pyr >> 8, b->adopted == nullptr));
     for (size_t i = 0; i < b->images.size(); i++) b->built[i] = 1;
     return STX_OK;
 }
@@ -266,6 +271,7 @@
 {
     if (!b || !img || !mask) return stx_fail(STX_ERR_INVALID, "null argument");
     if (b->finished) return stx_fail(STX_ERR_STATE, "feed after blend()");
+    if (b->adopted) return stx_fail(STX_ERR_STATE, "feed after stx_blend_use_weights adopted weights");
     if (!b->ctx) return stx_fail(STX_ERR_STATE, "geometry-only blender (created without a context)");
     STX_TRY(stx_set_device(b->ctx));
     if (img->c != 3 || (img->elem != STX_U8 && img->elem != STX_S16))
@@ -391,6 +397,105 @@
     return STX_OK;
 }
 
+void stx_mb_weights_release(stx_mb_weights* w)
+{
+    if (!w || --w->refs > 0) return;
+    if (w->ctx) hipSetDevice(w->ctx->device);
+    for (StxMbKept& k : w->images) stx_buf_release(k.mask);
+    for (void* p : w->allocs) stx_dev_free(w->ctx, p);
+    delete w;
+}
+
+static bool mb_weights_eligible(const stx_blender* b, bool built)
+{
+    if (b->kind != STX_BLEND_MULTIBAND || !b->ctx || b->num_bands < 1 || b->adopted) return false;
+    if ((b->pyr_mode & 255) != STX_PYRDOWN_SCALAR || getenv("STITCHING_AMD_NO_OCC") != nullptr || b->images.size() > 65535) return false;
+    for (const StxMbImage& im : b->images) {
+        if (im.kind != 0 || im.img0_is_s16) return false;
+        if (built && !im.occ[1]) return false;
+    }
+    return true;
+}
+
+static void mb_hand_over_weights(stx_blender* b)
+{
+    stx_mb_weights* w = b->keep;
+    if (!w || b->images.empty() || !mb_weights_eligible(b, true)) return;
+    w->num_bands = b->num_bands; w->pyr_mode = b->pyr_mode;
+    w->rx = b->rx; w->ry = b->ry; w->rw = b->rw; w->rh = b->rh;
+    for (const StxMbImage& im : b->images) {
+        StxMbKept k;
+        memset(&k, 0, sizeof(k));
+        for (size_t h = 1; h < b->held.size(); h += 2)
+            if (b->held[h]->ptr == im.mask0 && (long long)b->held[h]->stride == im.mask0_stride) k.mask = b->held[h];
+        if (!k.mask) {
+            for (StxMbKept& q : w->images) stx_buf_release(q.mask);
+            w->images.clear();
+            return;
+        }
+        stx_buf_retain(k.mask);
+        k.mask0 = im.mask0; k.mask0_stride = im.mask0_stride; k.mask_binary = im.mask_binary; k.w1_f16 = im.w1_f16;
+        k.iw = im.iw; k.ih = im.ih; k.ix = im.ix; k.iy = im.iy; k.fx = im.fx; k.fy = im.fy; k.fw = im.fw; k.fh = im.fh;
+        k.left = im.left; k.top = im.top;
+        for (int i = 1; i <= b->num_bands; i++) { k.wt[i] = im.wt[i]; k.wt_stride[i] = im.wt_stride[i]; k.occ[i] = im.occ[i]; }
+        w->images.push_back(k);
+    }
+    w->allocs.swap(b->wt_allocs);
+}
+
+STX_EXPORT int stx_blend_keep_weights(stx_blender* b, stx_mb_weights** out)
+{
+    if (!b || !out) return stx_fail(STX_ERR_INVALID, "null argument");
+    *out = nullptr;
+    if (b->finished) return stx_fail(STX_ERR_STATE, "keep_weights after blend()");
+    if (b->keep) return stx_fail(STX_ERR_STATE, "keep_weights was already called on this blender");
+    if (b->images.empty() || !mb_weights_eligible(b, false)) return STX_OK;
+    stx_mb_weights* w = new stx_mb_weights();
+    w->ctx = b->ctx;
+    w->refs = 2;
+    b->keep = w;
+    *out = w;
+    return STX_OK;
+}
+
+STX_EXPORT int stx_blend_use_weights(stx_blender* b, stx_mb_weights* w, int* out_adopted)
+{
+    if (!b || !w || !out_adopted) return stx_fail(STX_ERR_INVALID, "null argument");
+    *out_adopted = 0;
+    if (b->finished) return stx_fail(STX_ERR_STATE, "use_weights after blend()");
+    if (b->ctx != w->ctx) return stx_fail(STX_ERR_INVALID, "use_weights: the handle belongs to another context (no cross-stream use)");
+    if (b->adopted || b->keep || w->images.empty() || w->images.size() != b->images.size() || !mb_weights_eligible(b, false)) return STX_OK;
+    if (b->num_bands != w->num_bands || b->pyr_mode != w->pyr_mode || b->rx != w->rx || b->ry != w->ry || b->rw != w->rw || b->rh != w->rh)
+        return STX_OK;
+    for (size_t i = 0; i < b->images.size(); i++) {
+        const StxMbImage& im = b->images[i];
+        const StxMbKept& k = w->images[i];
+        if (b->built[i]) return STX_OK;
+        if (im.mask0 != k.mask0 || im.mask0_stride != k.mask0_stride || im.mask_binary != k.mask_binary || im.w1_f16 != k.w1_f16 ||
+            im.iw != k.iw || im.ih != k.ih || im.ix != k.ix || im.iy != k.iy || im.fx != k.fx || im.fy != k.fy || im.fw != k.fw ||
+            im.fh != k.fh || im.left != k.left || im.top != k.top)
+            return STX_OK;
+        for (int l = 1; l <= b->num_bands; l++)
+            if (im.wt_stride[l] != k.wt_stride[l]) return STX_OK;
+    }
+    STX_TRY(stx_set_device(b->ctx));
+    for (size_t i = 0; i < b->images.size(); i++)
+        for (int l = 1; l <= b->num_bands; l++) { b->images[i].wt[l] = w->images[i].wt[l]; b->images[i].occ[l] = w->images[i].occ[l]; }
+    for (void* p : b->wt_allocs) stx_dev_free(b->ctx, p);
+    b->wt_allocs.clear();
+    b->d_all = nullptr;
+    w->refs++;
+    b->adopted = w;
+    *out_adopted = 1;
+    return STX_OK;
+}
+
+STX_EXPORT int stx_mb_weights_free(stx_mb_weights* w)
+{
+    stx_mb_weights_release(w);
+    return STX_OK;
+}
+
 STX_EXPORT int stx_blend_set_band(stx_blender* b, int x0, int x1)
 {
     if (!b) return stx_fail(STX_ERR_INVALID, "null argument");
@@ -524,6 +629,7 @@
     if (!b || !rect_xywh || !packed) return stx_fail(STX_ERR_INVALID, "null argument");
     if (b->kind != STX_BLEND_MULTIBAND) return stx_fail(STX_ERR_UNSUPPORTED, "multi-band blender only");
     if (b->finished) return stx_fail(STX_ERR_STATE, "feed after blend()");
+    if (b->adopted) return stx_fail(STX_ERR_STATE, "feed after stx_blend_use_weights adopted weights");
     if (!b->ctx) return stx_fail(STX_ERR_STATE, "geometry-only blender (created without a context)");
     const int nb = b->num_bands, al = (1 << nb) - 1;
     const int x = rect_xywh[0], y = rect_xywh[1], w = rect_xywh[2], h = rect_xywh[3];
@@ -609,6 +715,7 @@
         if (b->kind == STX_BLEND_NO) return no_finish(b, pano.get(), pmask.get(), p16.get());
         return feather_finish(b, pano.get(), pmask.get(), p16.get());
     }();
+    if (rc == STX_OK) mb_hand_over_weights(b);
     b->finished = true;
     blender_release(b);
     STX_TRY(rc);
diff --git a/stitching_amd/csrc/stx_blend_kernels.h b/stitching_amd/csrc/stx_blend_kernels.h
--- a/stitching_amd/csrc/stx_blend_kernels.h
+++ b/stitching_amd/csrc/stx_blend_kernels.h
@@ -42,7 +42,7 @@
     unsigned long long* defer_list; unsigned* defer_count; unsigned defer_cap;
 };
 
-bool stx_fast_mb_down_batch(stx_ctx* ctx, const StxMbImage* d_images, const StxMbImage* h_images, int n, int level);
+bool stx_fast_mb_down_batch(stx_ctx* ctx, const StxMbImage* d_images, const StxMbImage* h_images, int n, int level, bool weights);
 bool stx_fast_mb_level(stx_ctx* ctx, const MbLevelK& K);
 
 int stx_fast_mb_emit_class(const MbLevelK& K, MbLevelK* KT);
diff --git a/stitching_amd/csrc/stx_internal.h b/stitching_amd/csrc/stx_internal.h
--- a/stitching_amd/csrc/stx_internal.h
+++ b/stitching_amd/csrc/stx_internal.h
@@ -180,7 +180,7 @@
     uint8_t* occ[STX_MAX_BANDS + 1];
 };
 int stx_launch_mb_pyramids(stx_ctx* ctx, const StxMbImage* d_images, const StxMbImage* h_images, int n, int num_bands, int pyr_mode,
-                           int pyr_lanes);
+                           int pyr_lanes, bool weights);
 struct MbLevelK;
 int stx_launch_mb_level(stx_ctx* ctx, const MbLevelK& K, double algo_bytes);
 int stx_launch_mb_coarse(stx_ctx* ctx, const MbLevelK& K_level_Bm2, double algo_bytes);
@@ -284,6 +284,9 @@
     std::vector<char> built;
     std::vector<stx_buf*> held;
     std::vector<void*> pyr_allocs;
+    std::vector<void*> wt_allocs;
+    stx_mb_weights* keep = nullptr;
+    stx_mb_weights* adopted = nullptr;
     StxMbImage* d_all = nullptr;
     int band_x0 = 0, band_x1 = 0;
     int next_order = 0;
@@ -291,5 +294,21 @@
     std::vector<NoImg> no_images;
     std::vector<FeatherImg> feather_images;
 };
+struct StxMbKept {
+    stx_buf* mask;
+    const uint8_t* mask0; long long mask0_stride; int mask_binary, w1_f16;
+    int iw, ih, ix, iy, fx, fy, fw, fh, left, top;
+    float* wt[STX_MAX_BANDS + 1]; long long wt_stride[STX_MAX_BANDS + 1];
+    uint8_t* occ[STX_MAX_BANDS + 1];
+};
+struct stx_mb_weights {
+    stx_ctx* ctx = nullptr;
+    std::atomic<int> refs{1};
+    int num_bands = 0, pyr_mode = 0;
+    int rx = 0, ry = 0, rw = 0, rh = 0;
+    std::vector<StxMbKept> images;
+    std::vector<void*> allocs;
+};
+void stx_mb_weights_release(stx_mb_weights* w);
 void mb_feed_rect(const stx_blender* b, int w, int h, int tlx, int tly, int* fx, int* fy, int* fw, int* fh);
 bool mb_contrib_range(const stx_blender* b, int fx, int fw, int bx0, int bx1, int* sx0, int* sx1);
diff --git a/stitching_amd/pipeline.py b/stitching_amd/pipeline.py
--- a/stitching_amd/pipeline.py
+++ b/stitching_amd/pipeline.py
@@ -74,11 +74,36 @@
     return cropper, crop_aspect
 
 
+class _RigGeometry:
+
+    __slots__ = ("key", "rects", "prep_corners", "prep_sizes", "feed_corners", "feed_masks", "blend_strength", "crop", "gain_in_warp",
+                 "gain_corners", "gain_sub", "weights", "blender")
+
+    def __init__(self):
+        self.key = self.weights = self.crop = self.gain_corners = self.gain_sub = None
+        self.blender = None
+        self.gain_in_warp = True
+
+
+def rig_key(cam_bytes, camera_aspect, warper_type, scale, sizes, blender_type, num_bands, blend_strength, modes, cropper, crop_aspect):
+    crop = None
+    if cropper is not None:
+        crop = (tuple(tuple(int(v) for v in r) for r in cropper.intersection_rectangles), float(crop_aspect))
+    return (cam_bytes, float(camera_aspect), str(warper_type), None if scale is None else float(scale), tuple((int(w), int(h)) for w, h in sizes),
+            str(blender_type), None if num_bands is None else int(num_bands), float(blend_strength) if num_bands is None else None,
+            tuple(modes), crop)
+
+
+def masks_belong_to_job(feed_masks, seam_masks):
+    given = feed_masks if feed_masks is not None else seam_masks
+    return given is None or all(isinstance(m, np.ndarray) for m in given)
+
+
 class StitchJob:
 
     def __init__(self, frames, cameras, warper_type="spherical", blender_type="multiband", num_bands=None,
                  blend_strength=Blender.DEFAULT_BLEND_STRENGTH, ctx=None, async_upload=False, feed_masks=None, seam_masks=None,
-                 crop_to_masks=True, compensator=None, cropper=None, crop_aspect=1, camera_aspect=1):
+                 crop_to_masks=True, compensator=None, cropper=None, crop_aspect=1, camera_aspect=1, reuse_geometry=True):
         cropper, crop_aspect = _split_cropper(cropper, crop_aspect)
         if len(frames) != len(cameras) or not frames:
             raise StitchingError("need one camera per frame and at least one frame")
@@ -97,11 +122,15 @@
         if cropper is not None and len(cropper.intersection_rectangles) != len(self.frames):
             raise StitchingError(f"the cropper was prepared on {len(cropper.intersection_rectangles)} images, the job has {len(self.frames)}")
         self._cam_arrays = self.warper.camera_arrays(self.cameras, camera_aspect)
+        self._cam_bytes = self._cam_arrays[0].tobytes() + self._cam_arrays[1].tobytes()
         self._mask_cols = None
         given = feed_masks if feed_masks is not None else seam_masks
         if crop_to_masks and given is not None and all(isinstance(m, np.ndarray) for m in given):
             self._mask_cols = [mask_box(m) for m in given]
         self._crop_cache = None
+        self.reuse_geometry = bool(reuse_geometry) and masks_belong_to_job(feed_masks, seam_masks)
+        self._geometry = None
+        self.last_reused = self.last_weights_adopted = False
         self.feed_masks = None if feed_masks is None else [as_device(m, self.ctx) for m in feed_masks]
         self.seam_masks = None if seam_masks is None else [as_device(m, self.ctx) for m in seam_masks]
 
@@ -128,56 +157,109 @@
             self._crop_cache = (key, view_rects(handle, corners, sizes, self._mask_cols))
         return self._crop_cache[1]
 
-    def run(self):
+    def set_frames(self, frames):
+        frames = list(frames)
+        got = [Images.get_image_size(f) for f in frames]
+        if got != [tuple(z) for z in self.sizes]:
+            raise StitchingError(f"the job was made for frames of sizes {self.sizes}, got {got}: same rig, same sizes")
+        self.frames = [as_device(f, self.ctx) for f in frames]
+
+    def release_geometry(self):
+        g, self._geometry = self._geometry, None
+        if g is not None and g.weights is not None:
+            g.weights.free()
+
+    def geometry_key(self):
+        modes = (config.trig_mode(), config.remap_mode()) + tuple(config.pyrdown_mode())
+        return rig_key(self._cam_bytes, self.camera_aspect, self.warper.warper_type, self.warper.scale, self.sizes, self.blender_type,
+                       self.num_bands, self.blend_strength, modes, self.cropper, self.crop_aspect)
+
+    def run(self, frames=None):
+        if frames is not None:
+            self.set_frames(frames)
         prev = config.device_resident()
         config.set_device_resident(True)
         try:
-            if self.cropper is not None:
-                return self._run_cropped()
-            warped = None
-            if self._mask_cols is None:
-                warped = self.warper.warp_images_and_masks(self.frames, self.cameras, self.camera_aspect, compensator=self.compensator,
-                                                           with_rois=True, camera_arrays=self._cam_arrays)
-                self._adopt([r[0:2] for r in warped[2]], [r[2:4] for r in warped[2]])
+            key = self.geometry_key() if self.reuse_geometry else None
+            g = self._geometry
+            if g is not None and g.key != key:
+                self.release_geometry()
+                g = None
+            self.last_reused, self.last_weights_adopted = g is not None, False
+            if g is None:
+                g, imgs = self._geometry_pass()
+                g.key = key
             else:
-                self.plan()
-            blender = Blender(self.blender_type, self.blend_strength, ctx=self.ctx)
-            blender.prepare(self.corners, self.warped_sizes)
-            crop = None
-            if self._mask_cols is not None and blender.blender.kind == _lib.BLEND_MULTIBAND:
-                crop = self._crop_rects(blender.blender, self.corners, self.warped_sizes)
-            if crop is not None:
-                box = [c if c is not None else (0, w, 0, h) for c, (w, h) in zip(crop, self.warped_sizes)]
-                rects = [(cx + x0, cy + y0, x1 - x0, y1 - y0) for (x0, x1, y0, y1), (cx, cy) in zip(box, self.corners)]
-                imgs, masks, rois = self.warper.warp_images_and_masks(self.frames, self.cameras, self.camera_aspect, rects=rects,
-                                                                      compensator=self.compensator, camera_arrays=self._cam_arrays)
-                if self.feed_masks is not None:
-                    masks = [m[y0:y1, x0:x1] for m, (x0, x1, y0, y1) in zip(self.feed_masks, box)]
-                else:
-                    masks = SeamFinder.resize_all(self.seam_masks, masks,
-                                                  sub=[(w, h, x0, y0) for (x0, x1, y0, y1), (w, h) in zip(box, self.warped_sizes)])
-                corners = [(r[0], r[1]) for r in rects]
-            else:
-                imgs, masks, rois = warped or self.warper.warp_images_and_masks(self.frames, self.cameras, self.camera_aspect,
-                                                                                compensator=self.compensator, camera_arrays=self._cam_arrays)
-                if self.feed_masks is not None:
-                    masks = self.feed_masks
-                elif self.seam_masks is not None:
-                    masks = SeamFinder.resize_all(self.seam_masks, masks)
-                corners = self.corners
-                for roi, corner in zip(rois, self.corners):
-                    if roi[0:2] != tuple(corner):
-                        raise StitchingError("warp roi changed between plan() and run()")
-            self.last_crop = crop
-            for img, mask, corner in zip(imgs, masks, corners):
+                imgs, _, _ = self.warper.warp_images_and_masks(self.frames, self.cameras, self.camera_aspect, rects=g.rects,
+                                                               compensator=self.compensator if g.gain_in_warp else None,
+                                                               camera_arrays=self._cam_arrays, masks=False)
+                if self.compensator is not None and not g.gain_in_warp:
+                    imgs = self.compensator.apply_all(g.gain_corners, imgs, None, sub=g.gain_sub, ctx=self.ctx)
+            self.last_crop = g.crop
+            blender, g.blender = g.blender, None
+            if blender is None:
+                blender = Blender(self.blender_type, g.blend_strength, ctx=self.ctx)
+                blender.prepare(g.prep_corners, g.prep_sizes)
+            for img, mask, corner in zip(imgs, g.feed_masks, g.feed_corners):
                 blender.feed(img, mask, corner)
             self.last_num_bands = blender.blender.num_bands()
+            if key is not None and blender.blender.kind == _lib.BLEND_MULTIBAND:
+                if not self.last_reused:
+                    g.weights = blender.blender.keep_weights()
+                elif g.weights is not None:
+                    self.last_weights_adopted = blender.blender.use_weights(g.weights)
             pano, pmask = blender.blend()
+            if key is not None:
+                self._geometry = g
         finally:
             config.set_device_resident(prev)
         return pano, pmask
 
-    def _run_cropped(self):
+    def _geometry_pass(self):
+        g = _RigGeometry()
+        if self.cropper is not None:
+            return self._geometry_pass_cropped(g)
+        warped = None
+        if self._mask_cols is None:
+            warped = self.warper.warp_images_and_masks(self.frames, self.cameras, self.camera_aspect, compensator=self.compensator,
+                                                       with_rois=True, camera_arrays=self._cam_arrays)
+            self._adopt([r[0:2] for r in warped[2]], [r[2:4] for r in warped[2]])
+        else:
+            self.plan()
+        g.blender = Blender(self.blender_type, self.blend_strength, ctx=self.ctx)
+        g.blender.prepare(self.corners, self.warped_sizes)
+        crop = None
+        if self._mask_cols is not None and g.blender.blender.kind == _lib.BLEND_MULTIBAND:
+            crop = self._crop_rects(g.blender.blender, self.corners, self.warped_sizes)
+        if crop is not None:
+            box = [c if c is not None else (0, w, 0, h) for c, (w, h) in zip(crop, self.warped_sizes)]
+            rects = [(cx + x0, cy + y0, x1 - x0, y1 - y0) for (x0, x1, y0, y1), (cx, cy) in zip(box, self.corners)]
+            imgs, masks, rois = self.warper.warp_images_and_masks(self.frames, self.cameras, self.camera_aspect, rects=rects,
+                                                                  compensator=self.compensator, camera_arrays=self._cam_arrays)
+            if self.feed_masks is not None:
+                masks = [m[y0:y1, x0:x1] for m, (x0, x1, y0, y1) in zip(self.feed_masks, box)]
+            else:
+                masks = SeamFinder.resize_all(self.seam_masks, masks,
+                                              sub=[(w, h, x0, y0) for (x0, x1, y0, y1), (w, h) in zip(box, self.warped_sizes)])
+            corners = [(r[0], r[1]) for r in rects]
+        else:
+            imgs, masks, rois = warped or self.warper.warp_images_and_masks(self.frames, self.cameras, self.camera_aspect,
+                                                                            compensator=self.compensator, camera_arrays=self._cam_arrays)
+            if self.feed_masks is not None:
+                masks = self.feed_masks
+            elif self.seam_masks is not None:
+                masks = SeamFinder.resize_all(self.seam_masks, masks)
+            corners = self.corners
+            for roi, corner in zip(rois, self.corners):
+                if roi[0:2] != tuple(corner):
+                    raise StitchingError("warp roi changed between plan() and run()")
+            rects = [(cx, cy, w, h) for (cx, cy), (w, h) in zip(self.corners, self.warped_sizes)]
+        g.rects, g.crop = [tuple(int(v) for v in r) for r in rects], crop
+        g.prep_corners, g.prep_sizes, g.blend_strength = list(self.corners), list(self.warped_sizes), self.blend_strength
+        g.feed_corners, g.feed_masks = list(corners), list(masks)
+        return g, imgs
+
+    def _geometry_pass_cropped(self, g):
         self.plan()
         cuts = [clip_rectangle(r.times(self.crop_aspect), w, h) for r, (w, h) in zip(self.cropper.intersection_rectangles, self.warped_sizes)]
         cut_sizes = [(x1 - x0, y1 - y0) for x0, x1, y0, y1 in cuts]
@@ -205,13 +287,11 @@
             masks = [m if b == (0, m.width, 0, m.height) else m[b[2]:b[3], b[0]:b[1]] for m, b in zip(self.feed_masks, box)]
         elif self.seam_masks is not None:
             masks = SeamFinder.resize_all(self.seam_masks, masks, sub=sub)
-        self.last_crop = crop
-        blender = Blender(self.blender_type, self.blend_strength, ctx=self.ctx)
-        blender.prepare(corners, sizes)
-        for img, mask, (cx, cy), b in zip(imgs, masks, corners, box):
-            blender.feed(img, mask, (cx + b[0], cy + b[2]))
-        self.last_num_bands = blender.blender.num_bands()
-        return blender.blend()
+        g.rects, g.crop = [tuple(int(v) for v in r) for r in rects], crop
+        g.gain_in_warp, g.gain_corners, g.gain_sub = False, corners, sub
+        g.prep_corners, g.prep_sizes, g.blend_strength = corners, sizes, self.blend_strength
+        g.feed_corners, g.feed_masks = [(cx + b[0], cy + b[2]) for (cx, cy), b in zip(corners, box)], list(masks)
+        return g, imgs
 
 
 def compose(frames, cameras, warper_type="spherical", blender_type="multiband", blend_strength=Blender.DEFAULT_BLEND_STRENGTH,
@@ -253,6 +333,7 @@
         self.cropper, self.compensator, self.seam_masks, self.seam_masks_host = cropper, compensator, seam_masks, seam_masks_host
         self.low_corners, self.low_sizes = low_corners, low_sizes
         self.frame_sizes = images.sizes
+        self.job = self.job_key = None
         R = Images.Resolution
         self.camera_aspect = images.get_ratio(R.MEDIUM, R.FINAL)
         self.lir_aspect = images.get_ratio(R.LOW, R.FINAL)
@@ -351,11 +432,16 @@
             final = list(plan.images.resize(Images.Resolution.FINAL, frames))
         finally:
             config.set_device_resident(prev)
-        job = StitchJob(final, plan.cameras, warper_type=st["warper_type"], blender_type=st["blender_type"],
-                        blend_strength=st["blend_strength"], ctx=ctx,
-                        seam_masks=plan.seam_masks_host if plan.seam_masks_host is not None else plan.seam_masks,
-                        compensator=plan.compensator, cropper=plan.cropper, crop_aspect=plan.lir_aspect, camera_aspect=plan.camera_aspect)
-        return job.run()
+        job_key = (id(ctx), st["warper_type"], st["blender_type"], st["blend_strength"])
+        if plan.job is None or plan.job_key != job_key:
+            plan.job = StitchJob(final, plan.cameras, warper_type=st["warper_type"], blender_type=st["blender_type"],
+                                 blend_strength=st["blend_strength"], ctx=ctx,
+                                 seam_masks=plan.seam_masks_host if plan.seam_masks_host is not None else plan.seam_masks,
+                                 compensator=plan.compensator, cropper=plan.cropper, crop_aspect=plan.lir_aspect,
+                                 camera_aspect=plan.camera_aspect)
+            plan.job_key = job_key
+            return plan.job.run()
+        return plan.job.run(frames=final)
 
     def compose(self, images, cameras):
         pano, _ = self.run(self.prepare(images, cameras))
diff --git a/stitching_amd/warper.py b/stitching_amd/warper.py
--- a/stitching_amd/warper.py
+++ b/stitching_amd/warper.py
@@ -133,7 +133,7 @@
                                                     src._h, C.byref(oi), C.byref(om), roi))
         return (self._result(DeviceImage(ctx, oi)), self._result(DeviceImage(ctx, om)), tuple(int(v) for v in roi))
 
-    def warp_images_and_masks(self, imgs, cameras, aspect=1, rects=None, compensator=None, with_rois=False, camera_arrays=None):
+    def warp_images_and_masks(self, imgs, cameras, aspect=1, rects=None, compensator=None, with_rois=False, camera_arrays=None, masks=True):
         ctx = self._ctx()
         srcs = [self._source(img, ctx) for img in imgs]
         cameras = list(cameras)
@@ -143,6 +143,10 @@
         Ks, Rs = camera_arrays if camera_arrays is not None else self.camera_arrays(cameras[:n], aspect)
         h_src = (C.c_void_p * n)(*[s._h for s in srcs[:n]])
         h_img, h_mask = (C.c_void_p * n)(), (C.c_void_p * n)()
+        if not masks:
+            if rects is None:
+                raise StitchingError("masks=False needs rects: the rectangles of the call that made the masks")
+            h_mask = None
         rois = np.zeros((n, 4), np.int32)
         blocks = compensator is not None and compensator.compensator_type in ("gain_blocks", "channel_blocks")
         if blocks and compensator.gains is None:
@@ -181,7 +185,7 @@
             finally:
                 config.set_device_resident(prev)
         imgs_out = [self._result(d) for d in d_imgs]
-        masks_out = [self._result(DeviceImage(ctx, C.c_void_p(h_mask[i]))) for i in range(n)]
+        masks_out = None if h_mask is None else [self._result(DeviceImage(ctx, C.c_void_p(h_mask[i]))) for i in range(n)]
         return imgs_out, masks_out, [tuple(int(v) for v in r) for r in rois]
 
     @staticmethod
```
